# fenghuayumo/DIVSHOT

Hardware: AMD Instinct MI355X
Metric: train views/sec (fwd+bwd raster) at 1M splats 1920x1080 (higher is better)
Workload: dtype f32; 1 GPU; C3: 1000000 splats, 1920x1080, SH degree 3, 8 views per iteration sharded over 1 GPU(s) (BASELINE config C4), 8 view(s) per GPU per step as 1 multi-view pass(es) of 8 view(s) (dvs_raster_forward_views / dvs_raster_backward_*); absgrad=True, mode=batch, stagger=False, groups=1, views_per_group=8, early_gather=False, a9_chunks=1, async_forward=True, hip_graph=False, fwd_variant=quadrant, grad_mode=0, tile_bounds=canonical, shN_layout=tiled[N/64][45][64]

## Files before the change

### divshot_amd/_lib.py

```python
import ctypes as C
import os

_HERE = os.path.dirname(os.path.abspath(__file__))
LIB_PATH = os.environ.get("DVS_RASTER_LIB") or os.path.join(_HERE, "lib", "libdvsraster.so")


class DvsError(RuntimeError):
    pass


if not os.path.exists(LIB_PATH):
    raise ImportError(
        f"{LIB_PATH} is missing: build it with `make -C divshot_amd/csrc` (or __graft_entry__.build()). "
        "divshot_amd has no CPU fallback.")

lib = C.CDLL(LIB_PATH, mode=C.RTLD_GLOBAL)


class Splats(C.Structure):
    _fields_ = [("pos", C.c_void_p), ("sh0", C.c_void_p), ("shN", C.c_void_p), ("opacity", C.c_void_p),
                ("scale", C.c_void_p), ("rot", C.c_void_p), ("n", C.c_int32), ("_pad", C.c_int32)]


class Camera(C.Structure):
    _fields_ = [("view", C.c_float * 16), ("proj", C.c_float * 16), ("tan_fovx", C.c_float), ("tan_fovy", C.c_float),
                ("focal_x", C.c_float), ("focal_y", C.c_float), ("campos", C.c_float * 3), ("width", C.c_int32),
                ("height", C.c_int32), ("bg", C.c_float * 3)]


class Opts(C.Structure):
    _fields_ = [("sh_degree", C.c_int32), ("antialias", C.c_int32), ("absgrad", C.c_int32), ("accumulate", C.c_int32),
                ("shn_layout", C.c_int32), ("grad_mode", C.c_int32), ("tile_bounds", C.c_int32), ("_reserved", C.c_int32 * 1)]


class FwdState(C.Structure):
    _fields_ = [("radii", C.c_void_p), ("splat2d", C.c_void_p), ("depth", C.c_void_p), ("flags", C.c_void_p), ("tiles_touched", C.c_void_p), ("sorted_tile", C.c_void_p),
                ("sorted_splat", C.c_void_p), ("ranges", C.c_void_p), ("final_T", C.c_void_p), ("n_contrib", C.c_void_p),
                ("num_rendered", C.c_uint64), ("n", C.c_int32), ("width", C.c_int32), ("height", C.c_int32),
                ("tiles_x", C.c_int32), ("tiles_y", C.c_int32), ("_pad", C.c_int32)]


class SplatGrads(C.Structure):
    _fields_ = [("pos", C.c_void_p), ("sh0", C.c_void_p), ("shN", C.c_void_p), ("opacity", C.c_void_p),
                ("scale", C.c_void_p), ("rot", C.c_void_p), ("absgrad2d", C.c_void_p), ("mean2d", C.c_void_p), ("dcolor", C.c_void_p)]


class DensifyParams(C.Structure):
    _fields_ = [("grad_threshold", C.c_float), ("scale_threshold", C.c_float), ("min_opacity", C.c_float), ("max_world_scale", C.c_float),
                ("max_screen_radius", C.c_int32), ("cap_max", C.c_int32), ("seed", C.c_uint32), ("shn_layout", C.c_int32), ("revised_opacity", C.c_int32)]


class AdamGroup(C.Structure):
    _fields_ = [("param", C.c_void_p), ("grad", C.c_void_p), ("m", C.c_void_p), ("v", C.c_void_p), ("count", C.c_uint64),
                ("lr", C.c_float), ("width", C.c_int32), ("layout", C.c_int32), ("active_chunks", C.c_int32)]


class MetricsView(C.Structure):
    _fields_ = [("img", C.c_void_p), ("target", C.c_void_p), ("mask", C.c_void_p)]


class DownsampleView(C.Structure):
    _fields_ = [("src", C.c_void_p), ("dst", C.c_void_p)]


class McmcSets(C.Structure):
    _fields_ = [("param", C.c_void_p * 6), ("m", C.c_void_p * 6), ("v", C.c_void_p * 6)]


class SceneSpec(C.Structure):
    _fields_ = [("n", C.c_int32), ("width", C.c_int32), ("height", C.c_int32), ("sh_degree", C.c_int32),
                ("n_cams", C.c_int32), ("seed", C.c_uint64), ("fov_x_deg", C.c_float), ("scale_log_offset", C.c_float)]


_PROTOS = {
    "dvs_create": (C.c_void_p, [C.c_int, C.c_size_t, C.c_int, C.c_int]),
    "dvs_create_views": (C.c_void_p, [C.c_int, C.c_size_t, C.c_int, C.c_int, C.c_int]),
    "dvs_destroy": (None, [C.c_void_p]),
    "dvs_raster_forward_views": (C.c_int, [C.c_void_p, C.c_void_p, C.POINTER(Splats), C.POINTER(Camera), C.c_int, C.POINTER(Opts), C.c_void_p]),
    "dvs_raster_forward_cancel_prepared": (C.c_int, [C.c_void_p]),
    "dvs_raster_forward_views_prepare": (C.c_int, [C.c_void_p, C.c_void_p, C.POINTER(Splats), C.POINTER(Camera), C.c_int, C.POINTER(Opts), C.c_int64, C.c_int64]),
    "dvs_raster_backward_views": (C.c_int, [C.c_void_p, C.c_void_p, C.POINTER(Splats), C.POINTER(Camera), C.c_int, C.POINTER(Opts),
                                            C.c_void_p, C.POINTER(SplatGrads)]),
    "dvs_get_view_state": (C.c_int, [C.c_void_p, C.c_int, C.POINTER(FwdState)]),
    "dvs_raster_forward": (C.c_int, [C.c_void_p, C.c_void_p, C.POINTER(Splats), C.POINTER(Camera), C.POINTER(Opts),
                                     C.c_void_p, C.POINTER(FwdState), C.POINTER(C.c_uint64)]),
    "dvs_raster_backward": (C.c_int, [C.c_void_p, C.c_void_p, C.POINTER(Splats), C.POINTER(Camera), C.POINTER(Opts),
                                      C.c_void_p, C.POINTER(SplatGrads)]),
    "dvs_raster_backward_composite": (C.c_int, [C.c_void_p, C.c_void_p, C.c_void_p, C.POINTER(Opts), C.c_void_p]),
    "dvs_raster_backward_project": (C.c_int, [C.c_void_p, C.c_void_p, C.POINTER(Splats), C.c_void_p, C.POINTER(Opts),
                                              C.POINTER(SplatGrads)]),
    "dvs_raster_backward_project_chunk": (C.c_int, [C.c_void_p, C.c_void_p, C.POINTER(Splats), C.c_void_p, C.POINTER(Opts),
                                                    C.POINTER(SplatGrads), C.c_int64, C.c_int64]),
    "dvs_raster_backward_dcolor": (C.c_int, [C.c_void_p, C.c_void_p, C.c_void_p]),
    "dvs_sh_grad_combine": (C.c_int, [C.c_void_p, C.c_void_p, C.c_int, C.c_void_p, C.c_int, C.c_int, C.c_void_p, C.c_void_p, C.c_void_p,
                                      C.c_void_p, C.c_int, C.c_int]),
    "dvs_shn_relayout": (C.c_int, [C.c_void_p, C.c_void_p, C.c_int, C.c_void_p, C.c_void_p, C.c_int]),
    "dvs_sort_pairs_u32": (C.c_int, [C.c_void_p, C.c_void_p, C.c_void_p, C.c_void_p, C.c_uint64, C.c_int, C.c_int]),
    "dvs_export_sorted_keys": (C.c_int, [C.c_void_p, C.c_void_p, C.c_void_p]),
    "dvs_get_bwd_intermediates": (C.c_int, [C.c_void_p, C.POINTER(C.c_void_p), C.POINTER(C.c_int)]),
    "dvs_keep_bwd_intermediates": (C.c_int, [C.c_void_p, C.c_int]),
    "dvs_set_async": (C.c_int, [C.c_void_p, C.c_int]),
    "dvs_get_num_rendered": (C.c_int, [C.c_void_p, C.c_void_p, C.POINTER(C.c_uint64)]),
    "dvs_get_sort_rank_mode": (C.c_int, [C.c_void_p]),
    "dvs_debug_sort_depth_keys": (C.c_int, [C.c_void_p, C.c_void_p, C.c_void_p, C.c_uint64, C.c_void_p, C.POINTER(C.c_uint32), C.POINTER(C.c_uint32)]),
    "dvs_set_export_sorted_tiles": (C.c_int, [C.c_void_p, C.c_int]),
    "dvs_get_arena_info": (C.c_int, [C.c_void_p, C.POINTER(C.c_uint64), C.POINTER(C.c_uint64), C.POINTER(C.c_uint64), C.POINTER(C.c_uint64)]),
    "dvs_set_backward_variant": (C.c_int, [C.c_void_p, C.c_int]),
    "dvs_debug_record_decisions": (C.c_int, [C.c_void_p, C.c_void_p, C.c_uint64]),
    "dvs_set_forward_variant": (C.c_int, [C.c_void_p, C.c_int]),
    "dvs_set_live_lists": (C.c_int, [C.c_void_p, C.c_int]),
    "dvs_enable_stage_timing": (C.c_int, [C.c_void_p, C.c_int]),
    "dvs_enable_kernel_probe": (C.c_int, [C.c_void_p, C.c_int]),
    "dvs_read_kernel_probe": (C.c_int, [C.c_void_p, C.POINTER(C.c_float), C.POINTER(C.c_int)]),
    "dvs_get_stage_timing": (C.c_int, [C.c_void_p, C.POINTER(C.POINTER(C.c_char_p)), C.POINTER(C.POINTER(C.c_float))]),
    "dvs_memcpy_d2h": (C.c_int, [C.c_void_p, C.c_void_p, C.c_void_p, C.c_size_t]),
    "dvs_memcpy_h2d": (C.c_int, [C.c_void_p, C.c_void_p, C.c_void_p, C.c_size_t]),
    "dvs_device_malloc": (C.c_void_p, [C.c_void_p, C.c_size_t]),
    "dvs_device_free": (None, [C.c_void_p, C.c_void_p]),
    "dvs_comm_create": (C.c_void_p, [C.c_int, C.c_int, C.c_int, C.c_char_p, C.c_int]),
    "dvs_comm_bootstrap": (C.c_int, [C.c_int, C.c_int, C.c_char_p, C.c_int, C.c_void_p]),
    "dvs_comm_destroy": (None, [C.c_void_p]),
    "dvs_comm_rank": (C.c_int, [C.c_void_p]),
    "dvs_comm_world": (C.c_int, [C.c_void_p]),
    "dvs_comm_backend_ranks": (C.c_int, [C.c_void_p]),
    "dvs_comm_backend_name": (C.c_char_p, [C.c_void_p]),
    "dvs_comm_all_reduce_sum_f32": (C.c_int, [C.c_void_p, C.c_void_p, C.c_void_p, C.c_size_t]),
    "dvs_comm_all_reduce_max_i32": (C.c_int, [C.c_void_p, C.c_void_p, C.c_void_p, C.c_size_t]),
    "dvs_comm_reduce_scatter_sum_f32": (C.c_int, [C.c_void_p, C.c_void_p, C.c_void_p, C.c_void_p, C.c_size_t]),
    "dvs_comm_all_gather_f32": (C.c_int, [C.c_void_p, C.c_void_p, C.c_void_p, C.c_void_p, C.c_size_t]),
    "dvs_comm_broadcast": (C.c_int, [C.c_void_p, C.c_void_p, C.c_void_p, C.c_size_t, C.c_int]),
    "dvs_comm_group_start": (C.c_int, [C.c_void_p]),
    "dvs_comm_group_end": (C.c_int, [C.c_void_p]),
    "dvs_last_error": (C.c_char_p, []),
    "dvs_version": (C.c_char_p, []),
    "dvs_synth_splats": (C.c_int, [C.POINTER(SceneSpec)] + [C.c_void_p] * 6),
    "dvs_synth_camera": (C.c_int, [C.POINTER(SceneSpec), C.c_int, C.POINTER(Camera)]),
    "dvs_synth_target": (C.c_int, [C.POINTER(SceneSpec), C.c_int, C.c_void_p]),
    "dvs_make_camera": (C.c_int, [C.c_void_p, C.c_void_p, C.c_float, C.c_int, C.c_int, C.POINTER(Camera)]),
    "dvs_make_camera_intrinsics": (C.c_int, [C.c_void_p, C.c_void_p, C.c_double, C.c_double, C.c_double, C.c_double, C.c_int, C.c_int, C.POINTER(Camera)]),
    "dvs_camera_downscale": (C.c_int, [C.POINTER(Camera), C.c_int, C.POINTER(Camera)]),
    "dvs_l1_loss_grad": (C.c_int, [C.c_void_p, C.c_void_p, C.c_void_p, C.c_size_t, C.c_void_p, C.c_void_p]),
    "dvs_l1_loss_grad_w": (C.c_int, [C.c_void_p, C.c_void_p, C.c_void_p, C.c_size_t, C.c_float, C.c_void_p, C.c_void_p]),
    "dvs_l2_loss_grad": (C.c_int, [C.c_void_p, C.c_void_p, C.c_void_p, C.c_size_t, C.c_float, C.c_void_p, C.c_void_p]),
    "dvs_ssim_forward": (C.c_int, [C.c_void_p, C.c_void_p, C.c_void_p, C.c_int, C.c_int, C.c_void_p, C.c_void_p, C.c_void_p, C.c_void_p]),
    "dvs_ssim_backward": (C.c_int, [C.c_void_p, C.c_void_p, C.c_void_p, C.c_int, C.c_int, C.c_void_p, C.c_void_p, C.c_void_p, C.c_float,
                                    C.c_void_p, C.c_int]),
    "dvs_loss_l1_ssim_backward": (C.c_int, [C.c_void_p, C.c_void_p, C.c_void_p, C.c_int, C.c_int, C.c_void_p, C.c_void_p, C.c_void_p, C.c_float,
                                            C.c_void_p, C.c_void_p]),
    "dvs_image_metrics_scratch_bytes": (C.c_size_t, [C.c_int, C.c_int, C.c_int]),
    "dvs_image_metrics_views": (C.c_int, [C.c_void_p, C.POINTER(MetricsView), C.c_int, C.c_int, C.c_int, C.c_int, C.c_void_p, C.c_void_p]),
    "dvs_downsample_views": (C.c_int, [C.c_void_p, C.POINTER(DownsampleView), C.c_int, C.c_int, C.c_int, C.c_int, C.c_int, C.c_int]),
    "dvs_densify_accumulate": (C.c_int, [C.c_void_p, C.c_int, C.c_void_p, C.c_void_p, C.c_int, C.c_int, C.c_void_p, C.c_void_p, C.c_void_p]),
    "dvs_densify_accumulate_rows": (C.c_int, [C.c_void_p, C.c_int, C.c_int, C.c_void_p, C.c_void_p, C.c_int, C.c_int, C.c_void_p, C.c_void_p, C.c_void_p]),
    "dvs_any_view_radius": (C.c_int, [C.c_void_p, C.c_int, C.c_int, C.c_void_p, C.c_void_p]),
    "dvs_densify_plan": (C.c_int, [C.c_void_p, C.c_int, C.c_void_p, C.c_void_p, C.c_void_p, C.c_void_p, C.c_void_p, C.POINTER(DensifyParams),
                                   C.c_void_p, C.c_void_p, C.c_void_p, C.c_void_p]),
    "dvs_densify_apply": (C.c_int, [C.c_void_p, C.c_int, C.c_void_p, C.c_void_p, C.POINTER(DensifyParams), C.c_int, C.c_void_p, C.c_void_p, C.c_int]),
    "dvs_reset_opacity": (C.c_int, [C.c_void_p, C.c_int, C.c_void_p, C.c_float, C.c_void_p, C.c_void_p]),
    "dvs_adam_step": (C.c_int, [C.c_void_p, C.c_void_p, C.c_void_p, C.c_void_p, C.c_void_p, C.c_size_t, C.c_float, C.c_float,
                                C.c_float, C.c_float, C.c_int]),
    "dvs_mcmc_scratch_bytes": (C.c_size_t, [C.c_int]),
    "dvs_mcmc_init_scratch": (C.c_int, [C.c_void_p, C.c_void_p, C.c_int]),
    "dvs_mcmc_relocate": (C.c_int, [C.c_void_p, C.c_int, C.POINTER(McmcSets), C.c_float, C.c_uint32, C.c_int, C.c_void_p, C.c_int, C.c_void_p]),
    "dvs_mcmc_grow": (C.c_int, [C.c_void_p, C.c_int, C.c_int, C.POINTER(McmcSets), C.c_float, C.c_uint32, C.c_int, C.c_void_p, C.c_int]),
    "dvs_mcmc_add_noise": (C.c_int, [C.c_void_p, C.c_int, C.c_void_p, C.c_void_p, C.c_void_p, C.c_void_p, C.c_float, C.c_uint32]),
    "dvs_mcmc_regularize": (C.c_int, [C.c_void_p, C.c_int, C.c_void_p, C.c_void_p, C.c_void_p, C.c_void_p, C.c_float, C.c_float]),
    "dvs_mcmc_add_noise_range": (C.c_int, [C.c_void_p, C.c_int, C.c_int, C.c_int, C.c_void_p, C.c_void_p, C.c_void_p, C.c_void_p, C.c_float, C.c_uint32]),
    "dvs_mcmc_regularize_range": (C.c_int, [C.c_void_p, C.c_int, C.c_int, C.c_int, C.c_void_p, C.c_void_p, C.c_void_p, C.c_void_p, C.c_float, C.c_float]),
    "dvs_adam_step_groups": (C.c_int, [C.c_void_p, C.POINTER(AdamGroup), C.c_int, C.c_float, C.c_float, C.c_float, C.c_int, C.c_void_p,
                                       C.c_int32]),
}
class SpzLayout(C.Structure):
    _fields_ = [("off", C.c_uint64 * 6), ("bytes", C.c_uint64 * 6), ("total", C.c_uint64)]


_EXPORT_PROTOS = {
    "dvs_pack_scratch_bytes": (C.c_size_t, [C.c_int]),
    "dvs_pack_compressed": (C.c_int, [C.c_void_p, C.c_int, C.c_void_p, C.c_void_p, C.c_void_p, C.c_void_p, C.c_void_p, C.c_void_p, C.c_void_p,
                                      C.c_void_p, C.c_void_p]),
    "dvs_pack_splat32": (C.c_int, [C.c_void_p, C.c_int, C.c_void_p, C.c_void_p, C.c_void_p, C.c_void_p, C.c_void_p, C.c_void_p]),
    "dvs_spz_layout_for": (C.c_int, [C.c_int, C.c_int, C.POINTER(SpzLayout)]),
    "dvs_pack_spz": (C.c_int, [C.c_void_p, C.c_int, C.c_int, C.c_void_p, C.c_void_p, C.c_void_p, C.c_int, C.c_void_p, C.c_void_p, C.c_void_p,
                               C.c_void_p]),
    "dvs_unpack_spz": (C.c_int, [C.c_void_p, C.c_int, C.c_int, C.c_void_p, C.c_void_p, C.c_void_p, C.c_void_p, C.c_int, C.c_void_p, C.c_void_p,
                                 C.c_void_p]),
}
_INIT_PROTOS = {
    "dvs_knn_scratch_bytes": (C.c_size_t, [C.c_int]),
    "dvs_knn_mean_dist2": (C.c_int, [C.c_void_p, C.c_int, C.c_void_p, C.c_void_p, C.c_void_p]),
    "dvs_knn_mean_dist2_stats": (C.c_int, [C.c_void_p, C.c_int, C.c_void_p, C.c_void_p, C.c_void_p, C.c_void_p]),
    "dvs_init_from_points": (C.c_int, [C.c_void_p, C.c_int, C.c_void_p, C.c_void_p, C.c_void_p, C.c_void_p, C.c_void_p, C.c_void_p, C.c_void_p]),
}
class JpegDesc(C.Structure):
    _fields_ = [("width", C.c_int32), ("height", C.c_int32), ("components", C.c_int32), ("hs", C.c_int32), ("vs", C.c_int32),
                ("blocks_w", C.c_int32 * 3), ("blocks_h", C.c_int32 * 3), ("_pad", C.c_int32), ("offset", C.c_uint64 * 3),
                ("quant", (C.c_uint16 * 64) * 3)]


_IMAGE_PROTOS = {
    "dvs_jpeg_reconstruct": (C.c_int, [C.c_void_p, C.POINTER(JpegDesc), C.c_void_p, C.c_void_p]),
}
for _name, (_res, _args) in list(_PROTOS.items()) + list(_EXPORT_PROTOS.items()) + list(_INIT_PROTOS.items()) + list(_IMAGE_PROTOS.items()):
    _f = getattr(lib, _name)
    _f.restype = _res
    _f.argtypes = _args


def check(status, what="dvs call"):
    if status != 0:
        raise DvsError(f"{what} failed with status {status}: {lib.dvs_last_error().decode()}")


_JPEG_HOST_PROTOS = {
    "gstrain_jpeg_open": (C.c_void_p, [C.c_char_p, C.c_char_p, C.c_int]),
    "gstrain_jpeg_info": (C.c_int, [C.c_void_p, C.c_void_p, C.c_void_p, C.c_void_p]),
    "gstrain_jpeg_coefficients": (C.c_int, [C.c_void_p, C.c_void_p]),
    "gstrain_jpeg_close": (None, [C.c_void_p]),
}
_host_lib = None


def host_lib():
    global _host_lib
    if _host_lib is None:
        path = os.path.join(_HERE, "lib", "libgsplyio.so")
        if not os.path.exists(path):
            raise ImportError(f"{path} is missing: build it with `make -C divshot_amd/gstrain`")
        h = C.CDLL(path)
        for name, (res, args) in _JPEG_HOST_PROTOS.items():
            f = getattr(h, name)
            f.restype = res
            f.argtypes = args
        _host_lib = h
    return _host_lib


def jpeg_decode_coefficients(path):
    import numpy as np
    h = host_lib()
    err = C.create_string_buffer(1024)
    f = h.gstrain_jpeg_open(os.fsencode(path), err, 1024)
    if not f:
        raise DvsError(err.value.decode(errors="replace"))
    try:
        ints, offs, desc = (C.c_int32 * 15)(), (C.c_uint64 * 4)(), JpegDesc()
        check(h.gstrain_jpeg_info(f, ints, C.addressof(desc.quant), offs), "gstrain_jpeg_info")
        desc.width, desc.height, desc.components, desc.hs, desc.vs = ints[0], ints[1], ints[2], ints[3], ints[6]
        for k in range(3):
            desc.blocks_w[k], desc.blocks_h[k], desc.offset[k] = ints[9 + k], ints[12 + k], offs[k]
        coef = np.zeros(offs[3], np.int16)
        check(h.gstrain_jpeg_coefficients(f, coef.ctypes.data), "gstrain_jpeg_coefficients")
        return desc, coef
    finally:
        h.gstrain_jpeg_close(f)
```

### divshot_amd/csrc/dvs_api.cpp

```cpp
#include <hip/hip_runtime.h>
#include <cstddef>
#include <cstdio>
#include <cstdlib>
#include <cstdint>
#include <cstring>
#include <mutex>
#include <string>
#include <vector>
#include "../../include/dvs_raster.h"
#include "dvs_kernels.h"

static thread_local std::string g_last_error;
static void set_error(const char* what, hipError_t e, const char* file, int line) {
    char buf[512];
    snprintf(buf, sizeof buf, "%s: %s (%s:%d)", what, hipGetErrorString(e), file, line);
    g_last_error = buf;
}
void dvs_set_last_error(const char* msg) { g_last_error = msg ? msg : ""; }
static int fail(int code, const char* who, const char* what) { g_last_error = std::string(who) + ": " + what; return code; }
#define HIPCHECK(expr) do { hipError_t _e = (expr); if (_e != hipSuccess) { set_error(#expr, _e, __FILE__, __LINE__); return DVS_ERR_HIP; } } while (0)
#define TRY(expr) do { int _r = (expr); if (_r != DVS_OK) return _r; } while (0)

namespace {
struct Buf {
    void* p = nullptr;
    size_t bytes = 0;
    ~Buf() { if (p) (void)hipFree(p); }
    int ensure(size_t need) {
        if (need <= bytes) return DVS_OK;
        if (p) { (void)hipFree(p); p = nullptr; bytes = 0; }
        size_t want = need + need / 4;
        hipError_t e = hipMalloc(&p, want);
        if (e != hipSuccess) { e = hipMalloc(&p, need); want = need; }
        if (e != hipSuccess) { set_error("hipMalloc", e, __FILE__, __LINE__); p = nullptr; return DVS_ERR_HIP; }
        bytes = want;
        return DVS_OK;
    }
    template <class T> T* as() const { return (T*)p; }
};
struct Carver {
    char* base; size_t off = 0;
    template <class T> T* take(size_t count) { T* p = base ? (T*)(base + off) : nullptr; off += count * sizeof(T); return p; }
};

static_assert(sizeof(DvsCam) == sizeof(dvs_camera) && offsetof(DvsCam, campos) == offsetof(dvs_camera, campos) &&
              offsetof(DvsCam, bg) == offsetof(dvs_camera, bg), "DvsCam must mirror dvs_camera");
DvsCam to_dev_cam(const dvs_camera& c) { DvsCam d; memcpy(&d, &c, sizeof d); return d; }
DvsCams pack_cams(const dvs_camera* cams, int V) {
    DvsCams d;
    for (int v = 0; v < V; ++v) d.c[v] = to_dev_cam(cams[v]);
    return d;
}
struct CamVec3 {
    float v[DVS_MAX_VIEWS * 3];
    CamVec3(const dvs_camera* cams, int V, float (dvs_camera::*field)[3]) {
        for (int i = 0; i < V; ++i) for (int k = 0; k < 3; ++k) v[3 * i + k] = (cams[i].*field)[k];
    }
};
int bits_for(uint32_t max_value) { int b = 0; while (max_value) { ++b; max_value >>= 1; } return b; }

struct TileGrid {
    int tiles_x, tiles_y, tiles, rect_fmt;
    TileGrid(int W, int H, int tile_bounds = DVS_TILES_CANONICAL)
        : tiles_x((W + DVS_TILE - 1) / DVS_TILE), tiles_y((H + DVS_TILE - 1) / DVS_TILE), tiles(tiles_x * tiles_y),
          rect_fmt(tile_bounds == DVS_TILES_TIGHT ? DVS_FE_RECT_TIGHT : (tiles_x <= 255 && tiles_y <= 255) ? DVS_FE_RECT_U8 : DVS_FE_RECT_U16) {}
};

struct FwdPass {
    hipStream_t st;
    const dvs_splats* p; const dvs_camera* cams; int V; const dvs_opts* opts;
    int n; TileGrid g;
    uint64_t T = 0, T_expected = 0;
    const uint64_t* T_dev = nullptr;
    int icur = 0;
    int ranges_encoded = 0;
    bool keys_written = true;
};

struct Arenas {
    Buf radii, splat2d, depth, flags, tiles_touched, rect, rect_sorted, key[2], ids[2];
    Buf ranges, final_T, n_contrib;
    Buf ranges_canon;
    Buf inst_tile[2], inst_splat[2];
    uint64_t inst_cap = 0;
    uint64_t inst_grow_events = 0;
    uint64_t* total_dev = nullptr;
    uint64_t* total_host = nullptr;
    uint64_t overflow_seen = 0;
    Buf tmp_keys, tmp_vals;
};
struct FrontEnd {
    Buf state, hist;
    uint32_t nbv = 0, nsb = 0;
    int rank_atomic = 0;
    DvsSeg *seg_all = nullptr, *seg_vis = nullptr, *seg_tile = nullptr;
    uint32_t *superexcl = nullptr, *totals = nullptr, *block_sums = nullptr, *kred = nullptr, *tile_ranges = nullptr;
    unsigned long long* super = nullptr;
    size_t zero_bytes = 0;
    int seg_n = -1, seg_V = -1;
    uint32_t seg_rows = 0;
    size_t carve_state(void* base, int max_views) {
        Carver k{(char*)base};
        seg_all = k.take<DvsSeg>(DVS_MAX_VIEWS); seg_vis = k.take<DvsSeg>(DVS_MAX_VIEWS); seg_tile = k.take<DvsSeg>(DVS_MAX_VIEWS);
        superexcl = k.take<uint32_t>((size_t)max_views * nsb);
        totals = k.take<uint32_t>((size_t)max_views * DVS_FE_MAXBINS);
        block_sums = k.take<uint32_t>((size_t)max_views * nbv);
        return k.off;
    }
    size_t carve_ranges(void* base, int max_views, size_t tiles) {
        Carver k{(char*)base};
        kred = k.take<uint32_t>(DVS_FE_KRED_WORDS);
        super = k.take<unsigned long long>((size_t)max_views * nsb * DVS_FE_SUPER_STRIDE);
        zero_bytes = k.off = (k.off + 255) & ~(size_t)255;
        tile_ranges = k.take<uint32_t>(tiles * 2);
        return k.off;
    }
};
struct Forward {
    dvs_fwd_state st{};
    int n_views = 1;
    bool have = false;
    uint32_t* live_splat = nullptr;
    uint32_t* live_pos = nullptr;
    bool live_lists = true;
    uint64_t* rec_masks = nullptr; uint64_t rec_cap = 0;
    struct Prep {
        bool valid = false;
        int64_t next = 0;
        int n = 0, V = 0;
        dvs_splats p{};
        dvs_opts opts{};
        dvs_camera cams[DVS_MAX_VIEWS];
    } prep;
};
struct Backward {
    Buf g_rows;
    Buf dcolor;
    int variant = DVS_BWD_TR;
    bool keep_rows = false;
    bool rows_clean = false;
    bool rows_pending = false;
    int64_t proj_next = 0;
};
struct Timing {
    struct Span { const char* name; size_t begin, end; };
    bool on = false;
    std::vector<hipEvent_t> events;
    size_t used = 0;
    std::vector<Span> spans;
    std::vector<const char*> out_names;
    std::vector<float> out_ms;
};
struct Probe {
    bool on = false;
    std::vector<hipEvent_t> ev;
    std::vector<int> kind;
    size_t used = 0;
};
}

struct dvs_ctx {
    int device = 0;
    size_t max_splats = 0;
    int max_w = 0, max_h = 0;
    int max_views = 1;
    bool async_T = false;
    bool export_tiles = false;
    Arenas a;
    FrontEnd fe;
    Forward fwd;
    Backward bwd;
    Timing timing;
    Probe probe;
    ~dvs_ctx() {
        if (a.total_dev) (void)hipFree(a.total_dev);
        if (a.total_host) (void)hipHostFree(a.total_host);
        for (const auto* pool : {&timing.events, &probe.ev}) for (hipEvent_t e : *pool) (void)hipEventDestroy(e);
    }
};

namespace {
enum : unsigned { DROP_FWD = 1u, DROP_ROWS = 2u, DROP_PREP = 4u, DROP_SEGS = 8u };
void invalidate(dvs_ctx* c, unsigned what) {
    if (what & DROP_FWD) c->fwd.have = false;
    if (what & DROP_ROWS) c->bwd.rows_pending = false;
    if (what & DROP_PREP) c->fwd.prep.valid = false;
    if (what & DROP_SEGS) c->fe.seg_n = -1;
}

struct StageScope {
    dvs_ctx* c; hipStream_t st; bool append; size_t last = 0;
    StageScope(dvs_ctx* c_, hipStream_t s, bool append_) : c(c_), st(s), append(append_) { c->timing.used = 0; c->timing.spans.clear(); }
    size_t mark() {
        Timing& t = c->timing;
        if (!t.on) return 0;
        if (t.used == t.events.size()) { hipEvent_t e; (void)hipEventCreate(&e); t.events.push_back(e); }
        (void)hipEventRecord(t.events[t.used], st);
        return t.used++;
    }
    void begin() { last = mark(); }
    void stage(const char* name) { const size_t e = mark(); if (c->timing.on) c->timing.spans.push_back({name, last, e}); last = e; }
    int finish() {
        Timing& t = c->timing;
        if (!t.on) return DVS_OK;
        HIPCHECK(hipStreamSynchronize(st));
        if (!append) { t.out_names.clear(); t.out_ms.clear(); }
        for (const Timing::Span& s : t.spans) {
            float ms = 0.f;
            (void)hipEventSynchronize(t.events[s.end]);
            (void)hipEventElapsedTime(&ms, t.events[s.begin], t.events[s.end]);
            t.out_names.push_back(s.name); t.out_ms.push_back(ms);
        }
        return DVS_OK;
    }
};
void probe_event(dvs_ctx* c, hipStream_t st, int opens = -1) {
    Probe& pr = c->probe;
    if (!pr.on) return;
    if (pr.used == pr.ev.size()) { hipEvent_t e; (void)hipEventCreate(&e); pr.ev.push_back(e); }
    (void)hipEventRecord(pr.ev[pr.used++], st);
    if (opens >= 0) pr.kind.push_back(opens);
}

bool fe_no_key16() { static const bool v = [] { const char* e = getenv("DVS_FE_NO_KEY16"); return e && e[0] == '1'; }(); return v; }
bool fe_no_fuse() { static const bool v = [] { const char* e = getenv("DVS_FE_NO_FUSE_A6"); return e && e[0] == '1'; }(); return v; }

int ensure_frontend_arenas(dvs_ctx* c) {
    FrontEnd& fe = c->fe;
    dvs_fe_block_counts((int)c->max_splats, &fe.nbv, &fe.nsb);
    TRY(fe.state.ensure(fe.carve_state(nullptr, c->max_views)));
    fe.carve_state(fe.state.p, c->max_views);
    return fe.hist.ensure(dvs_fe_hist_words((uint64_t)c->max_splats * c->max_views, c->max_views, DVS_FE_MAXBINS) * 4);
}
int ensure_splat_arenas(dvs_ctx* c, size_t n) {
    Arenas& a = c->a;
    const struct { Buf* buf; size_t each; } need[] = {{&a.radii, 4}, {&a.splat2d, 64}, {&a.depth, 4}, {&a.flags, 4}, {&a.tiles_touched, 4},
        {&a.rect, 16}, {&a.rect_sorted, 16}, {&a.key[0], 4}, {&a.key[1], 4}, {&a.ids[0], 4}, {&a.ids[1], 4}, {&c->bwd.g_rows, 48}};
    for (const auto& x : need) TRY(x.buf->ensure(n * x.each));
    return DVS_OK;
}
int ensure_image_arenas(dvs_ctx* c, int w, int h, int views) {
    const size_t P = (size_t)w * h * views;
    const size_t tiles = (size_t)TileGrid(w, h).tiles * views;
    TRY(c->a.ranges.ensure(c->fe.carve_ranges(nullptr, c->max_views, tiles)));
    c->fe.carve_ranges(c->a.ranges.p, c->max_views, tiles);
    TRY(c->a.ranges_canon.ensure(tiles * 8));
    TRY(c->a.final_T.ensure(P * 4));
    return c->a.n_contrib.ensure(P * 4);
}
int ensure_instance_arenas(dvs_ctx* c, uint64_t T) {
    Arenas& a = c->a;
    if (a.inst_cap && T > a.inst_cap) ++a.inst_grow_events;
    uint64_t cap = (1ull << 32) - 1;
    for (Buf* b : {&a.inst_tile[0], &a.inst_splat[0], &a.inst_tile[1], &a.inst_splat[1]}) {
        TRY(b->ensure(T * 4));
        if (b->bytes / 4 < cap) cap = b->bytes / 4;
    }
    a.inst_cap = cap;
    return c->fe.hist.ensure(dvs_fe_hist_words(a.inst_cap, c->max_views, 512) * 4);
}
}

extern "C" {

const char* dvs_last_error(void) { return g_last_error.c_str(); }
const char* dvs_version(void) { return "divshot_amd raster 0.1 (gfx950)"; }

dvs_ctx* dvs_create_views(int device, size_t max_splats, int max_w, int max_h, int max_views) {
    int count = 0;
    hipError_t e = hipGetDeviceCount(&count);
    if (e != hipSuccess || device < 0 || device >= count) { fail(0, "dvs_create", "no such HIP device (the rasterizer has no CPU fallback)"); return nullptr; }
    if (max_views < 1 || max_views > DVS_MAX_VIEWS) { fail(0, "dvs_create_views", "max_views must be in [1, 16]"); return nullptr; }
    if ((e = hipSetDevice(device)) != hipSuccess) { set_error("hipSetDevice", e, __FILE__, __LINE__); return nullptr; }
    dvs_ctx* c = new dvs_ctx();
    c->device = device; c->max_splats = max_splats; c->max_w = max_w; c->max_h = max_h; c->max_views = max_views;
    if (const char* v = getenv("DVS_BWD_VARIANT")) c->bwd.variant = v[0] == '0' ? DVS_BWD_BLOCKS : DVS_BWD_TR;
    if (const char* v = getenv("DVS_LIVE_LISTS")) c->fwd.live_lists = v[0] != '0';
    if (hipMalloc((void**)&c->a.total_dev, 32) != hipSuccess || hipHostMalloc((void**)&c->a.total_host, 32, hipHostMallocDefault) != hipSuccess ||
        hipMemset(c->a.total_dev, 0, 32) != hipSuccess) {
        fail(0, "dvs_create", "hipMalloc failed");
        delete c;
        return nullptr;
    }
    c->a.total_host[0] = c->a.total_host[1] = c->a.total_host[2] = c->a.total_host[3] = 0;
    {
        static int probed[64];
        static std::mutex probe_mutex;
        std::lock_guard<std::mutex> probe_lock(probe_mutex);
        const char* mode = getenv("DVS_FE_RANK");
        if (mode && mode[0] == 'b') c->fe.rank_atomic = 0;
        else {
            if (device < 64 && probed[device] == 0) {
                uint32_t bad = 1u;
                uint32_t* word = nullptr;
                if (hipMalloc((void**)&word, 4) == hipSuccess && hipMemset(word, 0, 4) == hipSuccess && dvs_fe_probe_rank_atomic(nullptr, word) == hipSuccess &&
                    hipMemcpy(&bad, word, 4, hipMemcpyDeviceToHost) == hipSuccess)
                    probed[device] = bad == 0u ? 1 : 2;
                if (word) (void)hipFree(word);
            }
            c->fe.rank_atomic = (device < 64 && probed[device] == 1) ? 1 : 0;
        }
    }
    if (const char* v = getenv("DVS_ASYNC")) c->async_T = v[0] == '1';
    if (ensure_frontend_arenas(c) != DVS_OK ||
        ensure_splat_arenas(c, max_splats * (size_t)max_views) != DVS_OK || ensure_image_arenas(c, max_w, max_h, max_views) != DVS_OK ||
        ensure_instance_arenas(c, (uint64_t)max_splats * 4 * (uint64_t)max_views) != DVS_OK) {
        dvs_destroy(c);
        return nullptr;
    }
    return c;
}
dvs_ctx* dvs_create(int device, size_t max_splats, int max_w, int max_h) { return dvs_create_views(device, max_splats, max_w, max_h, 1); }

void dvs_destroy(dvs_ctx* c) {
    if (!c) return;
    (void)hipSetDevice(c->device);
    delete c;
}

static int run_a2(dvs_ctx* c, hipStream_t st, const dvs_splats* p, const dvs_camera* cams, int V, const dvs_opts* opts, int64_t first, int64_t count, bool begin) {
    const TileGrid g(cams[0].width, cams[0].height, opts->tile_bounds);
    Arenas& a = c->a;
    if (begin) HIPCHECK(hipMemsetAsync(a.ranges.p, 0, c->fe.zero_bytes + (size_t)g.tiles * V * 8, st));
    HIPCHECK(dvs_launch_preprocess_fwd(st, p->n, p->pos, p->sh0, p->shN, p->opacity, p->scale, p->rot, pack_cams(cams, V), V, opts->sh_degree,
                                       opts->antialias, g.tiles_x, g.tiles_y, a.radii.as<int>(), a.splat2d.as<float>(),
                                       a.depth.as<float>(), a.flags.as<uint32_t>(), a.tiles_touched.as<uint32_t>(), a.key[0].as<uint32_t>(),
                                       opts->shn_layout, a.rect.as<uint32_t>(), g.rect_fmt, c->fe.kred, (int)first, (int)count));
    return DVS_OK;
}
static bool prep_matches(const dvs_ctx* c, const dvs_splats* p, const dvs_camera* cams, int V, const dvs_opts* opts) {
    const Forward::Prep& q = c->fwd.prep;
    return q.valid && q.n == p->n && q.V == V && memcmp(&q.p, p, sizeof *p) == 0 && memcmp(&q.opts, opts, sizeof *opts) == 0 &&
           memcmp(q.cams, cams, sizeof(dvs_camera) * (size_t)V) == 0;
}
static void publish_prep(dvs_ctx* c, const dvs_splats* p, const dvs_camera* cams, int V, const dvs_opts* opts, int64_t next) {
    Forward::Prep& q = c->fwd.prep;
    q.valid = true; q.next = next; q.n = p->n; q.V = V; q.p = *p; q.opts = *opts;
    memcpy(q.cams, cams, sizeof(dvs_camera) * (size_t)V);
}
static int ensure_segs(dvs_ctx* c, hipStream_t st, int n, int V, uint32_t rows) {
    FrontEnd& fe = c->fe;
    if (fe.seg_n == n && fe.seg_V == V && fe.seg_rows == rows) return DVS_OK;
    HIPCHECK(dvs_launch_seg_init(st, n, V, rows, fe.seg_all));
    fe.seg_n = n; fe.seg_V = V; fe.seg_rows = rows;
    return DVS_OK;
}


static int fwd_capacity_policy(dvs_ctx* c, FwdPass& f) {
    if (!c->async_T) return DVS_OK;
    Arenas& a = c->a;
    const uint64_t lastT = a.total_host[0], overflow = a.total_host[1];
    const bool overflowed = overflow != a.overflow_seen;
    if (overflowed || lastT + lastT / 8 > a.inst_cap) {
        a.overflow_seen = overflow;
        HIPCHECK(hipStreamSynchronize(f.st));
        TRY(ensure_instance_arenas(c, lastT + lastT / 2));
        if (overflowed)
            return fail(DVS_ERR_CAPACITY, "dvs_raster_forward (async)", "an earlier forward on this context produced more tile instances than the "
                        "instance arena held; its outputs are invalid. The arena has been enlarged — repeat that view.");
    }
    f.T = a.inst_cap;
    f.T_dev = a.total_dev;
    f.T_expected = lastT > 0 ? lastT + lastT / 16 + 4096 : 0;
    return DVS_OK;
}
static int fwd_project(dvs_ctx* c, const FwdPass& f, StageScope& tm) {
    const bool prepared = prep_matches(c, f.p, f.cams, f.V, f.opts) && c->fwd.prep.next == (int64_t)f.n;
    invalidate(c, DROP_PREP);
    tm.begin();
    if (!prepared) TRY(run_a2(c, f.st, f.p, f.cams, f.V, f.opts, 0, f.n, true));
    tm.stage("preprocess_fwd");
    return DVS_OK;
}
static hipError_t seg_binning(dvs_ctx* c, const FwdPass& f, uint32_t tile_part, unsigned long long capacity, int stage,
                              uint32_t* inst_tile = nullptr, uint32_t* inst_splat = nullptr, int key16 = 0) {
    Arenas& a = c->a; FrontEnd& fe = c->fe;
    return dvs_launch_seg_binning(f.st, f.n, f.V, f.g.rect_fmt, fe.seg_vis, fe.seg_tile, a.ids[1].as<uint32_t>(), a.rect.as<uint32_t>(),
                                  a.rect_sorted.as<uint32_t>(), fe.block_sums, fe.super, fe.superexcl, tile_part,
                                  (unsigned long long*)a.total_dev, capacity, stage, f.g.tiles_x, inst_tile, inst_splat, key16);
}
static int fwd_bin(dvs_ctx* c, FwdPass& f, StageScope& tm) {
    Arenas& a = c->a; FrontEnd& fe = c->fe;
    hipStream_t st = f.st;
    const int n = f.n, V = f.V, tiles = f.g.tiles;
    if (n > 0) {
        TRY(ensure_segs(c, st, n, V, dvs_depth_sort_rows_per_view(n, V)));
        HIPCHECK(dvs_launch_depth_sort(st, n, V, a.key[0].as<uint32_t>(), a.ids[0].as<uint32_t>(), a.key[1].as<uint32_t>(), a.ids[1].as<uint32_t>(),
                                       fe.seg_all, fe.seg_vis, fe.kred, fe.hist.as<uint32_t>(), fe.totals, fe.rank_atomic));
    }
    tm.stage("depth_sort");
    const uint64_t lastT = a.total_host[0];
    const uint64_t t_hint = f.T_expected ? f.T_expected : (lastT ? lastT : (uint64_t)n * V * 3);
    const uint32_t tile_part = dvs_fe_part_for(t_hint);
    if (n > 0) HIPCHECK(seg_binning(c, f, tile_part, c->async_T ? a.inst_cap : ~0ull, 0));
    else HIPCHECK(hipMemsetAsync(a.total_dev, 0, 8, st));
    HIPCHECK(hipMemcpyAsync(a.total_host, a.total_dev, 32, hipMemcpyDeviceToHost, st));
    tm.stage("tile_scan");
    if (!c->async_T) {
        HIPCHECK(hipStreamSynchronize(st));
        f.T = a.total_host[0];
        if (f.T >= (1ull << 32)) return fail(DVS_ERR_CAPACITY, "dvs_raster_forward", "more than 2^32 tile instances");
        TRY(ensure_instance_arenas(c, f.T ? f.T : 1));
    }
    const int key16 = (tiles <= 65536 && !fe_no_key16()) ? 1 : 0;
    tm.begin();
    if (n > 0) HIPCHECK(seg_binning(c, f, tile_part, a.inst_cap, 1, a.inst_tile[0].as<uint32_t>(), a.inst_splat[0].as<uint32_t>(), key16));
    tm.stage("duplicate");
    const bool fuse_a6 = !fe_no_fuse();
    f.keys_written = !(fuse_a6 && c->async_T) || c->export_tiles;
    if (n > 0) {
        const uint64_t cap = c->async_T ? a.inst_cap : f.T;
        const uint32_t nbtot = (uint32_t)(cap / tile_part) + (uint32_t)V + 2u;
        HIPCHECK(dvs_launch_seg_sort(st, V, a.inst_tile[0].as<uint32_t>(), a.inst_splat[0].as<uint32_t>(), a.inst_tile[1].as<uint32_t>(),
                                     a.inst_splat[1].as<uint32_t>(), fe.seg_tile, 0, tiles > 1 ? bits_for((uint32_t)(tiles - 1)) : 1,
                                     c->async_T ? (f.T_expected ? f.T_expected : a.inst_cap) : f.T, tile_part, nbtot, fe.hist.as<uint32_t>(), fe.totals,
                                     (uint32_t)tiles, &f.icur, fuse_a6 ? fe.tile_ranges : nullptr, f.keys_written ? 1 : 0, key16, fe.rank_atomic));
    }
    tm.stage("tile_sort");
    if (fuse_a6) f.ranges_encoded = n > 0 ? 1 : 0;
    else HIPCHECK(dvs_launch_tile_ranges(st, f.T, a.inst_tile[f.icur].as<uint32_t>(), fe.tile_ranges, f.T_dev, f.T_expected));
    tm.stage("tile_ranges");
    return DVS_OK;
}
static int fwd_composite_and_publish(dvs_ctx* c, const FwdPass& f, float* out_rgb, dvs_fwd_state* saved, uint64_t* num_rendered, StageScope& tm) {
    Arenas& a = c->a; Forward& fw = c->fwd;
    const int W = f.cams[0].width, H = f.cams[0].height, icur = f.icur;
    probe_event(c, f.st, 0);
    fw.live_splat = nullptr; fw.live_pos = nullptr;
    uint64_t* rec_masks = nullptr; uint64_t rec_cap = 0;
    if (fw.rec_masks && f.V == 1 && !c->async_T) {
        rec_masks = fw.rec_masks; rec_cap = fw.rec_cap;
        HIPCHECK(hipMemsetAsync(rec_masks, 0, (size_t)(f.T < rec_cap ? f.T : rec_cap) * 32, f.st));
    }
    if (fw.live_lists && c->bwd.variant == DVS_BWD_TR) { fw.live_splat = a.inst_splat[icur ^ 1].as<uint32_t>(); fw.live_pos = a.inst_tile[icur ^ 1].as<uint32_t>(); }
    uint32_t* const canon = f.ranges_encoded ? a.ranges_canon.as<uint32_t>() : nullptr;
    HIPCHECK(dvs_launch_render_fwd(f.st, W, H, f.g.tiles_x, f.g.tiles_y, f.V, c->fe.tile_ranges, a.inst_splat[icur].as<uint32_t>(),
                                   a.splat2d.as<float>(), CamVec3(f.cams, f.V, &dvs_camera::bg).v, out_rgb, a.final_T.as<float>(),
                                   a.n_contrib.as<uint32_t>(), fw.live_splat, fw.live_pos, rec_masks, rec_cap, canon));
    probe_event(c, f.st);
    tm.stage("render_fwd");

    dvs_fwd_state& s = fw.st;
    s.radii = a.radii.as<int32_t>(); s.splat2d = a.splat2d.as<float>(); s.depth = a.depth.as<float>();
    s.flags = a.flags.as<uint32_t>();
    s.tiles_touched = a.tiles_touched.as<uint32_t>();
    s.sorted_tile = f.keys_written ? a.inst_tile[icur].as<uint32_t>() : nullptr; s.sorted_splat = a.inst_splat[icur].as<uint32_t>();
    s.ranges = canon ? canon : c->fe.tile_ranges; s.final_T = a.final_T.as<float>(); s.n_contrib = a.n_contrib.as<uint32_t>();
    s.num_rendered = c->async_T ? DVS_T_UNKNOWN : f.T; s.n = f.n; s.width = W; s.height = H; s.tiles_x = f.g.tiles_x; s.tiles_y = f.g.tiles_y;
    s._pad = 0;
    fw.n_views = f.V;
    fw.have = true;
    if (saved) *saved = s;
    if (num_rendered) *num_rendered = s.num_rendered;
    return DVS_OK;
}
static int check_fwd_args(dvs_ctx* c, const dvs_splats* p, const dvs_camera* cams, int V, const dvs_opts* opts, const float* out_rgb) {
    const char* const who = "dvs_raster_forward";
    if (!c || !p || !cams || !opts || !out_rgb) return fail(DVS_ERR_INVALID, who, "null argument");
    if (V < 1 || V > c->max_views) return fail(DVS_ERR_CAPACITY, who, "n_views exceeds the max_views given to dvs_create_views");
    const dvs_camera* cam = &cams[0];
    if (p->n < 0 || cam->width <= 0 || cam->height <= 0 || opts->sh_degree < 0 || opts->sh_degree > 3 ||
        (opts->shn_layout != DVS_SHN_ROWS && opts->shn_layout != DVS_SHN_TILED) ||
        (opts->tile_bounds != DVS_TILES_CANONICAL && opts->tile_bounds != DVS_TILES_TIGHT))
        return fail(DVS_ERR_INVALID, who, "bad n / image size / sh_degree / shn_layout / tile_bounds");
    for (int v = 1; v < V; ++v)
        if (cams[v].width != cam->width || cams[v].height != cam->height) return fail(DVS_ERR_INVALID, who, "the views of a batch must share one image size");
    if (p->n > 0 && (((uintptr_t)p->pos | (uintptr_t)p->sh0 | (uintptr_t)p->shN | (uintptr_t)p->opacity | (uintptr_t)p->scale | (uintptr_t)p->rot) & 15u))
        return fail(DVS_ERR_INVALID, who, "parameter arrays must be 16-byte aligned");
    if ((size_t)p->n > c->max_splats || cam->width > c->max_w || cam->height > c->max_h)
        return fail(DVS_ERR_CAPACITY, who, "exceeds the capacity given to dvs_create");
    if ((uint64_t)p->n * (uint64_t)V >= (1ull << 31)) return fail(DVS_ERR_CAPACITY, who, "n * n_views must stay below 2^31");
    return DVS_OK;
}
static int forward_views(dvs_ctx* c, hipStream_t st, const dvs_splats* p, const dvs_camera* cams, int V, const dvs_opts* opts,
                         float* out_rgb, dvs_fwd_state* saved, uint64_t* num_rendered) {
    TRY(check_fwd_args(c, p, cams, V, opts, out_rgb));
    HIPCHECK(hipSetDevice(c->device));
    FwdPass f{st, p, cams, V, opts, p->n, TileGrid(cams[0].width, cams[0].height, opts->tile_bounds)};
    invalidate(c, DROP_FWD | DROP_ROWS);
    StageScope tm(c, st, false);
    TRY(fwd_capacity_policy(c, f));
    TRY(fwd_project(c, f, tm));
    TRY(fwd_bin(c, f, tm));
    TRY(fwd_composite_and_publish(c, f, out_rgb, saved, num_rendered, tm));
    return tm.finish();
}

int dvs_raster_forward(dvs_ctx* c, void* stream, const dvs_splats* p, const dvs_camera* cam, const dvs_opts* opts,
                       float* out_rgb, dvs_fwd_state* saved, uint64_t* num_rendered) {
    return forward_views(c, (hipStream_t)stream, p, cam, 1, opts, out_rgb, saved, num_rendered);
}

int dvs_raster_forward_views(dvs_ctx* c, void* stream, const dvs_splats* p, const dvs_camera* cams, int n_views, const dvs_opts* opts,
                             float* out_rgb) {
    return forward_views(c, (hipStream_t)stream, p, cams, n_views, opts, out_rgb, nullptr, nullptr);
}

int dvs_raster_forward_cancel_prepared(dvs_ctx* c) {
    if (!c) return fail(DVS_ERR_INVALID, "dvs_raster_forward_cancel_prepared", "null context");
    invalidate(c, DROP_PREP);
    return DVS_OK;
}
int dvs_raster_forward_views_prepare(dvs_ctx* c, void* stream, const dvs_splats* p, const dvs_camera* cams, int n_views, const dvs_opts* opts,
                                     int64_t first, int64_t count) {
    const char* const who = "dvs_raster_forward_views_prepare";
    static float dummy_rgb;
    TRY(check_fwd_args(c, p, cams, n_views, opts, &dummy_rgb));
    if (opts->shn_layout != DVS_SHN_TILED) return fail(DVS_ERR_INVALID, who, "needs the DVS_SHN_TILED layout");
    const bool begin = first == 0;
    if (!begin && !(prep_matches(c, p, cams, n_views, opts) && c->fwd.prep.next == first)) {
        invalidate(c, DROP_PREP);
        return fail(DVS_ERR_STATE, who, "chunks must cover [0, n) in ascending order with the same parameters, cameras and options");
    }
    if (count <= 0 || first < 0 || first + count > p->n || (first % 256) != 0) {
        invalidate(c, DROP_PREP);
        return fail(DVS_ERR_INVALID, who, "bad chunk (each starts at a multiple of 256 and lies inside [0, n))");
    }
    HIPCHECK(hipSetDevice(c->device));
    if (begin) invalidate(c, DROP_FWD | DROP_ROWS | DROP_PREP);
    const int r = run_a2(c, (hipStream_t)stream, p, cams, n_views, opts, first, count, begin);
    if (r != DVS_OK) { invalidate(c, DROP_PREP); return r; }
    publish_prep(c, p, cams, n_views, opts, first + count);
    return DVS_OK;
}

int dvs_get_view_state(dvs_ctx* c, int view, dvs_fwd_state* out) {
    if (!c || !out) return fail(DVS_ERR_INVALID, "dvs_get_view_state", "null argument");
    if (!c->fwd.have || view < 0 || view >= c->fwd.n_views) return fail(DVS_ERR_STATE, "dvs_get_view_state", "no such view in the last forward");
    dvs_fwd_state s = c->fwd.st;
    const size_t on = (size_t)view * s.n, op = (size_t)view * s.width * s.height, ot = (size_t)view * s.tiles_x * s.tiles_y;
    s.radii += on; s.splat2d += on * DVS_S2D_FLOATS; s.depth += on; s.flags += on; s.tiles_touched += on;
    s.ranges += 2 * ot; s.final_T += op; s.n_contrib += op;
    *out = s;
    return DVS_OK;
}

static int bwd_composite(dvs_ctx* c, hipStream_t st, const dvs_camera* cams, const dvs_opts* opts, const float* dL_drgb, StageScope& tm) {
    const dvs_fwd_state& s = c->fwd.st;
    Backward& b = c->bwd;
    const int V = c->fwd.n_views;
    tm.begin();
    if (!b.rows_clean) HIPCHECK(hipMemsetAsync(b.g_rows.p, 0, b.g_rows.bytes, st));
    b.rows_clean = false;
    tm.stage("bwd_zero");
    const CamVec3 bgs(cams, V, &dvs_camera::bg);
    probe_event(c, st, 1);
    if (b.variant == DVS_BWD_TR)
        HIPCHECK(dvs_launch_render_bwd_tr(st, s.width, s.height, s.tiles_x, s.tiles_y, V, s.ranges, s.sorted_splat, s.splat2d, bgs.v, s.final_T,
                                          s.n_contrib, dL_drgb, b.g_rows.as<float>(), opts->absgrad, opts->grad_mode, c->fwd.live_splat, c->fwd.live_pos));
    else
        HIPCHECK(dvs_launch_render_bwd_blocks(st, s.width, s.height, s.tiles_x, s.tiles_y, V, s.ranges, s.sorted_splat, s.splat2d,
                                              bgs.v, s.final_T, s.n_contrib, dL_drgb, b.g_rows.as<float>(), opts->absgrad, opts->grad_mode));
    probe_event(c, st);
    tm.stage("render_bwd");
    b.rows_pending = true;
    b.proj_next = 0;
    return DVS_OK;
}
static int bwd_project(dvs_ctx* c, hipStream_t st, const dvs_splats* p, const dvs_camera* cams, const dvs_opts* opts,
                       const dvs_splat_grads* out, int64_t first, int64_t count, StageScope& tm) {
    const dvs_fwd_state& s = c->fwd.st;
    Backward& b = c->bwd;
    const int V = c->fwd.n_views, n = p->n;
    tm.begin();
    if (opts->shn_layout == DVS_SHN_TILED) {
        const char* nf = getenv("DVS_A9_NO_FUSE_SH");
        const bool no_fuse = nf && nf[0] == '1';
        const bool fuse = !out->dcolor && out->sh0 && out->shN && !no_fuse;
        float* dcol = out->dcolor;
        if (!dcol && !fuse) { TRY(b.dcolor.ensure((size_t)V * n * 3 * sizeof(float))); dcol = b.dcolor.as<float>(); }
        HIPCHECK(dvs_launch_preprocess_bwd_views(st, n, V, p->pos, p->shN, p->opacity, p->scale, p->rot, pack_cams(cams, V), opts->sh_degree,
                                                 opts->antialias, s.radii, s.flags, b.g_rows.as<float>(), out->pos, out->opacity, out->scale,
                                                 out->rot, opts->absgrad ? out->absgrad2d : nullptr, out->mean2d, dcol, opts->accumulate,
                                                 b.keep_rows ? 0 : 1, opts->grad_mode, (int)first, (int)count, fuse ? out->sh0 : nullptr,
                                                 fuse ? out->shN : nullptr));
        if (!fuse && out->sh0 && out->shN)
            HIPCHECK(dvs_launch_sh_grad_combine(st, n, p->pos, opts->sh_degree, V, CamVec3(cams, V, &dvs_camera::campos).v, dcol, out->sh0,
                                                out->shN, opts->accumulate, 1));
    } else {
        for (int v = 0; v < V; ++v) {
            const DvsCam dcam = to_dev_cam(cams[v]);
            const size_t on = (size_t)v * n;
            HIPCHECK(dvs_launch_preprocess_bwd(st, n, p->pos, p->shN, p->opacity, p->scale, p->rot, dcam, opts->sh_degree, opts->antialias,
                                               s.radii + on, s.flags + on, b.g_rows.as<float>() + on * 12, out->pos, out->sh0, out->shN,
                                               out->opacity, out->scale, out->rot, opts->absgrad ? out->absgrad2d : nullptr, out->mean2d,
                                               out->dcolor ? out->dcolor + on * 3 : nullptr, (opts->accumulate || v > 0) ? 1 : 0,
                                               b.keep_rows ? 0 : 1, opts->shn_layout, opts->grad_mode));
        }
    }
    tm.stage("preprocess_bwd");
    b.proj_next = first + count < n ? first + count : 0;
    if (b.proj_next != 0) return DVS_OK;
    b.rows_clean = !b.keep_rows;
    b.rows_pending = b.keep_rows;
    return DVS_OK;
}
static int check_bwd_args(dvs_ctx* c, const dvs_splats* p, const dvs_camera* cams, int V , const dvs_opts* opts, const char* who) {
    if (!c || !cams || !opts) return fail(DVS_ERR_INVALID, who, "null argument");
    if (V < 0) V = c->fwd.n_views;
    if (opts->grad_mode != DVS_GRAD_TRUE && opts->grad_mode != DVS_GRAD_LINEAGE) return fail(DVS_ERR_INVALID, who, "bad grad_mode");
    if (!c->fwd.have || V != c->fwd.n_views || (p && c->fwd.st.n != p->n) || c->fwd.st.width != cams[0].width || c->fwd.st.height != cams[0].height)
        return fail(DVS_ERR_STATE, who, "no matching forward on this context");
    return DVS_OK;
}
static int check_dL(const float* dL_drgb, const char* who) {
    if (!dL_drgb) return fail(DVS_ERR_INVALID, who, "null argument");
    if ((uintptr_t)dL_drgb & 15u) return fail(DVS_ERR_INVALID, who, "dL_drgb must be 16-byte aligned (the composite backward reads it as 16-byte words)");
    return DVS_OK;
}
static int check_grads(const dvs_splats* p, const dvs_splat_grads* out, const char* who) {
    if (!p || !out) return fail(DVS_ERR_INVALID, who, "null argument");
    if (p->n > 0 && (!out->pos || !out->opacity || !out->scale || !out->rot || ((!out->sh0 || !out->shN) && !out->dcolor)))
        return fail(DVS_ERR_INVALID, who, "null gradient row pointer (sh0/shN may be NULL only when dcolor is given)");
    if (p->n > 0 && (((uintptr_t)out->pos | (uintptr_t)out->sh0 | (uintptr_t)out->shN | (uintptr_t)out->opacity | (uintptr_t)out->scale |
                      (uintptr_t)out->rot | (uintptr_t)out->absgrad2d | (uintptr_t)out->mean2d | (uintptr_t)out->dcolor) & 15u))
        return fail(DVS_ERR_INVALID, who, "gradient arrays must be 16-byte aligned");
    return DVS_OK;
}

static int backward_views(dvs_ctx* c, void* stream, const dvs_splats* p, const dvs_camera* cams, int V, const dvs_opts* opts,
                          const float* dL_drgb, const dvs_splat_grads* out, const char* who) {
    TRY(check_dL(dL_drgb, "dvs_raster_backward"));
    TRY(check_grads(p, out, who));
    TRY(check_bwd_args(c, p, cams, V, opts, who));
    HIPCHECK(hipSetDevice(c->device));
    StageScope tm(c, (hipStream_t)stream, true);
    TRY(bwd_composite(c, tm.st, cams, opts, dL_drgb, tm));
    TRY(bwd_project(c, tm.st, p, cams, opts, out, 0, p->n, tm));
    return tm.finish();
}
int dvs_raster_backward(dvs_ctx* c, void* stream, const dvs_splats* p, const dvs_camera* cam, const dvs_opts* opts,
                        const float* dL_drgb, const dvs_splat_grads* out) {
    return backward_views(c, stream, p, cam, 1, opts, dL_drgb, out, "dvs_raster_backward");
}
int dvs_raster_backward_views(dvs_ctx* c, void* stream, const dvs_splats* p, const dvs_camera* cams, int n_views, const dvs_opts* opts,
                              const float* dL_drgb, const dvs_splat_grads* out) {
    return backward_views(c, stream, p, cams, n_views, opts, dL_drgb, out, "dvs_raster_backward_views");
}

int dvs_raster_backward_composite(dvs_ctx* c, void* stream, const dvs_camera* cam, const dvs_opts* opts, const float* dL_drgb) {
    const char* const who = "dvs_raster_backward_composite";
    TRY(check_dL(dL_drgb, who));
    TRY(check_bwd_args(c, nullptr, cam, -1, opts, who));
    HIPCHECK(hipSetDevice(c->device));
    StageScope tm(c, (hipStream_t)stream, true);
    TRY(bwd_composite(c, tm.st, cam, opts, dL_drgb, tm));
    return tm.finish();
}

static int check_project(dvs_ctx* c, const dvs_splats* p, const dvs_camera* cam, const dvs_opts* opts, const dvs_splat_grads* out,
                         const char* who, const char* pending) {
    TRY(check_grads(p, out, who));
    TRY(check_bwd_args(c, p, cam, -1, opts, who));
    return c->bwd.rows_pending ? DVS_OK : fail(DVS_ERR_STATE, who, pending);
}
int dvs_raster_backward_project(dvs_ctx* c, void* stream, const dvs_splats* p, const dvs_camera* cam, const dvs_opts* opts,
                                const dvs_splat_grads* out) {
    const char* const who = "dvs_raster_backward_project";
    TRY(check_project(c, p, cam, opts, out, who, "no dvs_raster_backward_composite on this context"));
    if (c->bwd.proj_next != 0)
        return fail(DVS_ERR_STATE, who, "a dvs_raster_backward_project_chunk sequence is in progress on this context (finish it up to n)");
    HIPCHECK(hipSetDevice(c->device));
    StageScope tm(c, (hipStream_t)stream, true);
    TRY(bwd_project(c, tm.st, p, cam, opts, out, 0, p->n, tm));
    return tm.finish();
}

int dvs_raster_backward_project_chunk(dvs_ctx* c, void* stream, const dvs_splats* p, const dvs_camera* cam, const dvs_opts* opts,
                                      const dvs_splat_grads* out, int64_t first, int64_t count) {
    const char* const who = "dvs_raster_backward_project_chunk";
    TRY(check_project(c, p, cam, opts, out, who, "no dvs_raster_backward_composite pending on this context"));
    if (opts->shn_layout != DVS_SHN_TILED || !out->dcolor || out->sh0 || out->shN)
        return fail(DVS_ERR_INVALID, who, "needs the DVS_SHN_TILED layout and the factorised form (out->dcolor given, sh0 / shN NULL)");
    if (first != c->bwd.proj_next || count <= 0 || first + count > p->n || (first % 256) != 0)
        return fail(DVS_ERR_INVALID, who, "chunks must cover [0, n) in ascending order, each starting at a multiple of 256");
    HIPCHECK(hipSetDevice(c->device));
    StageScope tm(c, (hipStream_t)stream, true);
    TRY(bwd_project(c, tm.st, p, cam, opts, out, first, count, tm));
    return tm.finish();
}

int dvs_sort_pairs_u32(dvs_ctx* c, void* stream, uint32_t* keys, uint32_t* vals, uint64_t n, int bit_lo, int bit_hi) {
    if (!c || (n > 0 && (!keys || !vals)) || bit_lo < 0 || bit_hi > 32 || bit_lo > bit_hi) return fail(DVS_ERR_INVALID, "dvs_sort_pairs_u32", "bad argument");
    HIPCHECK(hipSetDevice(c->device));
    hipStream_t st = (hipStream_t)stream;
    if (n == 0) return DVS_OK;
    TRY(c->a.tmp_keys.ensure(n * 4));
    TRY(c->a.tmp_vals.ensure(n * 4));
    uint32_t* k[2] = {keys, c->a.tmp_keys.as<uint32_t>()};
    uint32_t* v[2] = {vals, c->a.tmp_vals.as<uint32_t>()};
    int cur = 0;
    if (n > (1ull << 32) - 4097ull) return fail(DVS_ERR_CAPACITY, "dvs_sort_pairs_u32", "n must be at most 2^32 - 4097");
    TRY(c->fe.hist.ensure(dvs_fe_hist_words(n, 1, 512) * 4));
    const uint32_t part = dvs_fe_part_for(n);
    HIPCHECK(dvs_launch_seg_init(st, (int)n, 1, 0, c->fe.seg_all));
    invalidate(c, DROP_SEGS);
    HIPCHECK(dvs_launch_seg_sort(st, 1, k[0], v[0], k[1], v[1], c->fe.seg_all, bit_lo, bit_hi - bit_lo, n, part, (uint32_t)(n / part) + 3u,
                                 c->fe.hist.as<uint32_t>(), c->fe.totals, 0u, &cur, nullptr, 1, 0, c->fe.rank_atomic));
    if (cur == 1) {
        HIPCHECK(hipMemcpyAsync(keys, k[1], n * 4, hipMemcpyDeviceToDevice, st));
        HIPCHECK(hipMemcpyAsync(vals, v[1], n * 4, hipMemcpyDeviceToDevice, st));
    }
    return DVS_OK;
}

int dvs_debug_sort_depth_keys(dvs_ctx* c, void* stream, const uint32_t* keys, uint64_t n, uint32_t* sorted_ids, uint32_t* n_sorted, uint32_t* digit_bits) {
    if (!c || !keys || !sorted_ids || !n_sorted || n == 0 || n > c->max_splats * (uint64_t)c->max_views || n >= (1ull << 31))
        return fail(DVS_ERR_INVALID, "dvs_debug_sort_depth_keys", "bad argument (n must be in [1, max_splats * max_views])");
    HIPCHECK(hipSetDevice(c->device));
    hipStream_t st = (hipStream_t)stream;
    Arenas& a = c->a; FrontEnd& fe = c->fe;
    std::vector<uint32_t> h(n);
    HIPCHECK(hipMemcpyAsync(h.data(), keys, n * 4, hipMemcpyDeviceToHost, st));
    HIPCHECK(hipStreamSynchronize(st));
    uint32_t mn = 0xFFFFFFFFu, mx = 0u; bool any = false;
    for (uint32_t k : h) if (k != 0xFFFFFFFFu) { mn = k < mn ? k : mn; mx = k > mx ? k : mx; any = true; }
    uint32_t slots[64 * 16] = {0};
    if (any) { slots[0] = ~mn; slots[1] = mx; }
    invalidate(c, DROP_FWD | DROP_PREP | DROP_SEGS);
    HIPCHECK(hipMemcpyAsync(fe.kred, slots, sizeof slots, hipMemcpyHostToDevice, st));
    HIPCHECK(hipMemcpyAsync(a.key[0].p, keys, n * 4, hipMemcpyDeviceToDevice, st));
    HIPCHECK(dvs_launch_seg_init(st, (int)n, 1, dvs_depth_sort_rows_per_view((int)n, 1), fe.seg_all));
    HIPCHECK(dvs_launch_depth_sort(st, (int)n, 1, a.key[0].as<uint32_t>(), a.ids[0].as<uint32_t>(), a.key[1].as<uint32_t>(), a.ids[1].as<uint32_t>(),
                                   fe.seg_all, fe.seg_vis, fe.kred, fe.hist.as<uint32_t>(), fe.totals, fe.rank_atomic));
    DvsSeg sv;
    HIPCHECK(hipMemcpyAsync(&sv, fe.seg_vis, sizeof sv, hipMemcpyDeviceToHost, st));
    HIPCHECK(hipStreamSynchronize(st));
    *n_sorted = sv.count;
    if (digit_bits) *digit_bits = sv.bits;
    HIPCHECK(hipMemcpyAsync(sorted_ids, a.ids[1].p, (size_t)sv.count * 4, hipMemcpyDeviceToDevice, st));
    HIPCHECK(hipMemsetAsync(fe.kred, 0, sizeof slots, st));
    return DVS_OK;
}

int dvs_export_sorted_keys(dvs_ctx* c, void* stream, uint64_t* out_keys) {
    const char* const who = "dvs_export_sorted_keys";
    if (!c || !out_keys) return fail(DVS_ERR_INVALID, who, "null argument");
    if (!c->fwd.have) return fail(DVS_ERR_STATE, who, "no forward state");
    const dvs_fwd_state& s = c->fwd.st;
    if (s.num_rendered == DVS_T_UNKNOWN) { uint64_t t; TRY(dvs_get_num_rendered(c, stream, &t)); }
    if (!s.sorted_tile)
        return fail(DVS_ERR_STATE, who, "the last forward was asynchronous (dvs_set_async) and did not materialise the sorted tile ids; "
                    "export the keys of a synchronous forward");
    HIPCHECK(hipSetDevice(c->device));
    HIPCHECK(dvs_launch_export_keys((hipStream_t)stream, s.num_rendered, s.sorted_tile, s.sorted_splat, s.depth, out_keys));
    return DVS_OK;
}

int dvs_shn_relayout(dvs_ctx* c, void* stream, int n, const float* src, float* dst, int to_tiled) {
    if (!c || n < 0 || (n > 0 && (!src || !dst))) return fail(DVS_ERR_INVALID, "dvs_shn_relayout", "bad argument");
    HIPCHECK(hipSetDevice(c->device));
    HIPCHECK(dvs_launch_shn_relayout((hipStream_t)stream, n, src, dst, to_tiled));
    return DVS_OK;
}

int dvs_sh_grad_combine(dvs_ctx* c, void* stream, int n, const float* pos, int sh_degree, int n_views, const float* campos,
                        const float* dcolor, float* g_sh0, float* g_shN, int accumulate, int shn_layout) {
    if (!c || n < 0 || n_views < 0 || sh_degree < 0 || sh_degree > 3 || (n > 0 && n_views > 0 && (!pos || !campos || !dcolor || !g_sh0 || !g_shN)))
        return fail(DVS_ERR_INVALID, "dvs_sh_grad_combine", "bad argument");
    HIPCHECK(hipSetDevice(c->device));
    HIPCHECK(dvs_launch_sh_grad_combine((hipStream_t)stream, n, pos, sh_degree, n_views, campos, dcolor, g_sh0, g_shN, accumulate, shn_layout));
    return DVS_OK;
}

int dvs_raster_backward_dcolor(dvs_ctx* c, void* stream, float* dcolor) {
    const char* const who = "dvs_raster_backward_dcolor";
    if (!c || !dcolor || ((uintptr_t)dcolor & 15u)) return fail(DVS_ERR_INVALID, who, "bad argument (dcolor: 16-byte aligned device array)");
    if (!c->bwd.rows_pending) return fail(DVS_ERR_STATE, who, "no dvs_raster_backward_composite pending on this context");
    HIPCHECK(hipSetDevice(c->device));
    const dvs_fwd_state& s = c->fwd.st;
    HIPCHECK(dvs_launch_dcolor_from_rows((hipStream_t)stream, (int64_t)c->fwd.n_views * s.n, s.radii, s.flags, c->bwd.g_rows.as<float>(), dcolor));
    return DVS_OK;
}

int dvs_set_async(dvs_ctx* c, int enable) {
    if (!c) return fail(DVS_ERR_INVALID, "dvs_set_async", "null context");
    c->async_T = enable != 0;
    return DVS_OK;
}
int dvs_get_num_rendered(dvs_ctx* c, void* stream, uint64_t* T) {
    const char* const who = "dvs_get_num_rendered";
    if (!c || !T) return fail(DVS_ERR_INVALID, who, "null argument");
    if (!c->fwd.have) return fail(DVS_ERR_STATE, who, "no forward state");
    HIPCHECK(hipSetDevice(c->device));
    HIPCHECK(hipStreamSynchronize((hipStream_t)stream));
    Arenas& a = c->a;
    *T = a.total_host[0];
    c->fwd.st.num_rendered = *T;
    if (a.total_host[1] != a.overflow_seen) {
        a.overflow_seen = a.total_host[1];
        (void)ensure_instance_arenas(c, *T + *T / 2);
        return fail(DVS_ERR_CAPACITY, who, "the last forward produced more tile instances than the instance arena held; its outputs are "
                    "invalid. The arena has been enlarged — repeat that view.");
    }
    return DVS_OK;
}

int dvs_get_sort_rank_mode(dvs_ctx* c) { return c ? c->fe.rank_atomic : -1; }
int dvs_set_export_sorted_tiles(dvs_ctx* c, int enable) {
    if (!c) return fail(DVS_ERR_INVALID, "dvs_set_export_sorted_tiles", "null context");
    c->export_tiles = enable != 0;
    return DVS_OK;
}

int dvs_get_arena_info(dvs_ctx* c, uint64_t* cap, uint64_t* grows, uint64_t* last_T, uint64_t* overflows) {
    if (!c) return fail(DVS_ERR_INVALID, "dvs_get_arena_info", "null context");
    if (cap) *cap = c->a.inst_cap;
    if (grows) *grows = c->a.inst_grow_events;
    if (last_T) *last_T = c->a.total_host[0];
    if (overflows) *overflows = c->a.total_host[1];
    return DVS_OK;
}

int dvs_debug_record_decisions(dvs_ctx* c, uint64_t* take_masks, uint64_t capacity_instances) {
    if (!c || (take_masks && (((uintptr_t)take_masks & 7u) || capacity_instances == 0))) return fail(DVS_ERR_INVALID, "dvs_debug_record_decisions", "bad argument");
    c->fwd.rec_masks = take_masks; c->fwd.rec_cap = take_masks ? capacity_instances : 0;
    return DVS_OK;
}

int dvs_set_backward_variant(dvs_ctx* c, int variant) {
    const char* const who = "dvs_set_backward_variant";
    if (!c || variant < DVS_BWD_BLOCKS || variant > DVS_BWD_TR) return fail(DVS_ERR_INVALID, who, "bad argument");
    if (variant == DVS_BWD_REDUCE || variant == DVS_BWD_MM)
        return fail(DVS_ERR_UNSUPPORTED, who, "the 'reduce' and 'mm' kernels are retired — this library contains 'tr' (default) and 'blocks' only");
    c->bwd.variant = variant;
    return DVS_OK;
}
int dvs_set_live_lists(dvs_ctx* c, int enable) {
    if (!c) return fail(DVS_ERR_INVALID, "dvs_set_live_lists", "null context");
    c->fwd.live_lists = enable != 0;
    return DVS_OK;
}
int dvs_set_forward_variant(dvs_ctx* c, int variant) {
    if (!c || (variant != 0 && variant != 1)) return fail(DVS_ERR_INVALID, "dvs_set_forward_variant", "bad argument");
    if (variant == 0)
        return fail(DVS_ERR_UNSUPPORTED, "dvs_set_forward_variant", "the per-block forward is retired — this library contains the quadrant forward only");
    return DVS_OK;
}

int dvs_keep_bwd_intermediates(dvs_ctx* c, int keep) { if (!c) return DVS_ERR_INVALID; c->bwd.keep_rows = keep != 0; return DVS_OK; }

int dvs_get_bwd_intermediates(dvs_ctx* c, const float** rows, int* row_floats) {
    if (!c) return DVS_ERR_INVALID;
    if (rows) *rows = c->bwd.g_rows.as<float>();
    if (row_floats) *row_floats = 12;
    return DVS_OK;
}

int dvs_enable_stage_timing(dvs_ctx* c, int enable) { if (!c) return DVS_ERR_INVALID; c->timing.on = enable != 0; return DVS_OK; }
int dvs_enable_kernel_probe(dvs_ctx* c, int enable) {
    if (!c) return DVS_ERR_INVALID;
    c->probe.on = enable != 0;
    c->probe.used = 0; c->probe.kind.clear();
    return DVS_OK;
}
int dvs_read_kernel_probe(dvs_ctx* c, float mean_ms[2], int count[2]) {
    if (!c || !mean_ms || !count) return DVS_ERR_INVALID;
    HIPCHECK(hipSetDevice(c->device));
    Probe& pr = c->probe;
    double sum[2] = {0, 0};
    count[0] = count[1] = 0;
    for (size_t k = 0; k < pr.kind.size() && 2 * k + 1 < pr.used; ++k) {
        float ms = 0.f;
        HIPCHECK(hipEventSynchronize(pr.ev[2 * k + 1]));
        HIPCHECK(hipEventElapsedTime(&ms, pr.ev[2 * k], pr.ev[2 * k + 1]));
        sum[pr.kind[k]] += ms; count[pr.kind[k]]++;
    }
    for (int i = 0; i < 2; ++i) mean_ms[i] = count[i] ? (float)(sum[i] / count[i]) : 0.f;
    pr.used = 0; pr.kind.clear();
    return DVS_OK;
}
int dvs_get_stage_timing(dvs_ctx* c, const char*** names, const float** ms) {
    if (!c) return 0;
    if (names) *names = c->timing.out_names.data();
    if (ms) *ms = c->timing.out_ms.data();
    return (int)c->timing.out_names.size();
}

int dvs_memcpy_d2h(dvs_ctx* c, void* host_dst, const void* dev_src, size_t bytes) {
    if (!c) return DVS_ERR_INVALID;
    HIPCHECK(hipSetDevice(c->device));
    HIPCHECK(hipDeviceSynchronize());
    HIPCHECK(hipMemcpy(host_dst, dev_src, bytes, hipMemcpyDeviceToHost));
    return DVS_OK;
}
int dvs_memcpy_h2d(dvs_ctx* c, void* dev_dst, const void* host_src, size_t bytes) {
    if (!c) return DVS_ERR_INVALID;
    HIPCHECK(hipSetDevice(c->device));
    HIPCHECK(hipMemcpy(dev_dst, host_src, bytes, hipMemcpyHostToDevice));
    return DVS_OK;
}
void* dvs_device_malloc(dvs_ctx* c, size_t bytes) {
    if (!c) return nullptr;
    void* p = nullptr;
    if (hipSetDevice(c->device) != hipSuccess || hipMalloc(&p, bytes ? bytes : 1) != hipSuccess) return nullptr;
    return p;
}
void dvs_device_free(dvs_ctx* c, void* p) { if (c && p) { (void)hipSetDevice(c->device); (void)hipFree(p); } }

}
```

### divshot_amd/csrc/dvs_kernels.h

```cpp
#pragma once
#include <hip/hip_runtime.h>
#include <stdint.h>
#include "dvs_device.h"

hipError_t dvs_launch_preprocess_fwd(hipStream_t st, int n, const float* pos, const float* sh0, const float* shN,
                                     const float* opacity, const float* scale, const float* rot, const DvsCams& cams, int n_views,
                                     int deg, int antialias, int tiles_x, int tiles_y, int* radii , float* splat2d,
                                     float* depth, uint32_t* flags,
                                     uint32_t* tiles_touched, uint32_t* depth_key, int shn_tiled,
                                     uint32_t* rect , int rect_fmt ,
                                     uint32_t* kred ,
                                     int first, int count );
hipError_t dvs_launch_preprocess_bwd(hipStream_t st, int n, const float* pos, const float* shN, const float* opacity,
                                     const float* scale, const float* rot, const DvsCam& cam, int deg, int antialias,
                                     const int* radii, const uint32_t* flags, float* grad_rows ,
                                     float* g_pos, float* g_sh0, float* g_shN, float* g_opacity, float* g_scale,
                                     float* g_rot, float* out_absgrad2d , float* out_mean2d ,
                                     float* out_dcolor , int accumulate, int rezero_rows, int shn_tiled, int grad_mode);
hipError_t dvs_launch_preprocess_bwd_views(hipStream_t st, int n, int n_views, const float* pos, const float* shN, const float* opacity,
                                           const float* scale, const float* rot, const DvsCams& cams, int deg, int antialias,
                                           const int* radii, const uint32_t* flags, float* grad_rows, float* g_pos, float* g_opacity,
                                           float* g_scale, float* g_rot, float* out_absgrad2d, float* out_mean2d, float* out_dcolor,
                                           int accumulate, int rezero_rows, int grad_mode, int first, int count, float* g_sh0 ,
                                           float* g_shN );
hipError_t dvs_launch_sh_grad_combine(hipStream_t st, int n, const float* pos, int deg, int n_views, const float* campos_host,
                                      const float* dcolor, float* g_sh0, float* g_shN, int accumulate, int shn_tiled);
hipError_t dvs_launch_dcolor_from_rows(hipStream_t st, int64_t total, const int* radii, const uint32_t* flags, const float* rows, float* dcolor);
hipError_t dvs_launch_shn_relayout(hipStream_t st, int n, const float* src, float* dst, int to_tiled);

struct DvsSeg {
    uint32_t base;
    uint32_t count;
    uint32_t pstart;
    uint32_t sub;
    uint32_t bits;
    uint32_t _r0, _r1, _r2;
};
enum { DVS_FE_RECT_U8 = 0 ,
       DVS_FE_RECT_U16 = 1 ,
       DVS_FE_RECT_TIGHT = 2  };
template <int FMT> struct FeRect;
template <> struct FeRect<DVS_FE_RECT_U8> {
    typedef uint32_t T;
    static __device__ __forceinline__ T pack(uint32_t minx, uint32_t miny, uint32_t maxx, uint32_t maxy, unsigned long long) {
        return minx | (miny << 8) | ((maxx - minx) << 16) | ((maxy - miny) << 24);
    }
    static __device__ __forceinline__ uint32_t count(T r) { return ((r >> 16) & 0xFFu) * (r >> 24); }
    static __device__ __forceinline__ uint32_t minx(T r) { return r & 0xFFu; }
    static __device__ __forceinline__ uint32_t miny(T r) { return (r >> 8) & 0xFFu; }
    static __device__ __forceinline__ uint32_t width(T r) { return (r >> 16) & 0xFFu; }
    static __device__ __forceinline__ T zero() { return 0u; }
};
template <> struct FeRect<DVS_FE_RECT_U16> {
    typedef uint2 T;
    static __device__ __forceinline__ T pack(uint32_t minx, uint32_t miny, uint32_t maxx, uint32_t maxy, unsigned long long) {
        return make_uint2(minx | (maxx << 16), miny | (maxy << 16));
    }
    static __device__ __forceinline__ uint32_t count(T r) { return ((r.x >> 16) - (r.x & 0xFFFFu)) * ((r.y >> 16) - (r.y & 0xFFFFu)); }
    static __device__ __forceinline__ uint32_t minx(T r) { return r.x & 0xFFFFu; }
    static __device__ __forceinline__ uint32_t miny(T r) { return r.y & 0xFFFFu; }
    static __device__ __forceinline__ uint32_t width(T r) { return (r.x >> 16) - (r.x & 0xFFFFu); }
    static __device__ __forceinline__ T zero() { return make_uint2(0u, 0u); }
};
template <> struct FeRect<DVS_FE_RECT_TIGHT> {
    typedef uint4 T;
    static __device__ __forceinline__ T pack(uint32_t minx, uint32_t miny, uint32_t maxx, uint32_t maxy, unsigned long long mask) {
        return make_uint4(minx | (maxx << 16), miny | (maxy << 16), (uint32_t)mask, (uint32_t)(mask >> 32));
    }
    static __device__ __forceinline__ uint32_t count(T r) {
        const uint32_t both = r.z & r.w;
        return both == 0xFFFFFFFFu ? ((r.x >> 16) - (r.x & 0xFFFFu)) * ((r.y >> 16) - (r.y & 0xFFFFu)) : (uint32_t)(__popc(r.z) + __popc(r.w));
    }
    static __device__ __forceinline__ uint32_t minx(T r) { return r.x & 0xFFFFu; }
    static __device__ __forceinline__ uint32_t miny(T r) { return r.y & 0xFFFFu; }
    static __device__ __forceinline__ uint32_t width(T r) { return (r.x >> 16) - (r.x & 0xFFFFu); }
    static __device__ __forceinline__ T zero() { return make_uint4(0u, 0u, 0u, 0u); }
};
#define DVS_FE_KRED_WORDS (DVS_MAX_VIEWS * 64 * 16)
#define DVS_FE_MAXBINS 2048
#define DVS_FE_SUPER_STRIDE 32
size_t dvs_fe_hist_words(uint64_t max_elems, int n_views, int max_bins);
uint32_t dvs_depth_sort_rows_per_view(int n, int V);
uint32_t dvs_fe_part_for(uint64_t grid_elems);
void dvs_fe_block_counts(int n, uint32_t* nbv, uint32_t* nsb);
hipError_t dvs_launch_seg_init(hipStream_t st, int n, int V, uint32_t rows_per_view, DvsSeg* seg_all);
hipError_t dvs_launch_depth_sort(hipStream_t st, int n, int V, uint32_t* keys0, uint32_t* vals0, uint32_t* keys1, uint32_t* vals1,
                                 DvsSeg* seg_all, DvsSeg* seg_vis, const uint32_t* kred, uint32_t* hist, uint32_t* totals ,
                                 int rank_atomic = 0 );
hipError_t dvs_launch_seg_sort(hipStream_t st, int V, uint32_t* keys0, uint32_t* vals0, uint32_t* keys1, uint32_t* vals1, DvsSeg* seg, int bit_lo, int bits,
                               uint64_t grid_elems, uint32_t part, uint32_t nbtot, uint32_t* hist, uint32_t* totals, uint32_t key_add_per_view,
                               int* result_in, uint32_t* ranges_enc = nullptr ,
                               int write_last_keys = 1, int first_keys16 = 0 , int rank_atomic = 0);
hipError_t dvs_fe_probe_rank_atomic(hipStream_t st, uint32_t* bad_dev);
hipError_t dvs_launch_seg_binning(hipStream_t st, int n, int V, int rect_fmt, const DvsSeg* seg_vis, DvsSeg* seg_tile, const uint32_t* sorted_ids,
                                  const uint32_t* rect, uint32_t* rect_sorted, uint32_t* block_sums, unsigned long long* super, uint32_t* superexcl,
                                  uint32_t tile_part, unsigned long long* total_dev, unsigned long long capacity, int stage, int tiles_x,
                                  uint32_t* inst_tile, uint32_t* inst_splat, int key16 = 0 );

hipError_t dvs_launch_tile_ranges(hipStream_t st, uint64_t T, const uint32_t* sorted_tile, uint32_t* ranges ,
                                  const uint64_t* T_dev = nullptr, uint64_t T_expected = 0);
hipError_t dvs_launch_export_keys(hipStream_t st, uint64_t T, const uint32_t* sorted_tile, const uint32_t* sorted_splat,
                                  const float* depth, uint64_t* out_keys);

hipError_t dvs_launch_render_fwd(hipStream_t st, int W, int H, int tiles_x, int tiles_y, int n_views, const uint32_t* ranges ,
                                 const uint32_t* sorted_splat, const float* splat2d, const float* bgs, float* out_color, float* final_T,
                                 uint32_t* n_contrib, uint32_t* live_splat , uint32_t* live_pos ,
                                 uint64_t* take_masks ,
                                 uint64_t take_cap, uint32_t* ranges_out = nullptr );
enum { DVS_BWD_BLOCKS = 0 , DVS_BWD_REDUCE = 1 , DVS_BWD_MM = 2 ,
       DVS_BWD_TR = 3  };

hipError_t dvs_launch_render_bwd_tr(hipStream_t st, int W, int H, int tiles_x, int tiles_y, int n_views, const uint32_t* ranges,
                                    const uint32_t* sorted_splat, const float* splat2d, const float* bgs , const float* final_T,
                                    const uint32_t* n_contrib, const float* dL_dout, float* grad_rows, int absgrad, int grad_mode,
                                    const uint32_t* live_splat ,
                                    const uint32_t* live_pos);

hipError_t dvs_launch_render_bwd_blocks(hipStream_t st, int W, int H, int tiles_x, int tiles_y, int n_views, const uint32_t* ranges,
                                        const uint32_t* sorted_splat, const float* splat2d, const float* bgs , const float* final_T,
                                        const uint32_t* n_contrib, const float* dL_dout, float* grad_rows, int absgrad, int grad_mode);

size_t dvs_morton_scratch_bytes(int n);
hipError_t dvs_launch_morton_order(hipStream_t st, int n, const float* pos, void* scratch, const uint32_t** sorted, const float** bounds);
```

### divshot_amd/csrc/frontend.hip

```cpp
#include <cstdlib>
#include "dvs_device.h"
#include "dvs_kernels.h"

#define FE_BLOCK 256
#define FE_WAVES (FE_BLOCK / 64)
#define FE_MAXBINS DVS_FE_MAXBINS
#define FE_REORDER_BITS 9
#define FE_CULLED 0xFFFFFFFFu

__device__ __forceinline__ uint32_t fe_lane() { return __builtin_amdgcn_mbcnt_hi(~0u, __builtin_amdgcn_mbcnt_lo(~0u, 0u)); }

__device__ __forceinline__ uint64_t fe_match(uint32_t d, bool valid, uint32_t b) {
    const uint64_t v0 = __ballot(valid);
    uint32_t lo = (uint32_t)v0, hi = (uint32_t)(v0 >> 32);
    for (uint32_t k = 0; k < b; ++k) {
        const uint32_t m = (uint32_t)(((int32_t)(d << (31u - k))) >> 31);
        const uint64_t bal = __ballot(m != 0u);
        lo = lo & ~((uint32_t)bal ^ m);
        hi = hi & ~((uint32_t)(bal >> 32) ^ m);
    }
    const uint64_t peers = ((uint64_t)hi << 32) | lo;
    return valid ? peers : 0ull;
}

// ... 382 lines not shown
    int c = 0, shift = bit_lo;
    for (int k = 0; k < npass; ++k) {
        const bool last = k == npass - 1;
        hipError_t e = fe_launch_pass(L, kk[c], vv[c], (last && !write_last_keys) ? nullptr : kk[c ^ 1], vv[c ^ 1], seg, nullptr, 0, k, shift, widths[k], 0,
                                      last ? key_add_per_view : 0u, nullptr, last ? ranges_enc : nullptr, (k == 0 && first_keys16) ? 1 : 0);
        if (e != hipSuccess) return e;
        shift += widths[k];
        c ^= 1;
    }
    if (result_in) *result_in = c;
    return hipSuccess;
}

__global__ void __launch_bounds__(FE_BLOCK)
k_fe_probe_rank_atomic(uint32_t* __restrict__ bad, uint32_t seed) {
    __shared__ uint32_t cnt_a[FE_WAVES * 256];
    __shared__ uint16_t cnt_b[FE_WAVES * 512];
    const uint32_t lane = fe_lane(), wave = threadIdx.x >> 6;
    uint32_t errs = 0;
    for (uint32_t pat = 0; pat < 24; ++pat) {
        for (uint32_t e = threadIdx.x; e < FE_WAVES * 256; e += FE_BLOCK) cnt_a[e] = 0u;
        for (uint32_t e = threadIdx.x; e < FE_WAVES * 512; e += FE_BLOCK) cnt_b[e] = 0;
        __syncthreads();
        const uint32_t bits = pat < 8 ? 9u : 1u + (pat - 8u) % 9u;
        for (uint32_t r = 0; r < 16; ++r) {
            uint32_t h = (lane * 0x9E3779B1u) ^ ((blockIdx.x * FE_WAVES + wave) * 0x85EBCA6Bu) ^ ((pat * 16u + r) * 0xC2B2AE35u) ^ seed;
            h ^= h >> 15; h *= 0x2C1B3C6Du; h ^= h >> 12;
            uint32_t d;
            switch (pat) {
                case 0: d = 5u; break;
                case 1: d = 6u + (lane & 1u); break;
                case 2: d = lane >> 1; break;
                case 3: d = lane / 3u; break;
                case 4: d = lane >> 5; break;
                case 5: d = lane & 7u; break;
                case 6: d = (lane & 1u) ? 511u : (h & 3u); break;
                case 7: d = 63u - lane; break;
                default: d = h & ((1u << bits) - 1u); break;
            }
            const bool valid = (h >> 20 & 15u) != 0u || pat < 8;
            uint32_t ra = 0, rb = 0;
            if (valid) {
                const uint32_t old = atomicAdd(&cnt_a[wave * 256u + (d >> 1)], (d & 1u) ? 0x10000u : 1u);
                ra = (d & 1u) ? (old >> 16) : (old & 0xFFFFu);
            }
            const uint64_t peers = fe_match(d, valid, 9u);
            const uint32_t below = __builtin_amdgcn_mbcnt_hi((uint32_t)(peers >> 32), __builtin_amdgcn_mbcnt_lo((uint32_t)peers, 0u));
            if (valid) {
                const uint32_t prev = cnt_b[wave * 512u + d];
                if (below == 0) cnt_b[wave * 512u + d] = (uint16_t)(prev + (uint32_t)__popcll(peers));
                rb = prev + below;
            }
            errs += (valid && ra != rb) ? 1u : 0u;
        }
        __syncthreads();
    }
    if (errs) atomicAdd(bad, errs);
}
hipError_t dvs_fe_probe_rank_atomic(hipStream_t st, uint32_t* bad_dev ) {
    hipLaunchKernelGGL(k_fe_probe_rank_atomic, dim3(512), dim3(FE_BLOCK), 0, st, bad_dev, 0x1234567u);
    hipLaunchKernelGGL(k_fe_probe_rank_atomic, dim3(512), dim3(FE_BLOCK), 0, st, bad_dev, 0x89ABCDEu);
    return hipGetLastError();
}

template <int FMT>
__global__ void __launch_bounds__(FE_BLOCK)
k_seg_blocksum(int n, int V, uint32_t nbv, uint32_t nsb, const DvsSeg* __restrict__ seg_vis, const uint32_t* __restrict__ sorted_ids,
               const typename FeRect<FMT>::T* __restrict__ rect, typename FeRect<FMT>::T* __restrict__ rect_sorted,
               uint32_t* __restrict__ block_sums, unsigned long long* __restrict__ super) {
    __shared__ uint32_t wsum[4][FE_WAVES];
    const uint32_t view = blockIdx.x % (uint32_t)V, blk0 = (blockIdx.x / (uint32_t)V) * 4u;
    const uint32_t nvis = seg_vis[view].count;
    if (blk0 * FE_BLOCK >= nvis) return;
    const size_t o = (size_t)view * n;
    const uint32_t lane = fe_lane(), wave = threadIdx.x >> 6;
    uint32_t id[4];
#pragma unroll
    for (int k = 0; k < 4; ++k) { const uint32_t j = (blk0 + (uint32_t)k) * FE_BLOCK + threadIdx.x; id[k] = j < nvis ? sorted_ids[o + j] : 0u; }
    typename FeRect<FMT>::T r[4];
#pragma unroll
    for (int k = 0; k < 4; ++k) r[k] = rect[o + id[k]];
#pragma unroll
    for (int k = 0; k < 4; ++k) {
        const uint32_t j = (blk0 + (uint32_t)k) * FE_BLOCK + threadIdx.x;
        uint32_t v = 0;
        if (j < nvis) { rect_sorted[o + j] = r[k]; v = FeRect<FMT>::count(r[k]); }
        const uint32_t s = fe_wave_sum(v);
        if (lane == 0) wsum[k][wave] = s;
    }
    __syncthreads();
    if (threadIdx.x < 4) {
        const uint32_t k = threadIdx.x, blk = blk0 + k;
        uint32_t tot = 0;
#pragma unroll
        for (int wv = 0; wv < FE_WAVES; ++wv) tot += wsum[k][wv];
        if (blk < nbv) block_sums[(size_t)view * nbv + blk] = tot;
        const uint32_t t4 = tot + (uint32_t)__shfl_down(tot, 1, 64) + (uint32_t)__shfl_down(tot, 2, 64) + (uint32_t)__shfl_down(tot, 3, 64);
        if (k == 0 && t4) atomicAdd(&super[((size_t)view * nsb + (blk0 >> 8)) * DVS_FE_SUPER_STRIDE], (unsigned long long)t4);
    }
}

__global__ void __launch_bounds__(1024)
k_seg_totals(int V, uint32_t nsb, const unsigned long long* __restrict__ super, uint32_t* __restrict__ superexcl, DvsSeg* __restrict__ seg_tile,
             uint32_t tile_part, unsigned long long* __restrict__ total, unsigned long long capacity) {
    __shared__ unsigned long long vsum[DVS_MAX_VIEWS];
    const uint32_t lane = fe_lane(), wave = threadIdx.x >> 6;
    if (wave < (uint32_t)V) {
        unsigned long long carry = 0ull;
        for (uint32_t c0 = 0; c0 < nsb; c0 += 64) {
            const uint32_t i = c0 + lane;
            const unsigned long long v = i < nsb ? super[((size_t)wave * nsb + i) * DVS_FE_SUPER_STRIDE] : 0ull;
            unsigned long long inc = v;
#pragma unroll
            for (int k = 1; k < 64; k <<= 1) { const unsigned long long o = __shfl_up(inc, k, 64); if (lane >= (uint32_t)k) inc += o; }
            const unsigned long long ex = carry + inc - v;
            if (i < nsb) superexcl[(size_t)wave * nsb + i] = ex > 0xFFFFFFFFull ? 0xFFFFFFFFu : (uint32_t)ex;
            carry += __shfl(inc, 63, 64);
        }
        if (lane == 0) vsum[wave] = carry;
    }
    __syncthreads();
    if (threadIdx.x == 0) {
        unsigned long long start = 0ull;
        uint32_t prow = 0;
        for (int v = 0; v < V; ++v) {
            const unsigned long long end = start + vsum[v];
            const unsigned long long cs = start < capacity ? start : capacity, ce = end < capacity ? end : capacity;
            DvsSeg s;
            s.base = (uint32_t)cs; s.count = (uint32_t)(ce - cs); s.pstart = prow; s.sub = 0u; s.bits = 0u; s._r0 = s._r1 = s._r2 = 0u;
            seg_tile[v] = s;
            prow += (s.count + tile_part - 1) / tile_part;
            start = end;
        }
        total[0] = start;
        if (start > capacity) total[1] += 1ull;
    }
}

__device__ __forceinline__ uint32_t fe_nth_set_bit64(uint32_t lo, uint32_t hi, uint32_t t) {
    uint32_t w = lo, base = 0;
    const uint32_t c = (uint32_t)__popc(lo);
    if (t >= c) { t -= c; w = hi; base = 32u; }
#pragma unroll
    for (uint32_t h = 16u; h >= 1u; h >>= 1) {
        const uint32_t cl = (uint32_t)__popc(w & ((1u << h) - 1u));
        if (t >= cl) { t -= cl; w >>= h; base += h; }
    }
    return base;
}

__device__ __forceinline__ uint32_t fe_wave_incl_max(uint32_t v) {
#define FE_DPP_MAX(ctrl, rmask) { const uint32_t o_ = (uint32_t)__builtin_amdgcn_update_dpp(0, (int)v, ctrl, rmask, 0xF, false); v = v > o_ ? v : o_; }
    FE_DPP_MAX(0x111, 0xF); FE_DPP_MAX(0x112, 0xF); FE_DPP_MAX(0x114, 0xF); FE_DPP_MAX(0x118, 0xF);
    FE_DPP_MAX(0x142, 0xA);
    FE_DPP_MAX(0x143, 0xC);
#undef FE_DPP_MAX
    return v;
}
template <int FMT>
__global__ void __launch_bounds__(FE_BLOCK)
k_seg_duplicate(int n, int V, uint32_t nbv, uint32_t nsb, const DvsSeg* __restrict__ seg_vis, const DvsSeg* __restrict__ seg_tile,
                const uint32_t* __restrict__ sorted_ids, const typename FeRect<FMT>::T* __restrict__ rect_sorted,
                const uint32_t* __restrict__ block_sums, const uint32_t* __restrict__ superexcl, int tiles_x,
                uint32_t* __restrict__ inst_tile, uint32_t* __restrict__ inst_splat, unsigned long long capacity, int key16 ) {
    __shared__ uint32_t tmp[FE_WAVES];
    __shared__ uint32_t s_pre[FE_BLOCK];
    __shared__ uint32_t s_id[FE_BLOCK];
    __shared__ uint32_t s_tile[FE_BLOCK];
    __shared__ uint32_t s_w[FE_BLOCK];
    __shared__ uint32_t s_mark[FE_BLOCK];
    __shared__ uint2 s_mask[FMT == DVS_FE_RECT_TIGHT ? FE_BLOCK : 1];
    const uint32_t view = blockIdx.x % (uint32_t)V, blk0 = (blockIdx.x / (uint32_t)V) * 2u;
    const uint32_t nvis = seg_vis[view].count;
    if (blk0 * FE_BLOCK >= nvis) return;
    const size_t o = (size_t)view * n;
    const uint32_t lane = fe_lane(), w0 = (threadIdx.x >> 6) * 64u;
    uint32_t id[2] = {0u, 0u};
    typename FeRect<FMT>::T r[2] = {FeRect<FMT>::zero(), FeRect<FMT>::zero()};
#pragma unroll
    for (int h = 0; h < 2; ++h) {
        const uint32_t j = (blk0 + (uint32_t)h) * FE_BLOCK + threadIdx.x;
        if (j < nvis) { id[h] = sorted_ids[o + j]; r[h] = rect_sorted[o + j]; }
    }
    const uint32_t sb = blk0 >> 8, nprev = blk0 & 255u;
    const uint32_t part = threadIdx.x < nprev ? block_sums[(size_t)view * nbv + (size_t)sb * 256 + threadIdx.x] : 0u;
    const unsigned long long vbase = (unsigned long long)seg_tile[view].base + superexcl[(size_t)view * nsb + sb];
    uint32_t before, tot;
    (void)fe_block_excl_scan(part, tmp, &before);
#pragma unroll
    for (int h = 0; h < 2; ++h) {
        if ((blk0 + (uint32_t)h) * FE_BLOCK >= nvis) break;
        const uint32_t touched = FeRect<FMT>::count(r[h]);
        const uint32_t pre = fe_block_excl_scan(touched, tmp, &tot);
        s_pre[threadIdx.x] = pre;
        s_id[threadIdx.x] = (uint32_t)o + id[h];
        s_tile[threadIdx.x] = FeRect<FMT>::miny(r[h]) * (uint32_t)tiles_x + FeRect<FMT>::minx(r[h]);
        s_w[threadIdx.x] = FeRect<FMT>::width(r[h]);
        if constexpr (FMT == DVS_FE_RECT_TIGHT) s_mask[threadIdx.x] = make_uint2(r[h].z, r[h].w);
        const unsigned long long gbase = vbase + before;
        const uint32_t k_beg = (uint32_t)__builtin_amdgcn_readfirstlane((int)pre);
        const uint32_t k_end = (uint32_t)__builtin_amdgcn_readlane((int)(pre + touched), 63);
        uint32_t cur1 = 0;
        for (uint32_t k0 = k_beg; k0 < k_end; k0 += 64u) {
            s_mark[w0 + lane] = 0u;
            __builtin_amdgcn_wave_barrier();
            const uint32_t rel = pre - k0;
            if (touched != 0u && rel < 64u) s_mark[w0 + rel] = lane + 1u;
            __builtin_amdgcn_wave_barrier();
            uint32_t m = s_mark[w0 + lane];
            __builtin_amdgcn_wave_barrier();
            m = fe_wave_incl_max(m);
            m = m > cur1 ? m : cur1;
            cur1 = (uint32_t)__builtin_amdgcn_readlane((int)m, 63);
            const uint32_t k = k0 + lane;
            if (k < k_end) {
                const uint32_t src = w0 + m - 1u, w = s_w[src];
                uint32_t t = k - s_pre[src];
                if constexpr (FMT == DVS_FE_RECT_TIGHT) {
                    const uint2 mk = s_mask[src];
                    if ((mk.x & mk.y) != 0xFFFFFFFFu) t = fe_nth_set_bit64(mk.x, mk.y, t);
                }
                uint32_t q = (uint32_t)((float)t * __builtin_amdgcn_rcpf((float)w));
                int32_t rem = (int32_t)(t - q * w);
                if (rem < 0) { --q; rem += (int32_t)w; } else if (rem >= (int32_t)w) { ++q; rem -= (int32_t)w; }
                const unsigned long long g = gbase + k;
                if (g < capacity) {
                    const uint32_t tile = s_tile[src] + q * (uint32_t)tiles_x + (uint32_t)rem;
                    if (key16) reinterpret_cast<uint16_t*>(inst_tile)[g] = (uint16_t)tile; else inst_tile[g] = tile;
                    inst_splat[g] = s_id[src];
                }
            }
        }
        before += tot;
        __builtin_amdgcn_wave_barrier();
    }
}

hipError_t dvs_launch_seg_binning(hipStream_t st, int n, int V, int rect_fmt, const DvsSeg* seg_vis, DvsSeg* seg_tile, const uint32_t* sorted_ids,
                                  const uint32_t* rect, uint32_t* rect_sorted, uint32_t* block_sums, unsigned long long* super, uint32_t* superexcl,
                                  uint32_t tile_part, unsigned long long* total_dev, unsigned long long capacity, int stage ,
                                  int tiles_x, uint32_t* inst_tile, uint32_t* inst_splat, int key16) {
    if (n <= 0 || V <= 0) return hipSuccess;
    const uint32_t nbv = (uint32_t)((n + FE_BLOCK - 1) / FE_BLOCK), nsb = (nbv + 255u) / 256u;
    const dim3 grid(((nbv + 1u) / 2u) * (uint32_t)V), grid3(((nbv + 3u) / 4u) * (uint32_t)V), blk(FE_BLOCK);
    if (stage == 0) {
#define FE_A3(F) hipLaunchKernelGGL(k_seg_blocksum<F>, grid3, blk, 0, st, n, V, nbv, nsb, seg_vis, sorted_ids, (const FeRect<F>::T*)rect, (FeRect<F>::T*)rect_sorted, block_sums, super)
        if (rect_fmt == DVS_FE_RECT_U8) FE_A3(DVS_FE_RECT_U8); else if (rect_fmt == DVS_FE_RECT_U16) FE_A3(DVS_FE_RECT_U16); else FE_A3(DVS_FE_RECT_TIGHT);
#undef FE_A3
        hipLaunchKernelGGL(k_seg_totals, dim3(1), dim3(1024), 0, st, V, nsb, (const unsigned long long*)super, superexcl, seg_tile, tile_part, total_dev, capacity);
    } else {
#define FE_A4(F) hipLaunchKernelGGL(k_seg_duplicate<F>, grid, blk, 0, st, n, V, nbv, nsb, seg_vis, (const DvsSeg*)seg_tile, sorted_ids, (const FeRect<F>::T*)rect_sorted, \
                                    (const uint32_t*)block_sums, (const uint32_t*)superexcl, tiles_x, inst_tile, inst_splat, capacity, key16)
        if (rect_fmt == DVS_FE_RECT_U8) FE_A4(DVS_FE_RECT_U8); else if (rect_fmt == DVS_FE_RECT_U16) FE_A4(DVS_FE_RECT_U16); else FE_A4(DVS_FE_RECT_TIGHT);
#undef FE_A4
    }
    return hipGetLastError();
}
void dvs_fe_block_counts(int n, uint32_t* nbv, uint32_t* nsb) { *nbv = (uint32_t)((n + FE_BLOCK - 1) / FE_BLOCK); *nsb = (*nbv + 255u) / 256u; }

__global__ void k_seg_init(int n, int V, uint32_t rows_per_view, DvsSeg* __restrict__ seg_all) {
    const int v = threadIdx.x;
    if (v < V) { DvsSeg s; s.base = (uint32_t)v * (uint32_t)n; s.count = (uint32_t)n; s.pstart = (uint32_t)v * rows_per_view; s.sub = 0; s.bits = 8; s._r0 = s._r1 = s._r2 = 0; seg_all[v] = s; }
}
hipError_t dvs_launch_seg_init(hipStream_t st, int n, int V, uint32_t rows_per_view, DvsSeg* seg_all) {
    hipLaunchKernelGGL(k_seg_init, dim3(1), dim3(64), 0, st, n, V, rows_per_view, seg_all);
    return hipGetLastError();
}

__global__ void __launch_bounds__(FE_BLOCK)
k_tile_ranges(uint64_t T_host, const uint64_t* __restrict__ T_dev, const uint32_t* __restrict__ sorted_tile, uint2* __restrict__ ranges) {
    const uint64_t T = T_dev ? (*T_dev < T_host ? *T_dev : T_host) : T_host;
    for (uint64_t q = (uint64_t)blockIdx.x * FE_BLOCK + threadIdx.x; q * 4 < T; q += (uint64_t)gridDim.x * FE_BLOCK) {
        const uint64_t j0 = q * 4;
        uint32_t t[6];
        if (j0 + 4 <= T) {
            const uint4 v = reinterpret_cast<const uint4*>(sorted_tile)[q];
            t[1] = v.x; t[2] = v.y; t[3] = v.z; t[4] = v.w;
        } else {
#pragma unroll
            for (int k = 0; k < 4; ++k) t[1 + k] = j0 + k < T ? sorted_tile[j0 + k] : 0xFFFFFFFFu;
        }
        t[0] = j0 > 0 ? sorted_tile[j0 - 1] : 0xFFFFFFFFu;
        t[5] = j0 + 4 < T ? sorted_tile[j0 + 4] : 0xFFFFFFFFu;
#pragma unroll
        for (int k = 0; k < 4; ++k) {
            const uint64_t j = j0 + k;
            if (j < T) {
                if (j == 0 || t[k] != t[k + 1]) ranges[t[k + 1]].x = (uint32_t)j;
                if (j + 1 == T || t[k + 2] != t[k + 1]) ranges[t[k + 1]].y = (uint32_t)(j + 1);
            }
        }
    }
}

hipError_t dvs_launch_tile_ranges(hipStream_t st, uint64_t T, const uint32_t* sorted_tile, uint32_t* ranges, const uint64_t* T_dev,
                                  uint64_t T_expected) {
    if (T == 0) return hipSuccess;
    const uint64_t T_grid = (T_dev && T_expected > 0 && T_expected < T) ? T_expected : T;
    const uint32_t nb = (uint32_t)((T_grid + 4 * FE_BLOCK - 1) / (4 * FE_BLOCK));
    hipLaunchKernelGGL(k_tile_ranges, dim3(nb), dim3(FE_BLOCK), 0, st, T, T_dev, sorted_tile, (uint2*)ranges);
    return hipGetLastError();
}

__global__ void __launch_bounds__(FE_BLOCK)
k_export_keys(uint64_t T, const uint32_t* __restrict__ sorted_tile, const uint32_t* __restrict__ sorted_splat,
              const float* __restrict__ depth, uint64_t* __restrict__ out) {
    const uint64_t j = (uint64_t)blockIdx.x * FE_BLOCK + threadIdx.x;
    if (j >= T) return;
    out[j] = ((uint64_t)sorted_tile[j] << 32) | (uint64_t)__float_as_uint(depth[sorted_splat[j]]);
}

hipError_t dvs_launch_export_keys(hipStream_t st, uint64_t T, const uint32_t* sorted_tile, const uint32_t* sorted_splat,
                                  const float* depth, uint64_t* out_keys) {
    if (T == 0) return hipSuccess;
    const uint32_t nb = (uint32_t)((T + FE_BLOCK - 1) / FE_BLOCK);
    hipLaunchKernelGGL(k_export_keys, dim3(nb), dim3(FE_BLOCK), 0, st, T, sorted_tile, sorted_splat, depth, out_keys);
    return hipGetLastError();
}
```

### divshot_amd/csrc/render.hip

```cpp
#include "dvs_device.h"
#include "dvs_kernels.h"
#include "render_common.h"

struct __attribute__((aligned(16))) FwdLds {
    float4 a[RB];
    float4 b[RB];
    float4 c[RB];
    uint64_t qmask[RB / 64][4];
    uint32_t wlive[RB / 64];
};
__device__ __forceinline__ void lds_put(FwdLds& L, int t, float2 xy, float4 co, float3 col) {
    L.a[t] = make_float4(xy.x, xy.y, -0.72134752044448170f * co.x, -1.4426950408889634f * co.y);
    L.b[t] = make_float4(-0.72134752044448170f * co.z, co.w, col.x, col.y);
    L.c[t].x = col.z;
}

__device__ __forceinline__ bool stage_batch(FwdLds& L, const uint32_t* __restrict__ sorted_splat, uint32_t first, int cnt,
                                            const float4* __restrict__ splat2d, float tile_x0, float tile_y0, uint32_t& id_out) {
    const int t = threadIdx.x;
    uint32_t qm = 0;
    id_out = 0u;
    if (t < cnt) {
        const uint32_t id = sorted_splat[first + t];
        id_out = id;
        const float4 r0 = splat2d[4 * (size_t)id], r1 = splat2d[4 * (size_t)id + 1];
        const float4 r2 = splat2d[4 * (size_t)id + 2], r3 = splat2d[4 * (size_t)id + 3];
        const float bl = r2.x;
        const float2 xy = make_float2(r0.x, r0.y);
        const float4 co = make_float4(r0.z, r0.w, r1.x, r1.y);
        const float3 col = make_float3(r1.z, r1.w, bl);
        lds_put(L, t, xy, co, col);
        const float bound = r2.w;
        const float a = co.x, c = co.z;
        const float det_c = r3.x, det_a = r3.y, nb_c = r3.z, nb_a = r3.w;
        const float ox = tile_x0 - xy.x, oy = tile_y0 - xy.y;
        float vy[2], vbase[2], hx[2], hbase[2];
        bool vin[2], hin[2];
#pragma unroll
        for (int i = 0; i < 2; ++i) {
            const float x0 = ox + 8.f * (float)i, x1 = x0 + 7.f, y0 = oy + 8.f * (float)i, y1 = y0 + 7.f;
            vin[i] = x0 <= 0.f && x1 >= 0.f; hin[i] = y0 <= 0.f && y1 >= 0.f;
            const float xe = x0 > 0.f ? x0 : x1, ye = y0 > 0.f ? y0 : y1;
            vy[i] = nb_c * xe; vbase[i] = vin[i] ? __builtin_inff() : xe * xe * det_c;
            hx[i] = nb_a * ye; hbase[i] = hin[i] ? __builtin_inff() : ye * ye * det_a;
        }
#pragma unroll
        for (int q = 0; q < 4; ++q) {
            const int col = q & 1, row = q >> 1;
            const float x0 = ox + 8.f * (float)col, x1 = x0 + 7.f, y0 = oy + 8.f * (float)row, y1 = y0 + 7.f;
            const float ty_ = fminf(fmaxf(vy[col], y0), y1) - vy[col], tx_ = fminf(fmaxf(hx[row], x0), x1) - hx[row];
            const float ev = __builtin_fmaf(c * ty_, ty_, vbase[col]), eh = __builtin_fmaf(a * tx_, tx_, hbase[row]);
            const float qmn = (vin[col] && hin[row]) ? 0.f : fminf(ev, eh);
            qm |= !(qmn > bound) ? (1u << q) : 0u;
        }
    }
    const uint64_t m0 = __ballot(qm & 1u), m1 = __ballot(qm & 2u), m2 = __ballot(qm & 4u), m3 = __ballot(qm & 8u);
    if ((t & 63) == 0) {
        uint64_t* dst = L.qmask[t >> 6];
        dst[0] = m0; dst[1] = m1; dst[2] = m2; dst[3] = m3;
    }
    return qm != 0u;
}

__device__ __forceinline__ uint64_t uniform_u64(uint64_t v) {
    const uint32_t lo = __builtin_amdgcn_readfirstlane((uint32_t)v), hi = __builtin_amdgcn_readfirstlane((uint32_t)(v >> 32));
    return ((uint64_t)hi << 32) | lo;
}

template <bool RECORD>
__global__ void __launch_bounds__(RB)
k_render_fwd(ViewBg bg_arg , int W, int H, int tiles_x, int tiles_per_view,
             int num_tiles , const uint2* __restrict__ ranges, uint2* __restrict__ ranges_out ,
             const uint32_t* __restrict__ sorted_splat, const float4* __restrict__ splat2d,
             float* __restrict__ out_color , float* __restrict__ final_T , uint32_t* __restrict__ n_contrib,
             uint32_t* __restrict__ live_splat ,
             uint32_t* __restrict__ live_pos ,
             uint64_t* __restrict__ take_masks , uint64_t take_cap) {
    __shared__ FwdLds L;
    (void)bg_arg;
    const int tile_g = tile_of_block(blockIdx.x, num_tiles);
    if (tile_g >= num_tiles) return;
    const int view = tile_g / tiles_per_view, tile = tile_g - view * tiles_per_view;
    const float3 bgv = dvs_load_bg(view);
    const float bg0 = bgv.x, bg1 = bgv.y, bg2 = bgv.z;
    out_color += (size_t)view * 3 * W * H; final_T += (size_t)view * W * H; n_contrib += (size_t)view * W * H;
    const int tx = tile % tiles_x, ty = tile / tiles_x;
    const int wave = threadIdx.x >> 6, lane = threadIdx.x & 63;
    const int px = tx * DVS_TILE + (wave & 1) * 8 + (lane & 7);
    const int py = ty * DVS_TILE + (wave >> 1) * 8 + (lane >> 3);
    const bool inside = px < W && py < H;
    const float pxf = (float)px, pyf = (float)py;
    uint2 range = ranges[tile_g];
    if (ranges_out) {
        range.x = range.y ? ~range.x : 0u;
        if (threadIdx.x == 0) ranges_out[tile_g] = range;
    }
    const int total = (int)(range.y - range.x);
    uint64_t notdone = __builtin_amdgcn_ballot_w64(inside);
    float T = 1.0f, C0 = 0.f, C1 = 0.f, C2 = 0.f;
    uint32_t last = 0;
    uint32_t live_base = 0;

    for (int base = 0; base < total; base += RB) {
        if (__syncthreads_and(notdone == 0ull)) break;
        const int cnt = min(RB, total - base);
        uint32_t my_id;
        const bool live = stage_batch(L, sorted_splat, range.x + base, cnt, splat2d, (float)(tx * DVS_TILE), (float)(ty * DVS_TILE), my_id);
        const uint64_t lm = __ballot(live);
        const uint32_t lrank = __builtin_amdgcn_mbcnt_hi((uint32_t)(lm >> 32), __builtin_amdgcn_mbcnt_lo((uint32_t)lm, 0u));
        if (lane == 0) L.wlive[wave] = (uint32_t)__popcll(lm);
        __syncthreads();
        if (live_pos) {
            uint32_t pre = 0, tot = 0;
#pragma unroll
            for (int w = 0; w < RB / 64; ++w) { const uint32_t c = L.wlive[w]; pre += w < wave ? c : 0u; tot += c; }
            const uint32_t lp = live_base + pre + lrank;
            if ((int)threadIdx.x < cnt) live_pos[range.x + base + threadIdx.x] = lp;
            if (live) live_splat[range.x + lp] = my_id;
            live_base += tot;
        }
        if (notdone == 0ull) continue;
#pragma unroll 1
        for (int lw = 0; lw < RB / 64; ++lw) {
            uint64_t m = uniform_u64(L.qmask[lw][wave]);
            if (m == 0) continue;
            if (notdone == 0ull) break;
            typedef float fwd_v4f __attribute__((ext_vector_type(4)));
            typedef __attribute__((address_space(3))) const fwd_v4f lds_cv4f;
            uint32_t word_a = (uint32_t)(uintptr_t)&L.a[lw * 64];
            asm("" : "+v"(word_a));
            const int idx0 = base + lw * 64 + 1;
            uint64_t exec_entry;
            asm volatile("s_mov_b64 %0, exec" : "=s"(exec_entry));
            while (m) {
                const int bit = __builtin_ctzll(m);
                asm("s_bitset0_b64 %0, %1" : "+s"(m) : "s"(bit));
                uint32_t ent_a;
                asm("v_lshl_add_u32 %0, %1, 4, %2" : "=v"(ent_a) : "s"(bit), "v"(word_a));
                const fwd_v4f A = *(lds_cv4f*)ent_a;
                const fwd_v4f B = *(lds_cv4f*)(ent_a + (uint32_t)sizeof(L.a));
                const float cb = *(const __attribute__((address_space(3))) float*)(ent_a + (uint32_t)(sizeof(L.a) + sizeof(L.b)));
                const float dx = A.x - pxf, dy = A.y - pyf;
                const float p2 = __builtin_fmaf(B.x * dy, dy, __builtin_fmaf(A.w, dy, A.z * dx) * dx);
                const float alpha = fminf(DVS_ALPHA_MAX, B.y * __builtin_amdgcn_exp2f(p2));
                const float aT = alpha * T;
                const float test_T = T - aT;
                const uint64_t nd_before = notdone;
                const uint32_t idx = (uint32_t)(idx0 + bit);
                asm volatile("s_mov_b64 exec, %[nd]\n\t"
                             "v_cmpx_nlt_f32_e32 vcc, 0, %[p2]\n\t"
                             "v_cmpx_ngt_f32_e32 vcc, %[amin], %[al]\n\t"
                             "v_cmp_gt_f32_e32 vcc, %[tstop], %[tt]\n\t"
                             "s_andn2_b64 %[nd], %[nd], vcc\n\t"
                             "s_andn2_b64 exec, exec, vcc\n\t"
                             "v_fmac_f32 %[c0], %[cr], %[at]\n\t"
                             "v_fmac_f32 %[c1], %[cg], %[at]\n\t"
                             "v_fmac_f32 %[c2], %[cbl], %[at]\n\t"
                             "v_sub_f32 %[T], %[T], %[at]\n\t"
                             "v_mov_b32 %[last], %[idx]\n\t"
                             "s_mov_b64 exec, %[ee]"
                             : [c0] "+v"(C0), [c1] "+v"(C1), [c2] "+v"(C2), [T] "+v"(T), [last] "+v"(last), [nd] "+s"(notdone)
                             : [p2] "v"(p2), [al] "v"(alpha), [tt] "v"(test_T), [cr] "v"(B.z), [cg] "v"(B.w), [cbl] "v"(cb), [at] "v"(aT), [idx] "s"(idx),
                               [amin] "s"(DVS_ALPHA_MIN), [tstop] "s"(DVS_T_STOP), [ee] "s"(exec_entry)
                             : "vcc", "scc");
                if (RECORD) {
                    const uint64_t took = nd_before & __builtin_amdgcn_ballot_w64(!(p2 > 0.f)) & __builtin_amdgcn_ballot_w64(!(alpha < DVS_ALPHA_MIN)) &
                                          ~__builtin_amdgcn_ballot_w64(test_T < DVS_T_STOP);
                    const uint64_t pos = (uint64_t)range.x + (uint64_t)(idx - 1u);
                    if (lane == 0 && pos < take_cap) take_masks[pos * 4 + wave] = took;
                }
            }
        }
    }
    if (inside) {
        const size_t P = (size_t)W * H, pix = (size_t)py * W + px;
        final_T[pix] = T;
        n_contrib[pix] = last;
        out_color[pix] = C0 + T * bg0;
        out_color[P + pix] = C1 + T * bg1;
        out_color[2 * P + pix] = C2 + T * bg2;
    }
}


hipError_t dvs_launch_render_fwd(hipStream_t st, int W, int H, int tiles_x, int tiles_y, int n_views, const uint32_t* ranges,
                                 const uint32_t* sorted_splat, const float* splat2d, const float* bgs, float* out_color, float* final_T,
                                 uint32_t* n_contrib, uint32_t* live_splat, uint32_t* live_pos, uint64_t* take_masks, uint64_t take_cap, uint32_t* ranges_out) {
    const int tiles_pv = tiles_x * tiles_y, num_tiles = tiles_pv * n_views;
    if (num_tiles <= 0) return hipSuccess;
    const int grid = ((num_tiles + 7) >> 3) << 3;
    if (take_masks)
        hipLaunchKernelGGL(k_render_fwd<true>, dim3(grid), dim3(RB), 0, st, make_view_bg(n_views, bgs), W, H, tiles_x, tiles_pv, num_tiles,
                           (const uint2*)ranges, (uint2*)ranges_out, sorted_splat, (const float4*)splat2d, out_color, final_T, n_contrib, live_splat, live_pos, take_masks, take_cap);
    else
        hipLaunchKernelGGL(k_render_fwd<false>, dim3(grid), dim3(RB), 0, st, make_view_bg(n_views, bgs), W, H, tiles_x, tiles_pv, num_tiles,
                           (const uint2*)ranges, (uint2*)ranges_out, sorted_splat, (const float4*)splat2d, out_color, final_T, n_contrib, live_splat, live_pos, (uint64_t*)nullptr, (uint64_t)0);
    return hipGetLastError();
}
```

### divshot_amd/csrc/render_blocks.hip

```cpp
#include "dvs_device.h"
#include "dvs_kernels.h"
#include "render_common.h"

#define BK_RB 64
#define BK_SW (BK_RB / 64)

struct __attribute__((aligned(16))) BlockLds {
    float4 xyc[BK_RB];
    float4 zoir[BK_RB];
    float4 cog[BK_RB];
    uint32_t id[BK_RB];
    uint8_t list[16][BK_RB];
    uint32_t cnt[16];
    uint32_t wcnt[BK_SW][16];
};

__device__ __forceinline__ void stage_blocks(BlockLds& L, const uint32_t* __restrict__ sorted_splat, uint32_t first, int cnt, int base,
                                             const float4* __restrict__ splat2d, float tile_x0, float tile_y0, const uint32_t* blast) {
    constexpr int GPT = 16 * BK_RB / RB, ROWS = GPT / 4;
    const int t = threadIdx.x, e = t % BK_RB, sub = t / BK_RB, lane = t & 63, ws = e >> 6;
    const bool stager = t < RB;
    uint32_t hits = 0;
    if (stager && e < cnt) {
        const uint32_t id = sorted_splat[first + e];
        const float4 r0 = splat2d[4 * (size_t)id], r1 = splat2d[4 * (size_t)id + 1];
        const float bl = splat2d[4 * (size_t)id + 2].x;
        const float a = r0.z, b = r0.w, c = r1.x, op = r1.y;
        if (sub == 0) {
            L.xyc[e] = make_float4(r0.x, r0.y, -0.72134752044448170f * a, -1.4426950408889634f * b);
            L.zoir[e] = make_float4(-0.72134752044448170f * c, op, bl, r1.z);
            L.cog[e] = make_float4(a, b, c, r1.w);
            L.id[e] = id;
        }
        const float bound = 1.3862943611f * __builtin_amdgcn_logf(255.0f * op) * 1.0001f + 1e-3f;
        const float det = fmaxf(0.f, __builtin_fmaf(-2.4e-7f, a * c, a * c - b * b));
        const float rc = __builtin_amdgcn_rcpf(c), ra = __builtin_amdgcn_rcpf(a);
        const float det_c = det * rc, det_a = det * ra, nb_c = -b * rc, nb_a = -b * ra;
        const float ox = tile_x0 - r0.x, oy = tile_y0 - r0.y;
        float vy[4], vbase[4], hx[ROWS], hbase[ROWS];
        bool vin[4], hin[ROWS];
        const float oyr = oy + (float)(4 * ROWS * sub);
#pragma unroll
        for (int i = 0; i < 4; ++i) {
            const float x0 = ox + 4.f * (float)i, x1 = x0 + 3.f;
            vin[i] = x0 <= 0.f && x1 >= 0.f;
            const float xe = x0 > 0.f ? x0 : x1;
            vy[i] = nb_c * xe; vbase[i] = vin[i] ? __builtin_inff() : xe * xe * det_c;
        }
#pragma unroll
        for (int r = 0; r < ROWS; ++r) {
            const float y0 = oyr + 4.f * (float)r, y1 = y0 + 3.f;
            hin[r] = y0 <= 0.f && y1 >= 0.f;
            const float ye = y0 > 0.f ? y0 : y1;
            hx[r] = nb_a * ye; hbase[r] = hin[r] ? __builtin_inff() : ye * ye * det_a;
        }
#pragma unroll
        for (int i = 0; i < GPT; ++i) {
            const int col = i & 3, r = i >> 2;
            const float x0 = ox + 4.f * (float)col, x1 = x0 + 3.f, y0 = oyr + 4.f * (float)r, y1 = y0 + 3.f;
            const float ty_ = fminf(fmaxf(vy[col], y0), y1) - vy[col], tx_ = fminf(fmaxf(hx[r], x0), x1) - hx[r];
            const float ev = __builtin_fmaf(c * ty_, ty_, vbase[col]), eh = __builtin_fmaf(a * tx_, tx_, hbase[r]);
            const float qm = (vin[col] && hin[r]) ? 0.f : fminf(ev, eh);
            bool h = !(qm > bound);
            h = h && ((uint32_t)(base + e) < blast[GPT * sub + i]);
            hits |= h ? (1u << i) : 0u;
        }
    }
    uint32_t rank[GPT];
    if (stager) {
#pragma unroll
        for (int i = 0; i < GPT; ++i) {
            const uint64_t m = __ballot((hits >> i) & 1u);
            rank[i] = __builtin_amdgcn_mbcnt_hi((uint32_t)(m >> 32), __builtin_amdgcn_mbcnt_lo((uint32_t)m, 0u));
            if (lane == 0) L.wcnt[ws][GPT * sub + i] = (uint32_t)__popcll(m);
        }
    }
    __syncthreads();
    if (stager) {
#pragma unroll
        for (int i = 0; i < GPT; ++i) {
            const int g = GPT * sub + i;
            uint32_t off = 0, tot = 0;
#pragma unroll
            for (int w = 0; w < BK_SW; ++w) { const uint32_t v = L.wcnt[w][g]; if (w < ws) off += v; tot += v; }
            if ((hits >> i) & 1u) L.list[g][off + rank[i]] = (uint8_t)e;
            if (e == 0) L.cnt[g] = tot;
        }
    }
}

__device__ __forceinline__ void lane_pixel(int wave, int lane, int& block, int& lx, int& ly) {
    const int gl = lane & 3, i = lane >> 2;
    const int bx = 2 * (wave & 1) + (gl & 1), by = 2 * (wave >> 1) + (gl >> 1);
    block = by * 4 + bx;
    lx = 4 * bx + (i & 3);
    ly = 4 * by + (i >> 2);
}
__device__ __forceinline__ int wave_max4(int v) {
    const int a = __builtin_amdgcn_readlane(v, 0), b = __builtin_amdgcn_readlane(v, 1), c = __builtin_amdgcn_readlane(v, 2),
              d = __builtin_amdgcn_readlane(v, 3);
    return max(max(a, b), max(c, d));
}

template <int NV>
__device__ __forceinline__ void group_reduce12(const float v[12], float q[3], int xaddr) {
    const float h0 = swap32_add(v[0], v[1]), h1 = swap32_add(v[2], v[3]), h2 = swap32_add(v[4], v[5]);
    const float h3 = swap32_add(v[6], v[7]);
    float h4, h5;
    if (NV == 11) {
        h4 = swap32_add(v[8], v[9]);
        h5 = v[10] + __int_as_float(__builtin_amdgcn_ds_bpermute(xaddr, __float_as_int(v[10])));
    } else {
        h4 = v[8] + __int_as_float(__builtin_amdgcn_ds_bpermute(xaddr, __float_as_int(v[8])));
        h5 = 0.f;
    }
    float r[3] = {swap16_add(h0, h1), swap16_add(h2, h3), swap16_add(h4, h5)};
#pragma unroll
    for (int k = 0; k < 3; ++k) {
        float x = r[k];
        x += __int_as_float(__builtin_amdgcn_ds_swizzle(__float_as_int(x), (4 << 10) | 0x1f));
        x += __int_as_float(__builtin_amdgcn_ds_swizzle(__float_as_int(x), (8 << 10) | 0x1f));
        q[k] = x;
    }
}

template <bool ABSGRAD>
__global__ void __launch_bounds__(RB) __attribute__((amdgpu_waves_per_eu(8, 8)))
k_render_bwd_blocks(ViewBg bg_arg , int W, int H, int tiles_x, int tiles_per_view,
                    int num_tiles , const uint2* __restrict__ ranges,
                    const uint32_t* __restrict__ sorted_splat, const float4* __restrict__ splat2d,
                    const float* __restrict__ final_T, const uint32_t* __restrict__ n_contrib, const float* __restrict__ dL_dout ,
                    float* __restrict__ grow , int lineage) {
    __shared__ BlockLds L;
    __shared__ float s_tab[4][BK_RB * 12];
    __shared__ uint32_t s_blast[16];
    (void)bg_arg;
    const int tile_g = tile_of_block(blockIdx.x, num_tiles);
    if (tile_g >= num_tiles) return;
    const int view = tile_g / tiles_per_view, tile = tile_g - view * tiles_per_view;
    const float3 bgv = dvs_load_bg(view);
    final_T += (size_t)view * W * H; n_contrib += (size_t)view * W * H; dL_dout += (size_t)view * 3 * W * H;
    const int tx = tile % tiles_x, ty = tile / tiles_x;
    const int wave = threadIdx.x >> 6, lane = threadIdx.x & 63;
    int block, lx, ly;
    lane_pixel(wave, lane, block, lx, ly);
    const int px = tx * DVS_TILE + lx, py = ty * DVS_TILE + ly;
    const bool inside = px < W && py < H;
    const float pxf = (float)px, pyf = (float)py;
    const uint2 range = ranges[tile_g];
    const size_t P = (size_t)W * H, pix = (size_t)py * W + px;
    const int lrow = lane >> 4, lsel = (lane & 15) >> 2;
    const int kv = lsel * 4 + ((lrow == 1) ? 2 : (lrow == 2) ? 1 : lrow);
    const bool publisher = lsel < 3 && kv < (ABSGRAD ? 11 : 9);
    const int xaddr = (lane ^ 32) << 2;
    const int mygroup = lane & 3;
    float* const tab = &s_tab[wave][kv];

    const float T_final = inside ? final_T[pix] : 0.f;
    const uint32_t last = inside ? n_contrib[pix] : 0u;
    float dLp0 = 0.f, dLp1 = 0.f, dLp2 = 0.f;
    if (inside) { dLp0 = dL_dout[pix]; dLp1 = dL_dout[P + pix]; dLp2 = dL_dout[2 * P + pix]; }
    const float bg_dot = (bgv.x * dLp0 + bgv.y * dLp1) + bgv.z * dLp2;

    uint32_t bmax = last;
#pragma unroll
    for (int d = 32; d >= 4; d >>= 1) bmax = max(bmax, (uint32_t)__shfl_xor((int)bmax, d, 64));
    if (lane < 4) s_blast[block] = bmax;
    for (int e = threadIdx.x; e < 4 * BK_RB * 12; e += RB) (&s_tab[0][0])[e] = 0.f;
    __syncthreads();
    uint32_t todo = 0;
#pragma unroll
    for (int g = 0; g < 16; ++g) todo = max(todo, s_blast[g]);
    if (todo == 0) return;

    float T = T_final;
    float D = T_final * bg_dot;
    const uint8_t* lp = &L.list[block][0];
    const int nbatch = (int)((todo + BK_RB - 1) / BK_RB);
    for (int b = nbatch - 1; b >= 0; --b) {
        const int base = b * BK_RB;
        const int cnt = min(BK_RB, (int)todo - base);
        __syncthreads();
        stage_blocks(L, sorted_splat, range.x + base, cnt, base, splat2d, (float)(tx * DVS_TILE), (float)(ty * DVS_TILE), s_blast);
        __syncthreads();
        const int len = (int)L.cnt[block];
        const int nmax = __builtin_amdgcn_readfirstlane(wave_max4(len));
        const int lastb = (int)min(last, (uint32_t)(base + BK_RB)) - base;
        int idx = len - 1;
        int jn = idx >= 0 ? (int)lp[idx] : 0;
#pragma unroll 1
        for (int it = 0; it < nmax; ++it, --idx) {
            const bool act = idx >= 0;
            const int j = jn;
            jn = idx >= 1 ? (int)lp[idx - 1] : 0;
            const float4 xy = L.xyc[j];
            const float4 zo4 = L.zoir[j];
            const float2 zo2 = make_float2(zo4.x, zo4.y);
            const float dx = xy.x - pxf, dy = xy.y - pyf;
            const float p2 = __builtin_fmaf(zo2.x * dy, dy, __builtin_fmaf(xy.w, dy, xy.z * dx) * dx);
            const float G = __builtin_amdgcn_exp2f(p2);
            const float oa = zo2.y * G;
            const float alpha = fminf(DVS_ALPHA_MAX, oa);
            const bool contrib = act && (j < lastb) && !(p2 > 0.f) && !(alpha < DVS_ALPHA_MIN);
            if (__builtin_amdgcn_ballot_w64(contrib) == 0) continue;
            const float4 cg = L.cog[j];
            const float3 c = make_float3(zo4.w, cg.w, zo4.z);
            const float al = contrib ? alpha : 0.f;
            const float inv_1ma = __builtin_amdgcn_rcpf(1.f - al);
            T = T * inv_1ma;
            const float w = al * T;
            const float cd = (c.x * dLp0 + c.y * dLp1) + c.z * dLp2;
            float dL_dalpha = cd * T - D * inv_1ma;
            D = D + cd * w;
            const bool capped = !lineage && (oa > DVS_ALPHA_MAX);
            dL_dalpha = (contrib && !capped) ? dL_dalpha : 0.f;
            const float v5 = G * dL_dalpha;
            const float sw = zo2.y * v5;
            const float su = sw * dx, st = sw * dy;
            float v[12];
            v[0] = su; v[1] = st;
            v[2] = su * dx; v[3] = su * dy; v[4] = st * dy;
            v[5] = v5;
            v[6] = w * dLp0; v[7] = w * dLp1; v[8] = w * dLp2;
            v[9] = ABSGRAD ? fabsf(__builtin_fmaf(cg.x, su, cg.y * st)) : 0.f;
            v[10] = ABSGRAD ? fabsf(__builtin_fmaf(cg.z, st, cg.y * su)) : 0.f;
            v[11] = 0.f;
            float q[3];
            group_reduce12<ABSGRAD ? 11 : 9>(v, q, xaddr);
            const float val = lsel == 0 ? q[0] : (lsel == 1 ? q[1] : q[2]);
            float* const slot = reinterpret_cast<float*>(reinterpret_cast<char*>(tab) + __umul24((unsigned)j, 48u));
            const bool pub = publisher && act;
#pragma unroll
            for (int g = 0; g < 4; ++g) {
                if (pub && mygroup == g) *slot += val;
                __builtin_amdgcn_wave_barrier();
                asm volatile("" ::: "memory");
            }
        }
        __syncthreads();
        for (int e = threadIdx.x; e < cnt * 12; e += RB) {
            const float val = (s_tab[0][e] + s_tab[1][e]) + (s_tab[2][e] + s_tab[3][e]);
            if (val != 0.f) {
                const int ent = e / 12, comp = e - 12 * ent;
                atomicAdd(&grow[(size_t)L.id[ent] * 12 + comp], val);
            }
            s_tab[0][e] = 0.f; s_tab[1][e] = 0.f; s_tab[2][e] = 0.f; s_tab[3][e] = 0.f;
        }
    }
}

hipError_t dvs_launch_render_bwd_blocks(hipStream_t st, int W, int H, int tiles_x, int tiles_y, int n_views, const uint32_t* ranges,
                                        const uint32_t* sorted_splat, const float* splat2d, const float* bgs, const float* final_T,
                                        const uint32_t* n_contrib, const float* dL_dout, float* grad_rows, int absgrad, int grad_mode) {
    const int tiles_pv = tiles_x * tiles_y, num_tiles = tiles_pv * n_views;
    if (num_tiles <= 0) return hipSuccess;
    const int grid = ((num_tiles + 7) >> 3) << 3;
    const int lineage = grad_mode == 1 ? 1 : 0;
#define DVS_RBB(KERNEL)                                                                                                     \
    hipLaunchKernelGGL(KERNEL, dim3(grid), dim3(RB), 0, st, make_view_bg(n_views, bgs), W, H, tiles_x, tiles_pv, num_tiles, \
                       (const uint2*)ranges, sorted_splat, (const float4*)splat2d, final_T, n_contrib, dL_dout, grad_rows, lineage)
    if (absgrad) DVS_RBB(k_render_bwd_blocks<true>); else DVS_RBB(k_render_bwd_blocks<false>);
#undef DVS_RBB
    return hipGetLastError();
}
```

### divshot_amd/csrc/render_common.h

```cpp
#pragma once
#include "dvs_device.h"

#define RB 256

struct ViewBg { float bg[DVS_MAX_VIEWS][4]; };
__device__ __forceinline__ float3 dvs_load_bg(int v) {
    typedef const __attribute__((address_space(4))) float* KF;
    const KF f = (KF)__builtin_amdgcn_kernarg_segment_ptr() + (size_t)v * 4;
    return make_float3(f[0], f[1], f[2]);
}

static inline ViewBg make_view_bg(int n_views, const float* bgs ) {
    ViewBg b{};
    for (int v = 0; v < n_views && v < DVS_MAX_VIEWS; ++v) for (int k = 0; k < 3; ++k) b.bg[v][k] = bgs[3 * v + k];
    return b;
}

__device__ __forceinline__ int tile_of_block(int b, int num_tiles) {
    const int chunk = (num_tiles + 7) >> 3;
    return (b & 7) * chunk + (b >> 3);
}

__device__ __forceinline__ float swap32_add(float a, float b) {
    const auto r = __builtin_amdgcn_permlane32_swap(__float_as_uint(a), __float_as_uint(b), false, false);
    return __uint_as_float(r[0]) + __uint_as_float(r[1]);
}
__device__ __forceinline__ float swap16_add(float a, float b) {
    const auto r = __builtin_amdgcn_permlane16_swap(__float_as_uint(a), __float_as_uint(b), false, false);
    return __uint_as_float(r[0]) + __uint_as_float(r[1]);
}
```

### divshot_amd/csrc/render_tr.hip

```cpp
#include "dvs_device.h"
#include "dvs_kernels.h"
#include "render_common.h"

#define TR_SLOTS 4
#define TR_SS 136
#define TR_MINW 6

template <int BK>
struct __attribute__((aligned(16))) TrLds {
    float4 ea[BK + 1];
    float4 eb[BK + 1];
    float4 ec[BK + 1];
    uint2 idop[2][BK];
    uint8_t list[(BK + 1) * 16];
    uint32_t cnt[16];
    uint32_t blast[16];
};

template <int BK>
__device__ __forceinline__ uint32_t tr_load_id(const uint32_t* __restrict__ sorted_splat, uint32_t first, int cnt) {
    const int e = threadIdx.x % BK;
    return e < cnt ? sorted_splat[first + e] : 0u;
}
template <int BK>
__device__ __forceinline__ void tr_stage(TrLds<BK>& L, const float4* __restrict__ splat2d, uint32_t id, int cnt, int base, int parity,
                                         float tile_x0, float tile_y0) {
    constexpr int GPT = 16 * BK / RB;
    static_assert(GPT == 4 || GPT == 2, "BK must be 64 or 32");
    const int t = threadIdx.x, e = t % BK, sub = t / BK, lane = t & 63;
    const int b0 = GPT * sub, row = b0 >> 2, col0 = b0 & 3;
    uint32_t hits = 0;
    if (e < cnt) {
        const float4 r0 = splat2d[4 * (size_t)id], r1 = splat2d[4 * (size_t)id + 1], r2 = splat2d[4 * (size_t)id + 2], r3 = splat2d[4 * (size_t)id + 3];
        const float a = r0.z, b = r0.w, c = r1.x, op = r1.y;
        if (sub == 0) {
            L.ea[e] = make_float4(r0.x, r0.y, -0.72134752044448170f * a, -1.4426950408889634f * b);
            L.eb[e] = make_float4(-0.72134752044448170f * c, op, r1.z, r1.w);
            L.ec[e] = make_float4(r2.x, a, b, c);
            L.idop[parity][e] = make_uint2(id, __float_as_uint(op));
        }
        const float bound = r2.w, det_c = r3.x, det_a = r3.y, nb_c = r3.z, nb_a = r3.w;
        const float ox = tile_x0 - r0.x + 4.f * (float)col0, oy = tile_y0 - r0.y + 4.f * (float)row;
        const float y0 = oy, y1 = oy + 3.f;
        const bool hin = y0 <= 0.f && y1 >= 0.f;
        const float ye = y0 > 0.f ? y0 : y1;
        const float hx = nb_a * ye, hbase = hin ? __builtin_inff() : ye * ye * det_a;
#pragma unroll
        for (int i = 0; i < GPT; ++i) {
            const float x0 = ox + 4.f * (float)i, x1 = x0 + 3.f;
            const bool vin = x0 <= 0.f && x1 >= 0.f;
            const float xe = x0 > 0.f ? x0 : x1;
            const float vy = nb_c * xe, vbase = vin ? __builtin_inff() : xe * xe * det_c;
            const float ty_ = fminf(fmaxf(vy, y0), y1) - vy, tx_ = fminf(fmaxf(hx, x0), x1) - hx;
            const float ev = __builtin_fmaf(c * ty_, ty_, vbase), eh = __builtin_fmaf(a * tx_, tx_, hbase);
            const float qm = (vin && hin) ? 0.f : fminf(ev, eh);
            bool h = !(qm > bound);
            h = h && ((uint32_t)(base + e) < L.blast[b0 + i]);
            hits |= h ? (1u << i) : 0u;
        }
    }
#pragma unroll
    for (int i = 0; i < GPT; ++i) {
        const bool hit = (hits & (1u << i)) != 0u;
        const uint64_t m = __ballot(hit);
        uint32_t rk, len;
        if (BK == 64) {
            rk = __builtin_amdgcn_mbcnt_hi((uint32_t)(m >> 32), __builtin_amdgcn_mbcnt_lo((uint32_t)m, 0u));
            len = (uint32_t)__popcll(m);
        } else {
            const uint32_t lo = (uint32_t)m, hi = (uint32_t)(m >> 32);
            const bool up = lane >= 32;
            rk = up ? __builtin_amdgcn_mbcnt_hi(hi, 0u) : __builtin_amdgcn_mbcnt_lo(lo, 0u);
            len = (uint32_t)__popc(up ? hi : lo);
        }
        if (hit) L.list[(rk + 1u) * 16u + (uint32_t)(b0 + i)] = (uint8_t)e;
        if (e == 0) L.cnt[b0 + i] = len;
    }
}

template <bool ABSGRAD, bool LINEAGE, int BK>
__global__ void __launch_bounds__(RB, TR_MINW)
k_render_bwd_tr(ViewBg bg_arg , int W, int H, int tiles_x, int tiles_per_view,
                int num_tiles , const uint2* __restrict__ ranges,
                const uint32_t* __restrict__ sorted_splat, const float4* __restrict__ splat2d,
                const float* __restrict__ final_T, const uint32_t* __restrict__ n_contrib, const float* __restrict__ dL_dout ,
                float* __restrict__ grow ,
                const uint32_t* __restrict__ live_splat ,
                const uint32_t* __restrict__ live_pos ) {
    __shared__ TrLds<BK> L;
    __shared__ __attribute__((aligned(16))) float s_tab[4][(BK + 1) * 12];
    __shared__ __attribute__((aligned(16))) float s_tb[4][TR_SLOTS * TR_SS];
    (void)bg_arg;
    const int tile_g = tile_of_block(blockIdx.x, num_tiles);
    if (tile_g >= num_tiles) return;
    const int view = tile_g / tiles_per_view, tile = tile_g - view * tiles_per_view;
    const float3 bgv = dvs_load_bg(view);
    final_T += (size_t)view * W * H; n_contrib += (size_t)view * W * H; dL_dout += (size_t)view * 3 * W * H;
    const int tx = tile % tiles_x, ty = tile / tiles_x;
    const int wave = threadIdx.x >> 6, lane = threadIdx.x & 63;
    const size_t P = (size_t)W * H;
    const int g1 = lane >> 4, pi = lane & 15;
    const int bx1 = 2 * (wave & 1) + (g1 & 1), by1 = 2 * (wave >> 1) + (g1 >> 1), blk1 = by1 * 4 + bx1;
    const int px = tx * DVS_TILE + 4 * bx1 + (pi & 3), py = ty * DVS_TILE + 4 * by1 + (pi >> 2);
    const bool inside = px < W && py < H;
    const size_t pix = (size_t)py * W + px;
    const float pxf = (float)px, pyf = (float)py;
    const uint2 range = ranges[tile_g];
    const int r2 = lane >> 4, s2 = (lane >> 2) & 3, g2 = lane & 3;
    const int bx2 = 2 * (wave & 1) + (g2 & 1), by2 = 2 * (wave >> 1) + (g2 >> 1);
    const int X0 = tx * DVS_TILE + 4 * bx2, Y0 = ty * DVS_TILE + 4 * by2 + r2;
    const float X0f = (float)X0, Y0f = (float)Y0;
    float d2[4][3];
    if ((W & 3) == 0) {
        const bool in2 = X0 < W && Y0 < H;
        const size_t q = (size_t)Y0 * W + X0;
#pragma unroll
        for (int c = 0; c < 3; ++c) {
            const float4 v = in2 ? *reinterpret_cast<const float4*>(dL_dout + c * P + q) : make_float4(0.f, 0.f, 0.f, 0.f);
            d2[0][c] = v.x; d2[1][c] = v.y; d2[2][c] = v.z; d2[3][c] = v.w;
        }
    } else {
#pragma unroll
        for (int x = 0; x < 4; ++x) {
            const bool in2 = X0 + x < W && Y0 < H;
            const size_t q = (size_t)Y0 * W + X0 + x;
#pragma unroll
            for (int c = 0; c < 3; ++c) d2[x][c] = in2 ? dL_dout[c * P + q] : 0.f;
        }
    }
    const int perm_r = (r2 == 1) ? 2 : (r2 == 2) ? 1 : r2;
    const int xaddr = (lane ^ 32) << 2;
    const int jaddr = (16 * g2) << 2;
    const uint32_t jshift = 8u * (uint32_t)(TR_SLOTS - 1 - s2);

    const float T_final = inside ? final_T[pix] : 0.f;
    uint32_t last = inside ? n_contrib[pix] : 0u;
    if (live_pos) {
        if (last > 0u) last = live_pos[range.x + last - 1u] + 1u;
        sorted_splat = live_splat;
    }
    float dLp0 = 0.f, dLp1 = 0.f, dLp2 = 0.f;
    if (inside) { dLp0 = dL_dout[pix]; dLp1 = dL_dout[P + pix]; dLp2 = dL_dout[2 * P + pix]; }
    const float bg_dot = (bgv.x * dLp0 + bgv.y * dLp1) + bgv.z * dLp2;

    uint32_t bmax = last;
#pragma unroll
    for (int d = 8; d >= 1; d >>= 1) bmax = max(bmax, (uint32_t)__shfl_xor((int)bmax, d, 64));
    if (pi == 0) L.blast[blk1] = bmax;
    for (int e = threadIdx.x; e < (BK + 1) * 12; e += RB) reinterpret_cast<float4*>(&s_tab[0][0])[e] = make_float4(0.f, 0.f, 0.f, 0.f);
    if (threadIdx.x < 16) L.list[threadIdx.x] = (uint8_t)BK;
    if (threadIdx.x == 0) { L.ea[BK] = make_float4(0.f, 0.f, 0.f, 0.f); L.eb[BK] = make_float4(0.f, 0.f, 0.f, 0.f); L.ec[BK] = make_float4(0.f, 0.f, 0.f, 0.f); }
    __syncthreads();
    uint32_t todo = 0;
#pragma unroll
    for (int g = 0; g < 16; ++g) todo = max(todo, L.blast[g]);
    if (todo == 0) return;

    float T = T_final;
    float D = T_final * bg_dot;
    const uint32_t tb_m0 = (uint32_t)__builtin_amdgcn_readfirstlane((int)(uint32_t)(uintptr_t)&s_tb[wave][0]);
    typedef __attribute__((address_space(3))) float lds_float;
    typedef float tr_v4f __attribute__((ext_vector_type(4)));
    typedef __attribute__((address_space(3))) const tr_v4f lds_cv4f;
    uint32_t tbr_a = (uint32_t)(uintptr_t)&s_tb[wave][TR_SS * s2 + 16 * g2 + 4 * r2];
    uint32_t tabw_a = (uint32_t)(uintptr_t)&s_tab[wave][perm_r];
    asm("" : "+v"(tbr_a), "+v"(tabw_a));
    const uint8_t* const lbase = &L.list[0];

    auto flush = [&](uint32_t jpack) {
        const uint32_t jp = (uint32_t)__builtin_amdgcn_ds_bpermute(jaddr, (int)jpack);
        const int j = (int)((jp >> jshift) & 0xffu);
        const tr_v4f V_ = *(lds_cv4f*)tbr_a, W_ = *(lds_cv4f*)(tbr_a + 256u);
        const float4 V = make_float4(V_.x, V_.y, V_.z, V_.w), Wv = make_float4(W_.x, W_.y, W_.z, W_.w);
        const float2 mean = *reinterpret_cast<const float2*>(&L.ea[j]);
        const float4 cq = L.ec[j];
        asm("" : : "v"(cq.x));
        const float Dx = mean.x - X0f, Dy = mean.y - Y0f;
        const float A0 = (V.x + V.y) + (V.z + V.w);
        const float B0 = __builtin_fmaf(3.f, V.w, __builtin_fmaf(2.f, V.z, V.y));
        const float C0 = __builtin_fmaf(9.f, V.w, __builtin_fmaf(4.f, V.z, V.y));
        float v[12];
        v[0] = __builtin_fmaf(Dx, A0, -B0);
        v[1] = Dy * A0;
        v[2] = __builtin_fmaf(Dx, v[0], -__builtin_fmaf(Dx, B0, -C0));
        v[3] = Dy * v[0];
        v[4] = Dy * v[1];
        v[5] = A0;
#pragma unroll
        for (int c = 0; c < 3; ++c)
            v[6 + c] = __builtin_fmaf(Wv.w, d2[3][c], __builtin_fmaf(Wv.z, d2[2][c], __builtin_fmaf(Wv.y, d2[1][c], Wv.x * d2[0][c])));
        if (ABSGRAD) {
            const float gx0 = __builtin_fmaf(cq.y, Dx, cq.z * Dy), gy0 = __builtin_fmaf(cq.z, Dx, cq.w * Dy);
            const float gx1 = gx0 - cq.y, gx2 = gx1 - cq.y, gx3 = gx2 - cq.y;
            const float gy1 = gy0 - cq.z, gy2 = gy1 - cq.z, gy3 = gy2 - cq.z;
            v[9] = __builtin_fmaf(fabsf(V.w), fabsf(gx3), __builtin_fmaf(fabsf(V.z), fabsf(gx2), __builtin_fmaf(fabsf(V.y), fabsf(gx1), fabsf(V.x) * fabsf(gx0))));
            v[10] = __builtin_fmaf(fabsf(V.w), fabsf(gy3), __builtin_fmaf(fabsf(V.z), fabsf(gy2), __builtin_fmaf(fabsf(V.y), fabsf(gy1), fabsf(V.x) * fabsf(gy0))));
        } else { v[9] = 0.f; v[10] = 0.f; }
        v[11] = 0.f;
        const float h0 = swap32_add(v[0], v[1]), h1 = swap32_add(v[2], v[3]), h2 = swap32_add(v[4], v[5]);
        const float h3 = swap32_add(v[6], v[7]);
        float h4, h5;
        if (ABSGRAD) {
            h4 = swap32_add(v[8], v[9]);
            h5 = v[10] + __int_as_float(__builtin_amdgcn_ds_bpermute(xaddr, __float_as_int(v[10])));
        } else {
            h4 = v[8] + __int_as_float(__builtin_amdgcn_ds_bpermute(xaddr, __float_as_int(v[8])));
            h5 = 0.f;
        }
        const float q0 = swap16_add(h0, h1), q1 = swap16_add(h2, h3), q2 = swap16_add(h4, h5);
        uint32_t slot_a;
        asm("v_mad_u32_u24 %0, %1, 48, %2" : "=v"(slot_a) : "v"(j), "v"(tabw_a));
        lds_float* const slot = (lds_float*)slot_a;
#pragma unroll
        for (int g = 0; g < 4; ++g) {
            if (g2 == g) { slot[0] += q0; slot[4] += q1; slot[8] += q2; }
            __builtin_amdgcn_wave_barrier();
            asm volatile("" ::: "memory");
        }
    };

    const int nbatch = (int)((todo + BK - 1) / BK);
    const float tile_x0 = (float)(tx * DVS_TILE), tile_y0 = (float)(ty * DVS_TILE);
    uint32_t id_stage = tr_load_id<BK>(sorted_splat, range.x + (nbatch - 1) * BK, min(BK, (int)todo - (nbatch - 1) * BK));
    for (int b = nbatch - 1; b >= 0; --b) {
        const int base = b * BK;
        const int cnt = min(BK, (int)todo - base);
        tr_stage<BK>(L, splat2d, id_stage, cnt, base, b & 1, tile_x0, tile_y0);
        __syncthreads();
        const int len = (int)L.cnt[blk1];
        int nmax = len;
        nmax = max(nmax, __shfl_xor(nmax, 16, 64));
        nmax = max(nmax, __shfl_xor(nmax, 32, 64));
        nmax = __builtin_amdgcn_readfirstlane(nmax);
        const int lastb = (int)min(last, (uint32_t)(base + BK)) - base;
        uint32_t p = (uint32_t)len * 16u + (uint32_t)blk1;
        uint32_t jn = lbase[p];
        asm("" : "+v"(jn));
        uint32_t jpack = 0;
        int nslot = 0;
#pragma unroll 1
        for (int it = 0; it < nmax; ++it) {
            const int j = (int)jn;
            jpack = (jpack << 8) | (uint32_t)j;
            const bool below_last = j < lastb;
            const float4 ea = L.ea[j];
            const float4 eb = L.eb[j];
            p = __builtin_elementwise_sub_sat(p, 16u);
            jn = lbase[p];
            asm("" : "+v"(jn));
            const float dx = ea.x - pxf, dy = ea.y - pyf;
            const float p2 = __builtin_fmaf(eb.x * dy, dy, __builtin_fmaf(ea.w, dy, ea.z * dx) * dx);
            const float G = __builtin_amdgcn_exp2f(p2);
            const float oa = eb.y * G;
            const float alpha = fminf(DVS_ALPHA_MAX, oa);
            const bool contrib = below_last && !(p2 > 0.f) && !(alpha < DVS_ALPHA_MIN);
            const float2 rg = make_float2(eb.z, eb.w);
            const float cb = L.ec[j].x;
            const float al = contrib ? alpha : 0.f;
            const float inv_1ma = __builtin_amdgcn_rcpf(1.f - al);
            T = T * inv_1ma;
            const float w = al * T;
            const float cd = (rg.x * dLp0 + rg.y * dLp1) + cb * dLp2;
            const float dL_dalpha = cd * T - D * inv_1ma;
            D = D + cd * w;
            const bool gate = LINEAGE ? contrib : (contrib && !(oa > DVS_ALPHA_MAX));
            const float v5 = gate ? G * dL_dalpha : 0.f;
            asm volatile("s_mov_b32 m0, %2\n\ts_nop 0\n\tds_write_addtid_b32 %0 offset:0\n\tds_write_addtid_b32 %1 offset:256"
                         : : "v"(v5), "v"(w), "s"(tb_m0 + (uint32_t)(TR_SS * 4) * (uint32_t)nslot) : "memory", "m0");
            if (++nslot == TR_SLOTS) { flush(jpack); nslot = 0; }
        }
        if (nslot > 0) {
            for (; nslot < TR_SLOTS; ++nslot) {
                float* const tbw = &s_tb[wave][lane];
                tbw[TR_SS * nslot] = 0.f; tbw[TR_SS * nslot + 64] = 0.f;
                jpack = (jpack << 8) | (uint32_t)BK;
            }
            flush(jpack);
        }
        __syncthreads();
        if (b > 0) id_stage = tr_load_id<BK>(sorted_splat, range.x + (b - 1) * BK, BK);
        for (int e = threadIdx.x; e < cnt * 12; e += RB) {
            const float val = (s_tab[0][e] + s_tab[1][e]) + (s_tab[2][e] + s_tab[3][e]);
            if (val != 0.f) {
                const int ent = e / 12, comp = e - 12 * ent;
                const uint2 io = L.idop[b & 1][ent];
                const float sc = (comp == 5 || (comp >= 6 && comp <= 8)) ? 1.f : __uint_as_float(io.y);
                if (comp < 11) atomicAdd(&grow[(size_t)io.x * 12 + comp], val * sc);
            }
            s_tab[0][e] = 0.f; s_tab[1][e] = 0.f; s_tab[2][e] = 0.f; s_tab[3][e] = 0.f;
        }
    }
}

hipError_t dvs_launch_render_bwd_tr(hipStream_t st, int W, int H, int tiles_x, int tiles_y, int n_views, const uint32_t* ranges,
                                    const uint32_t* sorted_splat, const float* splat2d, const float* bgs, const float* final_T,
                                    const uint32_t* n_contrib, const float* dL_dout, float* grad_rows, int absgrad, int grad_mode,
                                    const uint32_t* live_splat, const uint32_t* live_pos) {
    const int tiles_pv = tiles_x * tiles_y, num_tiles = tiles_pv * n_views;
    if (num_tiles <= 0) return hipSuccess;
    const int grid = ((num_tiles + 7) >> 3) << 3;
    const int lineage = grad_mode == 1 ? 1 : 0;
#define DVS_TR(A, LN, BKV)                                                                                                              \
    hipLaunchKernelGGL((k_render_bwd_tr<A, LN, BKV>), dim3(grid), dim3(RB), 0, st, make_view_bg(n_views, bgs), W, H, tiles_x, tiles_pv, \
                       num_tiles, (const uint2*)ranges, sorted_splat, (const float4*)splat2d, final_T, n_contrib, dL_dout, grad_rows, live_splat, live_pos)
#define DVS_TR_B(BKV)                                                                                   \
    do {                                                                                                \
        if (absgrad) { if (lineage) DVS_TR(true, true, BKV); else DVS_TR(true, false, BKV); }           \
        else { if (lineage) DVS_TR(false, true, BKV); else DVS_TR(false, false, BKV); }                 \
    } while (0)
    DVS_TR_B(64);
#undef DVS_TR_B
#undef DVS_TR
    return hipGetLastError();
}
```

### divshot_amd/raster.py

```python
import ctypes as C
import numpy as np
import torch
from ._lib import lib, Splats, Camera, Opts, FwdState, SplatGrads, check, DvsError

PARAM_KEYS = ("pos", "sh0", "shN", "opacity", "scale", "rot")
PARAM_WIDTH = {"pos": 3, "sh0": 3, "shN": 45, "opacity": 1, "scale": 3, "rot": 4}


def tiled_floats(n):
    return ((n + 63) // 64) * 64 * 48


def shn_rows_to_tiled_np(a):
    n = a.shape[0]
    nt = (n + 63) // 64
    pad = np.zeros((nt * 64, 48), a.dtype)
    pad[:n, :45] = a.reshape(n, 45)
    return np.ascontiguousarray(pad.reshape(nt, 64, 12, 4).transpose(0, 2, 1, 3)).reshape(-1)


def shn_tiled_to_rows_np(t, n):
    nt = (n + 63) // 64
    rows = np.ascontiguousarray(np.asarray(t).reshape(nt, 12, 64, 4).transpose(0, 2, 1, 3)).reshape(nt * 64, 48)
    return rows[:n, :45].reshape(n, 15, 3)


def _stream_ptr():
    return C.c_void_p(torch.cuda.current_stream().cuda_stream)


class Rasterizer:
    def __init__(self, device=0, max_splats=1 << 20, max_w=1920, max_h=1080, max_views=1):
        if not torch.cuda.is_available():
            raise DvsError("no HIP device visible: the rasterizer has no CPU fallback")
        self.device = device
        self.tdev = torch.device("cuda", device)
        self.max_views = max_views
        self.ctx = lib.dvs_create_views(device, max_splats, max_w, max_h, max_views)
        if not self.ctx:
            raise DvsError("dvs_create failed: " + lib.dvs_last_error().decode())
        self.state = None
        self._cam = None
        self._opts = None
        self._params = None

    def close(self):
        if self.ctx:
            lib.dvs_destroy(self.ctx)
            self.ctx = None

    def __del__(self):
        try:
            self.close()
        except Exception:
            pass

    def _splats(self, params, tiled=False):
        n = params["pos"].shape[0]
        for k in PARAM_KEYS:
            t = params[k]
            assert t.is_cuda and t.dtype == torch.float32 and t.is_contiguous(), k
            want = tiled_floats(n) if (tiled and k == "shN") else n * PARAM_WIDTH[k]
            assert t.numel() == want, (k, t.numel(), want)
        return Splats(*[params[k].data_ptr() for k in PARAM_KEYS], n, 0)

    def shn_relayout(self, src, n, to_tiled):
        dst = torch.zeros(tiled_floats(n) if to_tiled else n * 45, dtype=torch.float32, device=self.tdev)
        with torch.cuda.device(self.tdev):
            check(lib.dvs_shn_relayout(self.ctx, _stream_ptr(), n, src.data_ptr(), dst.data_ptr(), 1 if to_tiled else 0), "dvs_shn_relayout")
        return dst if to_tiled else dst.view(n, 15, 3)

    def keep_intermediates(self, on=True):
        check(lib.dvs_keep_bwd_intermediates(self.ctx, 1 if on else 0))

    def set_async(self, on=True):
        check(lib.dvs_set_async(self.ctx, 1 if on else 0), "dvs_set_async")

    def get_num_rendered(self):
        T = C.c_uint64(0)
        with torch.cuda.device(self.tdev):
            check(lib.dvs_get_num_rendered(self.ctx, _stream_ptr(), C.byref(T)), "dvs_get_num_rendered")
        self.num_rendered = int(T.value)
        if self.state is not None:
            self.state.num_rendered = self.num_rendered
        return self.num_rendered

    def set_backward_variant(self, variant):
        v = {"blocks": 0, "reduce": 1, "mm": 2, "tr": 3}.get(variant, variant)
        check(lib.dvs_set_backward_variant(self.ctx, int(v)), "dvs_set_backward_variant")

    def set_forward_variant(self, variant):
        v = {"blocks": 0, "quadrant": 1}.get(variant, variant)
        check(lib.dvs_set_forward_variant(self.ctx, int(v)), "dvs_set_forward_variant")

    def set_live_lists(self, on=True):
        check(lib.dvs_set_live_lists(self.ctx, 1 if on else 0), "dvs_set_live_lists")

    def record_decisions(self, capacity_instances):
        if not capacity_instances:
            check(lib.dvs_debug_record_decisions(self.ctx, None, 0), "dvs_debug_record_decisions")
            self._rec = None
            return None
        self._rec = torch.zeros((int(capacity_instances), 4), dtype=torch.int64, device=self.tdev)
        check(lib.dvs_debug_record_decisions(self.ctx, self._rec.data_ptr(), int(capacity_instances)), "dvs_debug_record_decisions")
        return self._rec

    def enable_timing(self, on=True):
        check(lib.dvs_enable_stage_timing(self.ctx, 1 if on else 0))

    def kernel_probe(self, on=True):
        check(lib.dvs_enable_kernel_probe(self.ctx, 1 if on else 0))

    def read_kernel_probe(self):
        ms, cnt = (C.c_float * 2)(), (C.c_int * 2)()
        check(lib.dvs_read_kernel_probe(self.ctx, ms, cnt), "dvs_read_kernel_probe")
        return {"render_fwd": (float(ms[0]), int(cnt[0])), "render_bwd": (float(ms[1]), int(cnt[1]))}

    def stage_timing(self):
        names = C.POINTER(C.c_char_p)()
        ms = C.POINTER(C.c_float)()
        k = lib.dvs_get_stage_timing(self.ctx, C.byref(names), C.byref(ms))
        return {names[i].decode(): float(ms[i]) for i in range(k)}

    def forward(self, params, cam, sh_degree=3, antialias=False, absgrad=False, out=None, shn_tiled=False, grad_mode=0, tight_tiles=False):
        sp = self._splats(params, shn_tiled)
        opts = Opts(sh_degree, int(antialias), int(absgrad), 0, int(shn_tiled), int(grad_mode), int(bool(tight_tiles)))
        self._tiled = bool(shn_tiled)
        if out is None:
            out = torch.empty((3, cam.height, cam.width), dtype=torch.float32, device=self.tdev)
        st = FwdState()
        T = C.c_uint64(0)
        with torch.cuda.device(self.tdev):
            check(lib.dvs_raster_forward(self.ctx, _stream_ptr(), C.byref(sp), C.byref(cam), C.byref(opts),
                                         out.data_ptr(), C.byref(st), C.byref(T)), "dvs_raster_forward")
        self.state, self._cam, self._opts, self._params = st, cam, opts, params
        self._cams = None
        self.num_rendered = int(T.value)
        return out

    def forward_views(self, params, cams, sh_degree=3, antialias=False, absgrad=False, out=None, shn_tiled=False, grad_mode=0, tight_tiles=False):
        V = len(cams)
        sp = self._splats(params, shn_tiled)
        opts = Opts(sh_degree, int(antialias), int(absgrad), 0, int(shn_tiled), int(grad_mode), int(bool(tight_tiles)))
        self._tiled = bool(shn_tiled)
        if out is None:
            out = torch.empty((V, 3, cams[0].height, cams[0].width), dtype=torch.float32, device=self.tdev)
        carr = (Camera * V)(*cams)
        with torch.cuda.device(self.tdev):
            check(lib.dvs_raster_forward_views(self.ctx, _stream_ptr(), C.byref(sp), carr, V, C.byref(opts), out.data_ptr()), "dvs_raster_forward_views")
        st = FwdState()
        check(lib.dvs_get_view_state(self.ctx, 0, C.byref(st)), "dvs_get_view_state")
        self.state, self._cam, self._cams, self._opts, self._params = st, cams[0], carr, opts, params
        self.num_rendered = int(st.num_rendered)
        return out

    def backward_views(self, dL_drgb, grads=None, accumulate=False, want_mean2d=False, factorised_sh=False):
        V = len(self._cams)
        n = self._params["pos"].shape[0]
        if factorised_sh and (grads is None or "dcolor" not in grads):
            grads = dict(grads or {}); grads["dcolor"] = torch.empty((V, n, 3), dtype=torch.float32, device=self.tdev)
        had = grads is not None and any(k in grads for k in PARAM_KEYS)
        if not had:
            base = {k: (torch.zeros_like(self._params[k]) if (k == "shN" and self._tiled) else torch.empty_like(self._params[k])) for k in PARAM_KEYS}
            base.update(grads or {}); grads = base; accumulate = False
        grads, opts, g = self._grad_args(grads, accumulate, want_mean2d, factorised_sh)
        sp = self._splats(self._params, self._tiled)
        assert dL_drgb.is_cuda and dL_drgb.dtype == torch.float32 and dL_drgb.is_contiguous() and dL_drgb.shape[0] == V
        with torch.cuda.device(self.tdev):
            check(lib.dvs_raster_backward_views(self.ctx, _stream_ptr(), C.byref(sp), self._cams, V, C.byref(opts), dL_drgb.data_ptr(), C.byref(g)),
                  "dvs_raster_backward_views")
        return grads

    def view_saved(self, v):
        st = FwdState()
        check(lib.dvs_get_view_state(self.ctx, v, C.byref(st)), "dvs_get_view_state")
        if self.state.num_rendered == 2 ** 64 - 1:
            self.get_num_rendered()
        n, W, H, tiles = st.n, st.width, st.height, st.tiles_x * st.tiles_y
        T = self.state.num_rendered
        rec = self._d2h(st.splat2d, (n, 16), np.float32)
        ranges = self._d2h(st.ranges, (tiles, 2), np.uint32).astype(np.int64)
        st0 = FwdState()
        check(lib.dvs_get_view_state(self.ctx, 0, C.byref(st0)), "dvs_get_view_state")
        all_tile = self._sorted_tile(st0, T, tiles * len(self._cams)); all_splat = self._d2h(st.sorted_splat, (T,), np.uint32)
        nz = ranges[:, 1] > ranges[:, 0]
        lo = int(ranges[nz, 0].min()) if nz.any() else 0
        hi = int(ranges[nz, 1].max()) if nz.any() else 0
        loc = ranges.copy(); loc[nz] -= lo; loc[~nz] = 0
        return {"radii": self._d2h(st.radii, (n,), np.int32), "mean2d": rec[:, 0:2].copy(), "depth": self._d2h(st.depth, (n,), np.float32),
                "conic_opacity": rec[:, 2:6].copy(), "rgb": rec[:, 6:9].copy(), "flags": self._d2h(st.flags, (n,), np.uint32),
                "tiles_touched": self._d2h(st.tiles_touched, (n,), np.uint32),
                "sorted_tile": all_tile[lo:hi] - np.uint32(v * tiles), "vals": all_splat[lo:hi] - np.uint32(v * n),
                "ranges": loc.astype(np.uint32), "final_T": self._d2h(st.final_T, (H, W), np.float32),
                "n_contrib": self._d2h(st.n_contrib, (H, W), np.uint32)}

    def _grad_args(self, grads, accumulate, want_mean2d, factorised_sh):
        params = self._params
        n = params["pos"].shape[0]
        if grads is None:
            grads = {k: (torch.zeros_like(params[k]) if (k == "shN" and self._tiled) else torch.empty_like(params[k])) for k in PARAM_KEYS}
            accumulate = False
        opts = Opts(self._opts.sh_degree, self._opts.antialias, self._opts.absgrad, int(accumulate), self._opts.shn_layout, self._opts.grad_mode,
                    self._opts.tile_bounds)
        if self._opts.absgrad and "absgrad2d" not in grads:
            grads["absgrad2d"] = torch.empty((n, 2), dtype=torch.float32, device=self.tdev)
        if want_mean2d and "mean2d" not in grads:
            grads["mean2d"] = torch.empty((n, 2), dtype=torch.float32, device=self.tdev)
        if factorised_sh and "dcolor" not in grads:
            grads["dcolor"] = torch.empty((n, 3), dtype=torch.float32, device=self.tdev)

        def ptr(k):
            if factorised_sh and k in ("sh0", "shN"):
                return None
            return grads[k].data_ptr()
        g = SplatGrads(*[ptr(k) for k in PARAM_KEYS],
                       grads["absgrad2d"].data_ptr() if "absgrad2d" in grads else None,
                       grads["mean2d"].data_ptr() if "mean2d" in grads else None,
                       grads["dcolor"].data_ptr() if factorised_sh else None)
        return grads, opts, g

    def backward(self, dL_drgb, grads=None, accumulate=False, want_mean2d=False, factorised_sh=False):
        assert self.state is not None, "forward first"
        grads, opts, g = self._grad_args(grads, accumulate, want_mean2d, factorised_sh)
        sp = self._splats(self._params, self._tiled)
        assert dL_drgb.is_cuda and dL_drgb.dtype == torch.float32 and dL_drgb.is_contiguous()
        with torch.cuda.device(self.tdev):
            check(lib.dvs_raster_backward(self.ctx, _stream_ptr(), C.byref(sp), C.byref(self._cam), C.byref(opts),
                                          dL_drgb.data_ptr(), C.byref(g)), "dvs_raster_backward")
        return grads

    def backward_composite(self, dL_drgb):
        assert self.state is not None, "forward first"
        assert dL_drgb.is_cuda and dL_drgb.dtype == torch.float32 and dL_drgb.is_contiguous()
        cam_arg = self._cams if getattr(self, "_cams", None) is not None else C.byref(self._cam)
        with torch.cuda.device(self.tdev):
            check(lib.dvs_raster_backward_composite(self.ctx, _stream_ptr(), cam_arg, C.byref(self._opts), dL_drgb.data_ptr()),
                  "dvs_raster_backward_composite")

    def backward_dcolor(self, dcolor):
        assert dcolor.is_cuda and dcolor.dtype == torch.float32 and dcolor.is_contiguous()
        with torch.cuda.device(self.tdev):
            check(lib.dvs_raster_backward_dcolor(self.ctx, _stream_ptr(), dcolor.data_ptr()), "dvs_raster_backward_dcolor")
        return dcolor

    def backward_project(self, grads=None, accumulate=False, want_mean2d=False, factorised_sh=False):
        grads, opts, g = self._grad_args(grads, accumulate, want_mean2d, factorised_sh)
        sp = self._splats(self._params, self._tiled)
        cam_arg = self._cams if getattr(self, "_cams", None) is not None else C.byref(self._cam)
        with torch.cuda.device(self.tdev):
            check(lib.dvs_raster_backward_project(self.ctx, _stream_ptr(), C.byref(sp), cam_arg, C.byref(opts), C.byref(g)),
                  "dvs_raster_backward_project")
        return grads

    def backward_project_chunks(self, grads, chunks, after_chunk, accumulate=False, want_mean2d=False):
        grads, opts, g = self._grad_args(grads, accumulate, want_mean2d, True)
        sp = self._splats(self._params, self._tiled)
        cam_arg = self._cams if getattr(self, "_cams", None) is not None else C.byref(self._cam)
        with torch.cuda.device(self.tdev):
            for k, (first, count) in enumerate(chunks):
                check(lib.dvs_raster_backward_project_chunk(self.ctx, _stream_ptr(), C.byref(sp), cam_arg, C.byref(opts), C.byref(g),
                                                            int(first), int(count)), "dvs_raster_backward_project_chunk")
                if after_chunk is not None:
                    after_chunk(k, first, count)
        return grads

    def sh_grad_combine(self, pos, campos, dcolor_all, g_sh0, g_shN, sh_degree, accumulate=False, shn_tiled=False):
        campos = np.ascontiguousarray(campos, np.float32)
        V, n = dcolor_all.shape[0], pos.shape[0]
        assert campos.shape == (V, 3) and dcolor_all.is_contiguous() and dcolor_all.shape == (V, n, 3)
        with torch.cuda.device(self.tdev):
            check(lib.dvs_sh_grad_combine(self.ctx, _stream_ptr(), n, pos.data_ptr(), sh_degree, V, campos.ctypes.data,
                                          dcolor_all.data_ptr(), g_sh0.data_ptr(), g_shN.data_ptr(), int(accumulate), int(shn_tiled)),
                  "dvs_sh_grad_combine")

    def _sorted_tile(self, st, T, total_tiles):
        if st.sorted_tile:
            return self._d2h(st.sorted_tile, (T,), np.uint32)
        rg = self._d2h(st.ranges, (total_tiles, 2), np.uint32).astype(np.int64)
        out = np.repeat(np.arange(total_tiles, dtype=np.uint32), (rg[:, 1] - rg[:, 0]))
        assert out.size == T, (out.size, T)
        return out

    def _d2h(self, ptr, shape, dtype):
        a = np.empty(shape, dtype)
        if a.nbytes:
            check(lib.dvs_memcpy_d2h(self.ctx, a.ctypes.data, C.c_void_p(ptr), a.nbytes), "dvs_memcpy_d2h")
        return a

    def saved(self):
        s = self.state
        if s.num_rendered == 2 ** 64 - 1:
            self.get_num_rendered()
        n, T, W, H = s.n, s.num_rendered, s.width, s.height
        tiles = s.tiles_x * s.tiles_y
        rec = self._d2h(s.splat2d, (n, 16), np.float32)
        return {
            "radii": self._d2h(s.radii, (n,), np.int32), "mean2d": rec[:, 0:2].copy(),
            "depth": self._d2h(s.depth, (n,), np.float32), "conic_opacity": rec[:, 2:6].copy(),
            "rgb": rec[:, 6:9].copy(), "splat2d": rec, "flags": self._d2h(s.flags, (n,), np.uint32),
            "tiles_touched": self._d2h(s.tiles_touched, (n,), np.uint32),
            "sorted_tile": self._sorted_tile(s, T, tiles), "vals": self._d2h(s.sorted_splat, (T,), np.uint32),
            "ranges": self._d2h(s.ranges, (tiles, 2), np.uint32), "final_T": self._d2h(s.final_T, (H, W), np.float32),
            "n_contrib": self._d2h(s.n_contrib, (H, W), np.uint32),
        }

    def sorted_keys(self):
        if self.state.num_rendered == 2 ** 64 - 1:
            self.get_num_rendered()
        T = self.state.num_rendered
        buf = torch.empty((max(T, 1),), dtype=torch.int64, device=self.tdev)
        check(lib.dvs_export_sorted_keys(self.ctx, _stream_ptr(), buf.data_ptr()), "dvs_export_sorted_keys")
        torch.cuda.synchronize(self.tdev)
        return buf[:T].cpu().numpy().view(np.uint64)

    def bwd_intermediates(self):
        rows, width = C.c_void_p(), C.c_int(0)
        check(lib.dvs_get_bwd_intermediates(self.ctx, C.byref(rows), C.byref(width)))
        n = self.state.n
        r = self._d2h(rows.value, (n, width.value), np.float32).astype(np.float64)
        rec = self._d2h(self.state.splat2d, (n, 16), np.float32).astype(np.float64)
        a, b, c = rec[:, 2], rec[:, 3], rec[:, 4]
        dmean = np.stack([-(a * r[:, 0] + b * r[:, 1]), -(c * r[:, 1] + b * r[:, 0])], 1)
        dconic = np.stack([-0.5 * r[:, 2], -r[:, 3], -0.5 * r[:, 4], r[:, 5]], 1)
        return {"dL_dmean2d": dmean.astype(np.float32), "dL_dconic_opacity": dconic.astype(np.float32),
                "dL_drgb": r[:, 6:9].astype(np.float32), "absgrad": r[:, 9:11].astype(np.float32)}

    def sort_pairs(self, keys, vals, bit_lo=0, bit_hi=32):
        assert keys.is_cuda and vals.is_cuda and keys.numel() == vals.numel()
        check(lib.dvs_sort_pairs_u32(self.ctx, _stream_ptr(), keys.data_ptr(), vals.data_ptr(), keys.numel(), bit_lo, bit_hi),
              "dvs_sort_pairs_u32")


def params_to_device(params_np, device):
    return {k: torch.from_numpy(np.ascontiguousarray(v)).to(device) for k, v in params_np.items()}
```

### include/dvs_raster.h

```cpp
#ifndef DVS_RASTER_H
#define DVS_RASTER_H

#include <stddef.h>
#include <stdint.h>

#ifdef __cplusplus
extern "C" {
#endif

#define DVS_TILE 16
#define DVS_SH_REST 15

enum {
    DVS_OK = 0,
    DVS_ERR_INVALID = 1,
    DVS_ERR_HIP = 2,
    DVS_ERR_CAPACITY = 3,
    DVS_ERR_STATE = 4,
    DVS_ERR_UNSUPPORTED = 5
};

typedef struct dvs_splats {
    const float* pos;
    const float* sh0;
    const float* shN;
    const float* opacity;
    const float* scale;
    const float* rot;
    int32_t n;
    int32_t _pad;
} dvs_splats;

typedef struct dvs_camera {
    float view[16];
    float proj[16];
    float tan_fovx, tan_fovy;
    float focal_x, focal_y;
    float campos[3];
    int32_t width, height;
    float bg[3];
} dvs_camera;

enum {
    DVS_SHN_ROWS = 0,
    DVS_SHN_TILED = 1
};
#define DVS_SHN_TILE_FLOATS 3072

typedef struct dvs_opts {
    int32_t sh_degree;
    int32_t antialias;
    int32_t absgrad;
    int32_t accumulate;
    int32_t shn_layout;
    int32_t grad_mode;
    int32_t tile_bounds;
    int32_t _reserved[1];
} dvs_opts;

enum { DVS_TILES_CANONICAL = 0, DVS_TILES_TIGHT = 1 };

enum { DVS_GRAD_TRUE = 0, DVS_GRAD_LINEAGE = 1 };

enum { DVS_S2D_X = 0, DVS_S2D_Y = 1, DVS_S2D_CONIC = 2, DVS_S2D_OPACITY = 5, DVS_S2D_RGB = 6, DVS_S2D_DEPTH = 9, DVS_S2D_RADIUS = 10,
       DVS_S2D_CULL = 11, DVS_S2D_FLOATS = 16 };
typedef struct dvs_fwd_state {
    const int32_t*  radii;
    const float*    splat2d;
    const float*    depth;
    const uint32_t* flags;
    const uint32_t* tiles_touched;
    const uint32_t* sorted_tile;
    const uint32_t* sorted_splat;
    const uint32_t* ranges;
    const float*    final_T;
    const uint32_t* n_contrib;
    uint64_t num_rendered;
    int32_t n, width, height, tiles_x, tiles_y, _pad;
} dvs_fwd_state;

typedef struct dvs_splat_grads {
    float* pos;
    float* sh0;
    float* shN;
    float* opacity;
    float* scale;
    float* rot;
    float* absgrad2d;
    float* mean2d;
    float* dcolor;
} dvs_splat_grads;

typedef struct dvs_ctx dvs_ctx;

dvs_ctx* dvs_create(int device, size_t max_splats, int max_w, int max_h);
void     dvs_destroy(dvs_ctx* ctx);

int dvs_raster_forward(dvs_ctx* ctx, void* stream, const dvs_splats* params, const dvs_camera* cam,
                       const dvs_opts* opts, float* out_rgb, dvs_fwd_state* saved, uint64_t* num_rendered);

int dvs_raster_backward(dvs_ctx* ctx, void* stream, const dvs_splats* params, const dvs_camera* cam,
                        const dvs_opts* opts, const float* dL_drgb, const dvs_splat_grads* out);

int dvs_raster_backward_composite(dvs_ctx* ctx, void* stream, const dvs_camera* cam, const dvs_opts* opts, const float* dL_drgb);
int dvs_raster_backward_project(dvs_ctx* ctx, void* stream, const dvs_splats* params, const dvs_camera* cam,
                                const dvs_opts* opts, const dvs_splat_grads* out);

int dvs_raster_backward_project_chunk(dvs_ctx* ctx, void* stream, const dvs_splats* params, const dvs_camera* cam,
                                      const dvs_opts* opts, const dvs_splat_grads* out, int64_t first, int64_t count);

int dvs_raster_backward_dcolor(dvs_ctx* ctx, void* stream, float* dcolor);

int dvs_sh_grad_combine(dvs_ctx* ctx, void* stream, int n, const float* pos, int sh_degree, int n_views, const float* campos,
                        const float* dcolor, float* g_sh0, float* g_shN, int accumulate, int shn_layout);
int dvs_shn_relayout(dvs_ctx* ctx, void* stream, int n, const float* src, float* dst, int to_tiled);

dvs_ctx* dvs_create_views(int device, size_t max_splats, int max_w, int max_h, int max_views);
int dvs_raster_forward_views(dvs_ctx* ctx, void* stream, const dvs_splats* params, const dvs_camera* cams, int n_views,
                             const dvs_opts* opts, float* out_rgb);
int dvs_raster_backward_views(dvs_ctx* ctx, void* stream, const dvs_splats* params, const dvs_camera* cams, int n_views,
                              const dvs_opts* opts, const float* dL_drgb, const dvs_splat_grads* out);

int dvs_raster_forward_views_prepare(dvs_ctx* ctx, void* stream, const dvs_splats* params, const dvs_camera* cams, int n_views,
                                     const dvs_opts* opts, int64_t first, int64_t count);
int dvs_raster_forward_cancel_prepared(dvs_ctx* ctx);
int dvs_get_view_state(dvs_ctx* ctx, int view, dvs_fwd_state* state);

#define DVS_T_UNKNOWN (~0ull)
int dvs_set_async(dvs_ctx* ctx, int enable);
int dvs_get_num_rendered(dvs_ctx* ctx, void* stream, uint64_t* num_rendered);
int dvs_get_arena_info(dvs_ctx* ctx, uint64_t* instance_capacity, uint64_t* grow_events, uint64_t* last_num_rendered, uint64_t* overflows);
int dvs_get_sort_rank_mode(dvs_ctx* ctx);
int dvs_set_export_sorted_tiles(dvs_ctx* ctx, int enable);

int dvs_debug_record_decisions(dvs_ctx* ctx, uint64_t* take_masks, uint64_t capacity_instances);
int dvs_debug_sort_depth_keys(dvs_ctx* ctx, void* stream, const uint32_t* keys, uint64_t n, uint32_t* sorted_ids, uint32_t* n_sorted, uint32_t* digit_bits);

int dvs_set_backward_variant(dvs_ctx* ctx, int variant);
int dvs_set_forward_variant(dvs_ctx* ctx, int variant);
int dvs_set_live_lists(dvs_ctx* ctx, int enable);

int dvs_sort_pairs_u32(dvs_ctx* ctx, void* stream, uint32_t* keys, uint32_t* vals, uint64_t n, int bit_lo, int bit_hi);
int dvs_export_sorted_keys(dvs_ctx* ctx, void* stream, uint64_t* out_keys);

int dvs_get_bwd_intermediates(dvs_ctx* ctx, const float** rows, int* row_floats);
int dvs_keep_bwd_intermediates(dvs_ctx* ctx, int keep);

int dvs_enable_stage_timing(dvs_ctx* ctx, int enable);
int dvs_get_stage_timing(dvs_ctx* ctx, const char*** names, const float** ms);
int dvs_enable_kernel_probe(dvs_ctx* ctx, int enable);
int dvs_read_kernel_probe(dvs_ctx* ctx, float mean_ms[2], int count[2]);

int dvs_memcpy_d2h(dvs_ctx* ctx, void* host_dst, const void* dev_src, size_t bytes);
int dvs_memcpy_h2d(dvs_ctx* ctx, void* dev_dst, const void* host_src, size_t bytes);
void* dvs_device_malloc(dvs_ctx* ctx, size_t bytes);
void  dvs_device_free(dvs_ctx* ctx, void* p);

const char* dvs_last_error(void);
const char* dvs_version(void);

#ifdef __cplusplus
}
#endif
#endif
```

Baseline: 1851 views/s.

## Add XCD-aware tile-to-block orderings (strips, work-balanced) for raster kernels

Replaces the fixed banded block-to-tile mapping with a selectable order: strips, which interleaves whole tile rows across the 8 XCDs, and a work-balanced order whose per-XCD tile bounds come from a prefix-max scan of the tile ranges. The default picks strips when the strip count divides evenly by 8, which holds for this configuration. The aim is to even out per-XCD render load, since under banded each XCD gets roughly one view and views differ in cost. Forward and both backward render kernels take the new order. Strips may weaken the vertical L2 locality each XCD had within a contiguous view region.

```diff
diff --git a/divshot_amd/_lib.py b/divshot_amd/_lib.py
--- a/divshot_amd/_lib.py
+++ b/divshot_amd/_lib.py
@@ -109,6 +109,8 @@
     "dvs_debug_record_decisions": (C.c_int, [C.c_void_p, C.c_void_p, C.c_uint64]),
     "dvs_set_forward_variant": (C.c_int, [C.c_void_p, C.c_int]),
     "dvs_set_live_lists": (C.c_int, [C.c_void_p, C.c_int]),
+    "dvs_set_tile_order": (C.c_int, [C.c_void_p, C.c_int]),
+    "dvs_debug_get_live_lists": (C.c_int, [C.c_void_p, C.POINTER(C.c_void_p), C.POINTER(C.c_void_p)]),
     "dvs_enable_stage_timing": (C.c_int, [C.c_void_p, C.c_int]),
     "dvs_enable_kernel_probe": (C.c_int, [C.c_void_p, C.c_int]),
     "dvs_read_kernel_probe": (C.c_int, [C.c_void_p, C.POINTER(C.c_float), C.POINTER(C.c_int)]),
diff --git a/divshot_amd/csrc/dvs_api.cpp b/divshot_amd/csrc/dvs_api.cpp
--- a/divshot_amd/csrc/dvs_api.cpp
+++ b/divshot_amd/csrc/dvs_api.cpp
@@ -88,6 +88,7 @@
     uint64_t* total_host = nullptr;
     uint64_t overflow_seen = 0;
     Buf tmp_keys, tmp_vals;
+    Buf tile_bound;
 };
 struct FrontEnd {
     Buf state, hist;
@@ -123,6 +124,10 @@
     uint32_t* live_splat = nullptr;
     uint32_t* live_pos = nullptr;
     bool live_lists = true;
+    int tile_order = DVS_ORDER_STRIPS;
+    bool tile_order_forced = false;
+    uint32_t tile_cost = DVS_WORK_TILE_COST;
+    DvsTileOrder order_used{DVS_ORDER_BANDED, nullptr};
     uint64_t* rec_masks = nullptr; uint64_t rec_cap = 0;
     struct Prep {
         bool valid = false;
@@ -222,6 +227,9 @@
     if (opens >= 0) pr.kind.push_back(opens);
 }
 
+int tile_order_by_name(const char* v) {
+    return !strcmp(v, "banded") ? DVS_ORDER_BANDED : !strcmp(v, "strips") ? DVS_ORDER_STRIPS : !strcmp(v, "work") ? DVS_ORDER_WORK : -1;
+}
 bool fe_no_key16() { static const bool v = [] { const char* e = getenv("DVS_FE_NO_KEY16"); return e && e[0] == '1'; }(); return v; }
 bool fe_no_fuse() { static const bool v = [] { const char* e = getenv("DVS_FE_NO_FUSE_A6"); return e && e[0] == '1'; }(); return v; }
 
@@ -276,6 +284,11 @@
     c->device = device; c->max_splats = max_splats; c->max_w = max_w; c->max_h = max_h; c->max_views = max_views;
     if (const char* v = getenv("DVS_BWD_VARIANT")) c->bwd.variant = v[0] == '0' ? DVS_BWD_BLOCKS : DVS_BWD_TR;
     if (const char* v = getenv("DVS_LIVE_LISTS")) c->fwd.live_lists = v[0] != '0';
+    if (const char* v = getenv("DVS_TILE_ORDER")) {
+        const int o = tile_order_by_name(v);
+        if (o >= 0) { c->fwd.tile_order = o; c->fwd.tile_order_forced = true; }
+    }
+    if (const char* v = getenv("DVS_TILE_COST")) { const long k = atol(v); if (k >= 0 && k <= 1000000) c->fwd.tile_cost = (uint32_t)k; }
     if (hipMalloc((void**)&c->a.total_dev, 32) != hipSuccess || hipHostMalloc((void**)&c->a.total_host, 32, hipHostMallocDefault) != hipSuccess ||
         hipMemset(c->a.total_dev, 0, 32) != hipSuccess) {
         fail(0, "dvs_create", "hipMalloc failed");
@@ -304,7 +317,7 @@
     if (const char* v = getenv("DVS_ASYNC")) c->async_T = v[0] == '1';
     if (ensure_frontend_arenas(c) != DVS_OK ||
         ensure_splat_arenas(c, max_splats * (size_t)max_views) != DVS_OK || ensure_image_arenas(c, max_w, max_h, max_views) != DVS_OK ||
-        ensure_instance_arenas(c, (uint64_t)max_splats * 4 * (uint64_t)max_views) != DVS_OK) {
+        ensure_instance_arenas(c, (uint64_t)max_splats * 4 * (uint64_t)max_views) != DVS_OK || c->a.tile_bound.ensure(64) != DVS_OK) {
         dvs_destroy(c);
         return nullptr;
     }
@@ -426,6 +439,11 @@
 static int fwd_composite_and_publish(dvs_ctx* c, const FwdPass& f, float* out_rgb, dvs_fwd_state* saved, uint64_t* num_rendered, StageScope& tm) {
     Arenas& a = c->a; Forward& fw = c->fwd;
     const int W = f.cams[0].width, H = f.cams[0].height, icur = f.icur;
+    fw.order_used = DvsTileOrder{fw.tile_order_forced ? fw.tile_order : dvs_default_tile_order(f.g.tiles * f.V, f.g.tiles_x), nullptr};
+    if (fw.order_used.order == DVS_ORDER_WORK) {
+        fw.order_used.bound = a.tile_bound.as<int>();
+        HIPCHECK(dvs_launch_tile_bands(f.st, f.g.tiles * f.V, c->fe.tile_ranges, fw.tile_cost, a.tile_bound.as<int>()));
+    }
     probe_event(c, f.st, 0);
     fw.live_splat = nullptr; fw.live_pos = nullptr;
     uint64_t* rec_masks = nullptr; uint64_t rec_cap = 0;
@@ -437,7 +455,7 @@
     uint32_t* const canon = f.ranges_encoded ? a.ranges_canon.as<uint32_t>() : nullptr;
     HIPCHECK(dvs_launch_render_fwd(f.st, W, H, f.g.tiles_x, f.g.tiles_y, f.V, c->fe.tile_ranges, a.inst_splat[icur].as<uint32_t>(),
                                    a.splat2d.as<float>(), CamVec3(f.cams, f.V, &dvs_camera::bg).v, out_rgb, a.final_T.as<float>(),
-                                   a.n_contrib.as<uint32_t>(), fw.live_splat, fw.live_pos, rec_masks, rec_cap, canon));
+                                   a.n_contrib.as<uint32_t>(), fw.live_splat, fw.live_pos, rec_masks, rec_cap, canon, fw.order_used));
     probe_event(c, f.st);
     tm.stage("render_fwd");
 
@@ -548,10 +566,10 @@
     probe_event(c, st, 1);
     if (b.variant == DVS_BWD_TR)
         HIPCHECK(dvs_launch_render_bwd_tr(st, s.width, s.height, s.tiles_x, s.tiles_y, V, s.ranges, s.sorted_splat, s.splat2d, bgs.v, s.final_T,
-                                          s.n_contrib, dL_drgb, b.g_rows.as<float>(), opts->absgrad, opts->grad_mode, c->fwd.live_splat, c->fwd.live_pos));
+                                          s.n_contrib, dL_drgb, b.g_rows.as<float>(), opts->absgrad, opts->grad_mode, c->fwd.live_splat, c->fwd.live_pos, c->fwd.order_used));
     else
         HIPCHECK(dvs_launch_render_bwd_blocks(st, s.width, s.height, s.tiles_x, s.tiles_y, V, s.ranges, s.sorted_splat, s.splat2d,
-                                              bgs.v, s.final_T, s.n_contrib, dL_drgb, b.g_rows.as<float>(), opts->absgrad, opts->grad_mode));
+                                              bgs.v, s.final_T, s.n_contrib, dL_drgb, b.g_rows.as<float>(), opts->absgrad, opts->grad_mode, c->fwd.order_used));
     probe_event(c, st);
     tm.stage("render_bwd");
     b.rows_pending = true;
@@ -832,6 +850,18 @@
     c->fwd.live_lists = enable != 0;
     return DVS_OK;
 }
+int dvs_set_tile_order(dvs_ctx* c, int order) {
+    if (!c || order < DVS_ORDER_BANDED || order > DVS_ORDER_WORK) return fail(DVS_ERR_INVALID, "dvs_set_tile_order", "bad argument");
+    c->fwd.tile_order = order;
+    c->fwd.tile_order_forced = true;
+    return DVS_OK;
+}
+int dvs_debug_get_live_lists(dvs_ctx* c, const uint32_t** live_splat, const uint32_t** live_pos) {
+    if (!c || !live_splat || !live_pos) return fail(DVS_ERR_INVALID, "dvs_debug_get_live_lists", "null argument");
+    if (!c->fwd.have) return fail(DVS_ERR_STATE, "dvs_debug_get_live_lists", "no forward on this context");
+    *live_splat = c->fwd.live_splat; *live_pos = c->fwd.live_pos;
+    return DVS_OK;
+}
 int dvs_set_forward_variant(dvs_ctx* c, int variant) {
     if (!c || (variant != 0 && variant != 1)) return fail(DVS_ERR_INVALID, "dvs_set_forward_variant", "bad argument");
     if (variant == 0)
diff --git a/divshot_amd/csrc/dvs_kernels.h b/divshot_amd/csrc/dvs_kernels.h
--- a/divshot_amd/csrc/dvs_kernels.h
+++ b/divshot_amd/csrc/dvs_kernels.h
@@ -2,6 +2,7 @@
 #include <hip/hip_runtime.h>
 #include <stdint.h>
 #include "dvs_device.h"
+#include "tile_order.h"
 
 hipError_t dvs_launch_preprocess_fwd(hipStream_t st, int n, const float* pos, const float* sh0, const float* shN,
                                      const float* opacity, const float* scale, const float* rot, const DvsCams& cams, int n_views,
@@ -99,6 +100,7 @@
 
 hipError_t dvs_launch_tile_ranges(hipStream_t st, uint64_t T, const uint32_t* sorted_tile, uint32_t* ranges ,
                                   const uint64_t* T_dev = nullptr, uint64_t T_expected = 0);
+hipError_t dvs_launch_tile_bands(hipStream_t st, int num_tiles, const uint32_t* ranges, uint32_t tile_cost, int* bound );
 hipError_t dvs_launch_export_keys(hipStream_t st, uint64_t T, const uint32_t* sorted_tile, const uint32_t* sorted_splat,
                                   const float* depth, uint64_t* out_keys);
 
@@ -106,7 +108,8 @@
                                  const uint32_t* sorted_splat, const float* splat2d, const float* bgs, float* out_color, float* final_T,
                                  uint32_t* n_contrib, uint32_t* live_splat , uint32_t* live_pos ,
                                  uint64_t* take_masks ,
-                                 uint64_t take_cap, uint32_t* ranges_out = nullptr );
+                                 uint64_t take_cap, uint32_t* ranges_out = nullptr ,
+                                 DvsTileOrder order = DvsTileOrder{DVS_ORDER_BANDED, nullptr} );
 enum { DVS_BWD_BLOCKS = 0 , DVS_BWD_REDUCE = 1 , DVS_BWD_MM = 2 ,
        DVS_BWD_TR = 3  };
 
@@ -114,11 +117,12 @@
                                     const uint32_t* sorted_splat, const float* splat2d, const float* bgs , const float* final_T,
                                     const uint32_t* n_contrib, const float* dL_dout, float* grad_rows, int absgrad, int grad_mode,
                                     const uint32_t* live_splat ,
-                                    const uint32_t* live_pos);
+                                    const uint32_t* live_pos, DvsTileOrder order = DvsTileOrder{DVS_ORDER_BANDED, nullptr});
 
 hipError_t dvs_launch_render_bwd_blocks(hipStream_t st, int W, int H, int tiles_x, int tiles_y, int n_views, const uint32_t* ranges,
                                         const uint32_t* sorted_splat, const float* splat2d, const float* bgs , const float* final_T,
-                                        const uint32_t* n_contrib, const float* dL_dout, float* grad_rows, int absgrad, int grad_mode);
+                                        const uint32_t* n_contrib, const float* dL_dout, float* grad_rows, int absgrad, int grad_mode,
+                                        DvsTileOrder order = DvsTileOrder{DVS_ORDER_BANDED, nullptr});
 
 size_t dvs_morton_scratch_bytes(int n);
 hipError_t dvs_launch_morton_order(hipStream_t st, int n, const float* pos, void* scratch, const uint32_t** sorted, const float** bounds);
diff --git a/divshot_amd/csrc/frontend.hip b/divshot_amd/csrc/frontend.hip
--- a/divshot_amd/csrc/frontend.hip
+++ b/divshot_amd/csrc/frontend.hip
@@ -708,6 +708,69 @@
     return hipGetLastError();
 }
 
+#define TB_BLOCK 1024
+__global__ void __launch_bounds__(TB_BLOCK)
+k_tile_bands(int num_tiles, const uint2* __restrict__ ranges, uint32_t tile_cost, int* __restrict__ bound) {
+    constexpr int NW = TB_BLOCK / 64;
+    __shared__ uint32_t s_max[NW];
+    __shared__ uint32_t s_cnt[DVS_XCDS];
+    const int wave = threadIdx.x >> 6, lane = threadIdx.x & 63;
+    const int sec = ((num_tiles + NW * 64 - 1) / (NW * 64)) * 64;
+    const int lo = min(wave * sec, num_tiles), hi = min(lo + sec, num_tiles);
+    uint32_t m = 0;
+    for (int t = lo + lane; t < hi; t += 64) m = max(m, ranges[t].y);
+#pragma unroll
+    for (int d = 32; d >= 1; d >>= 1) m = max(m, (uint32_t)__shfl_xor((int)m, d, 64));
+    if (lane == 0) s_max[wave] = m;
+    if (threadIdx.x < DVS_XCDS) s_cnt[threadIdx.x] = 0u;
+    __syncthreads();
+    uint32_t carry = 0, total = 0;
+#pragma unroll
+    for (int w = 0; w < NW; ++w) { const uint32_t v = s_max[w]; carry = max(carry, w < wave ? v : 0u); total = max(total, v); }
+    const uint64_t ctot = (uint64_t)total + (uint64_t)tile_cost * (uint64_t)num_tiles;
+    uint32_t cnt[DVS_XCDS - 1];
+#pragma unroll
+    for (int k = 0; k < DVS_XCDS - 1; ++k) cnt[k] = 0u;
+    for (int base = lo; base < hi; base += 64) {
+        const int t = base + lane;
+        uint32_t e = t < hi ? ranges[t].y : 0u;
+#pragma unroll
+        for (int d = 1; d < 64; d <<= 1) {
+            const uint32_t o = (uint32_t)__shfl_up((int)e, d, 64);
+            if (lane >= d) e = max(e, o);
+        }
+        e = max(e, carry);
+        carry = (uint32_t)__shfl((int)e, 63, 64);
+        if (t < hi) {
+            const uint64_t c = (uint64_t)e + (uint64_t)tile_cost * (uint64_t)(t + 1);
+#pragma unroll
+            for (int k = 0; k < DVS_XCDS - 1; ++k) cnt[k] += c * DVS_XCDS <= ctot * (uint64_t)(k + 1) ? 1u : 0u;
+        }
+    }
+#pragma unroll
+    for (int k = 0; k < DVS_XCDS - 1; ++k) {
+        uint32_t v = cnt[k];
+#pragma unroll
+        for (int d = 32; d >= 1; d >>= 1) v += (uint32_t)__shfl_xor((int)v, d, 64);
+        if (lane == 0 && v) atomicAdd(&s_cnt[k], v);
+    }
+    __syncthreads();
+    if (threadIdx.x == 0) {
+        int prev = 0;
+        bound[0] = 0;
+        for (int k = 1; k <= DVS_XCDS; ++k) {
+            prev = dvs_work_clamp_bound(k, k < DVS_XCDS ? (int)s_cnt[k - 1] : num_tiles, prev, num_tiles);
+            bound[k] = prev;
+        }
+    }
+}
+
+hipError_t dvs_launch_tile_bands(hipStream_t st, int num_tiles, const uint32_t* ranges, uint32_t tile_cost, int* bound) {
+    if (num_tiles <= 0) return hipSuccess;
+    hipLaunchKernelGGL(k_tile_bands, dim3(1), dim3(TB_BLOCK), 0, st, num_tiles, (const uint2*)ranges, tile_cost, bound);
+    return hipGetLastError();
+}
+
 __global__ void __launch_bounds__(FE_BLOCK)
 k_export_keys(uint64_t T, const uint32_t* __restrict__ sorted_tile, const uint32_t* __restrict__ sorted_splat,
               const float* __restrict__ depth, uint64_t* __restrict__ out) {
diff --git a/divshot_amd/csrc/render.hip b/divshot_amd/csrc/render.hip
--- a/divshot_amd/csrc/render.hip
+++ b/divshot_amd/csrc/render.hip
@@ -75,11 +75,11 @@
              float* __restrict__ out_color , float* __restrict__ final_T , uint32_t* __restrict__ n_contrib,
              uint32_t* __restrict__ live_splat ,
              uint32_t* __restrict__ live_pos ,
-             uint64_t* __restrict__ take_masks , uint64_t take_cap) {
+             uint64_t* __restrict__ take_masks , uint64_t take_cap, DvsTileOrder order) {
     __shared__ FwdLds L;
     (void)bg_arg;
-    const int tile_g = tile_of_block(blockIdx.x, num_tiles);
-    if (tile_g >= num_tiles) return;
+    const int tile_g = tile_of_block(blockIdx.x, num_tiles, tiles_x, order);
+    if (tile_g < 0) return;
     const int view = tile_g / tiles_per_view, tile = tile_g - view * tiles_per_view;
     const float3 bgv = dvs_load_bg(view);
     const float bg0 = bgv.x, bg1 = bgv.y, bg2 = bgv.z;
@@ -185,15 +185,15 @@
 
 hipError_t dvs_launch_render_fwd(hipStream_t st, int W, int H, int tiles_x, int tiles_y, int n_views, const uint32_t* ranges,
                                  const uint32_t* sorted_splat, const float* splat2d, const float* bgs, float* out_color, float* final_T,
-                                 uint32_t* n_contrib, uint32_t* live_splat, uint32_t* live_pos, uint64_t* take_masks, uint64_t take_cap, uint32_t* ranges_out) {
+                                 uint32_t* n_contrib, uint32_t* live_splat, uint32_t* live_pos, uint64_t* take_masks, uint64_t take_cap, uint32_t* ranges_out, DvsTileOrder order) {
     const int tiles_pv = tiles_x * tiles_y, num_tiles = tiles_pv * n_views;
     if (num_tiles <= 0) return hipSuccess;
-    const int grid = ((num_tiles + 7) >> 3) << 3;
+    const int grid = (int)dvs_tile_order_grid(order.order, num_tiles, tiles_x);
     if (take_masks)
         hipLaunchKernelGGL(k_render_fwd<true>, dim3(grid), dim3(RB), 0, st, make_view_bg(n_views, bgs), W, H, tiles_x, tiles_pv, num_tiles,
-                           (const uint2*)ranges, (uint2*)ranges_out, sorted_splat, (const float4*)splat2d, out_color, final_T, n_contrib, live_splat, live_pos, take_masks, take_cap);
+                           (const uint2*)ranges, (uint2*)ranges_out, sorted_splat, (const float4*)splat2d, out_color, final_T, n_contrib, live_splat, live_pos, take_masks, take_cap, order);
     else
         hipLaunchKernelGGL(k_render_fwd<false>, dim3(grid), dim3(RB), 0, st, make_view_bg(n_views, bgs), W, H, tiles_x, tiles_pv, num_tiles,
-                           (const uint2*)ranges, (uint2*)ranges_out, sorted_splat, (const float4*)splat2d, out_color, final_T, n_contrib, live_splat, live_pos, (uint64_t*)nullptr, (uint64_t)0);
+                           (const uint2*)ranges, (uint2*)ranges_out, sorted_splat, (const float4*)splat2d, out_color, final_T, n_contrib, live_splat, live_pos, (uint64_t*)nullptr, (uint64_t)0, order);
     return hipGetLastError();
 }
diff --git a/divshot_amd/csrc/render_blocks.hip b/divshot_amd/csrc/render_blocks.hip
--- a/divshot_amd/csrc/render_blocks.hip
+++ b/divshot_amd/csrc/render_blocks.hip
@@ -130,13 +130,13 @@
                     int num_tiles , const uint2* __restrict__ ranges,
                     const uint32_t* __restrict__ sorted_splat, const float4* __restrict__ splat2d,
                     const float* __restrict__ final_T, const uint32_t* __restrict__ n_contrib, const float* __restrict__ dL_dout ,
-                    float* __restrict__ grow , int lineage) {
+                    float* __restrict__ grow , int lineage, DvsTileOrder order) {
     __shared__ BlockLds L;
     __shared__ float s_tab[4][BK_RB * 12];
     __shared__ uint32_t s_blast[16];
     (void)bg_arg;
-    const int tile_g = tile_of_block(blockIdx.x, num_tiles);
-    if (tile_g >= num_tiles) return;
+    const int tile_g = tile_of_block(blockIdx.x, num_tiles, tiles_x, order);
+    if (tile_g < 0) return;
     const int view = tile_g / tiles_per_view, tile = tile_g - view * tiles_per_view;
     const float3 bgv = dvs_load_bg(view);
     final_T += (size_t)view * W * H; n_contrib += (size_t)view * W * H; dL_dout += (size_t)view * 3 * W * H;
@@ -251,14 +251,14 @@
 
 hipError_t dvs_launch_render_bwd_blocks(hipStream_t st, int W, int H, int tiles_x, int tiles_y, int n_views, const uint32_t* ranges,
                                         const uint32_t* sorted_splat, const float* splat2d, const float* bgs, const float* final_T,
-                                        const uint32_t* n_contrib, const float* dL_dout, float* grad_rows, int absgrad, int grad_mode) {
+                                        const uint32_t* n_contrib, const float* dL_dout, float* grad_rows, int absgrad, int grad_mode, DvsTileOrder order) {
     const int tiles_pv = tiles_x * tiles_y, num_tiles = tiles_pv * n_views;
     if (num_tiles <= 0) return hipSuccess;
-    const int grid = ((num_tiles + 7) >> 3) << 3;
+    const int grid = (int)dvs_tile_order_grid(order.order, num_tiles, tiles_x);
     const int lineage = grad_mode == 1 ? 1 : 0;
 #define DVS_RBB(KERNEL)                                                                                                     \
     hipLaunchKernelGGL(KERNEL, dim3(grid), dim3(RB), 0, st, make_view_bg(n_views, bgs), W, H, tiles_x, tiles_pv, num_tiles, \
-                       (const uint2*)ranges, sorted_splat, (const float4*)splat2d, final_T, n_contrib, dL_dout, grad_rows, lineage)
+                       (const uint2*)ranges, sorted_splat, (const float4*)splat2d, final_T, n_contrib, dL_dout, grad_rows, lineage, order)
     if (absgrad) DVS_RBB(k_render_bwd_blocks<true>); else DVS_RBB(k_render_bwd_blocks<false>);
 #undef DVS_RBB
     return hipGetLastError();
diff --git a/divshot_amd/csrc/render_common.h b/divshot_amd/csrc/render_common.h
--- a/divshot_amd/csrc/render_common.h
+++ b/divshot_amd/csrc/render_common.h
@@ -1,5 +1,6 @@
 #pragma once
 #include "dvs_device.h"
+#include "tile_order.h"
 
 #define RB 256
 
@@ -16,9 +17,10 @@
     return b;
 }
 
-__device__ __forceinline__ int tile_of_block(int b, int num_tiles) {
-    const int chunk = (num_tiles + 7) >> 3;
-    return (b & 7) * chunk + (b >> 3);
+__device__ __forceinline__ int tile_of_block(int b, int num_tiles, int tiles_x, DvsTileOrder o) {
+    if (o.order == DVS_ORDER_STRIPS) return dvs_tile_strips(b, num_tiles, tiles_x);
+    if (o.order == DVS_ORDER_WORK) return dvs_tile_work(b, num_tiles, o.bound);
+    return dvs_tile_banded(b, num_tiles);
 }
 
 __device__ __forceinline__ float swap32_add(float a, float b) {
diff --git a/divshot_amd/csrc/render_tr.hip b/divshot_amd/csrc/render_tr.hip
--- a/divshot_amd/csrc/render_tr.hip
+++ b/divshot_amd/csrc/render_tr.hip
@@ -86,13 +86,13 @@
                 const float* __restrict__ final_T, const uint32_t* __restrict__ n_contrib, const float* __restrict__ dL_dout ,
                 float* __restrict__ grow ,
                 const uint32_t* __restrict__ live_splat ,
-                const uint32_t* __restrict__ live_pos ) {
+                const uint32_t* __restrict__ live_pos , DvsTileOrder order) {
     __shared__ TrLds<BK> L;
     __shared__ __attribute__((aligned(16))) float s_tab[4][(BK + 1) * 12];
     __shared__ __attribute__((aligned(16))) float s_tb[4][TR_SLOTS * TR_SS];
     (void)bg_arg;
-    const int tile_g = tile_of_block(blockIdx.x, num_tiles);
-    if (tile_g >= num_tiles) return;
+    const int tile_g = tile_of_block(blockIdx.x, num_tiles, tiles_x, order);
+    if (tile_g < 0) return;
     const int view = tile_g / tiles_per_view, tile = tile_g - view * tiles_per_view;
     const float3 bgv = dvs_load_bg(view);
     final_T += (size_t)view * W * H; n_contrib += (size_t)view * W * H; dL_dout += (size_t)view * 3 * W * H;
@@ -295,14 +295,14 @@
 hipError_t dvs_launch_render_bwd_tr(hipStream_t st, int W, int H, int tiles_x, int tiles_y, int n_views, const uint32_t* ranges,
                                     const uint32_t* sorted_splat, const float* splat2d, const float* bgs, const float* final_T,
                                     const uint32_t* n_contrib, const float* dL_dout, float* grad_rows, int absgrad, int grad_mode,
-                                    const uint32_t* live_splat, const uint32_t* live_pos) {
+                                    const uint32_t* live_splat, const uint32_t* live_pos, DvsTileOrder order) {
     const int tiles_pv = tiles_x * tiles_y, num_tiles = tiles_pv * n_views;
     if (num_tiles <= 0) return hipSuccess;
-    const int grid = ((num_tiles + 7) >> 3) << 3;
+    const int grid = (int)dvs_tile_order_grid(order.order, num_tiles, tiles_x);
     const int lineage = grad_mode == 1 ? 1 : 0;
 #define DVS_TR(A, LN, BKV)                                                                                                              \
     hipLaunchKernelGGL((k_render_bwd_tr<A, LN, BKV>), dim3(grid), dim3(RB), 0, st, make_view_bg(n_views, bgs), W, H, tiles_x, tiles_pv, \
-                       num_tiles, (const uint2*)ranges, sorted_splat, (const float4*)splat2d, final_T, n_contrib, dL_dout, grad_rows, live_splat, live_pos)
+                       num_tiles, (const uint2*)ranges, sorted_splat, (const float4*)splat2d, final_T, n_contrib, dL_dout, grad_rows, live_splat, live_pos, order)
 #define DVS_TR_B(BKV)                                                                                   \
     do {                                                                                                \
         if (absgrad) { if (lineage) DVS_TR(true, true, BKV); else DVS_TR(true, false, BKV); }           \
diff --git a/divshot_amd/csrc/tile_order.h b/divshot_amd/csrc/tile_order.h
--- /dev/null
+++ b/divshot_amd/csrc/tile_order.h
@@ -0,0 +1,62 @@
+#pragma once
+
+#if defined(__HIPCC__)
+#define DVS_TO_FN __host__ __device__ __forceinline__
+#else
+#define DVS_TO_FN static inline
+#endif
+
+enum { DVS_ORDER_BANDED = 0, DVS_ORDER_STRIPS = 1, DVS_ORDER_WORK = 2 };
+#define DVS_XCDS 8
+#define DVS_WORK_TILE_COST 16u
+struct DvsTileOrder { int order; const int* bound; };
+
+DVS_TO_FN int dvs_tile_banded(int b, int num_tiles) {
+    const int chunk = (num_tiles + 7) >> 3, j = b >> 3;
+    const int t = (b & 7) * chunk + j;
+    return (j < chunk && t < num_tiles) ? t : -1;
+}
+DVS_TO_FN int dvs_tile_strips(int b, int num_tiles, int tiles_x) {
+    const int x = b & 7, j = b >> 3;
+    const int k = j / tiles_x, col = j - k * tiles_x;
+    const long long t = ((long long)x + 8ll * k) * tiles_x + col;
+    return t < (long long)num_tiles ? (int)t : -1;
+}
+DVS_TO_FN int dvs_tile_work(int b, int num_tiles, const int* bound) {
+    const int x = b & 7, j = b >> 3;
+    const int lo = bound[x], hi = bound[x + 1];
+    const long long t = (long long)lo + j;
+    return (lo >= 0 && t < (long long)hi && t < (long long)num_tiles) ? (int)t : -1;
+}
+
+DVS_TO_FN int dvs_work_band_cap(int num_tiles) {
+    const long long c = 2ll * ((num_tiles + 7) >> 3);
+    return c < (long long)num_tiles ? (int)c : num_tiles;
+}
+DVS_TO_FN long long dvs_tile_order_grid(int order, int num_tiles, int tiles_x) {
+    if (order == DVS_ORDER_STRIPS) {
+        const long long strips = ((long long)num_tiles + tiles_x - 1) / tiles_x;
+        return 8ll * ((strips + 7) >> 3) * tiles_x;
+    }
+    if (order == DVS_ORDER_WORK) return 8ll * dvs_work_band_cap(num_tiles);
+    return 8ll * ((num_tiles + 7) >> 3);
+}
+
+DVS_TO_FN int dvs_default_tile_order(int num_tiles, int tiles_x) {
+    const long long strips = ((long long)num_tiles + tiles_x - 1) / tiles_x;
+    return (strips % DVS_XCDS) == 0 ? DVS_ORDER_STRIPS : DVS_ORDER_BANDED;
+}
+
+DVS_TO_FN int dvs_work_clamp_bound(int k, int raw_k, int prev_bound, int num_tiles) {
+    if (k <= 0) return 0;
+    if (k >= DVS_XCDS) return num_tiles;
+    const long long cap = dvs_work_band_cap(num_tiles);
+    long long lo = (long long)num_tiles - (DVS_XCDS - k) * cap;
+    if (lo < prev_bound) lo = prev_bound;
+    long long hi = prev_bound + cap;
+    if (hi > num_tiles) hi = num_tiles;
+    long long v = raw_k;
+    if (v < lo) v = lo;
+    if (v > hi) v = hi;
+    return (int)v;
+}
diff --git a/divshot_amd/raster.py b/divshot_amd/raster.py
--- a/divshot_amd/raster.py
+++ b/divshot_amd/raster.py
@@ -95,6 +95,17 @@
 
     def set_live_lists(self, on=True):
         check(lib.dvs_set_live_lists(self.ctx, 1 if on else 0), "dvs_set_live_lists")
+
+    def set_tile_order(self, order):
+        v = {"banded": 0, "strips": 1, "work": 2}.get(order, order)
+        check(lib.dvs_set_tile_order(self.ctx, int(v)), "dvs_set_tile_order")
+
+    def live_lists(self, T):
+        ls, lp = C.c_void_p(), C.c_void_p()
+        check(lib.dvs_debug_get_live_lists(self.ctx, C.byref(ls), C.byref(lp)), "dvs_debug_get_live_lists")
+        if not ls.value or not lp.value:
+            return None
+        return self._d2h(ls.value, (T,), np.uint32), self._d2h(lp.value, (T,), np.uint32)
 
     def record_decisions(self, capacity_instances):
         if not capacity_instances:
diff --git a/include/dvs_raster.h b/include/dvs_raster.h
--- a/include/dvs_raster.h
+++ b/include/dvs_raster.h
@@ -139,6 +139,9 @@
 int dvs_set_backward_variant(dvs_ctx* ctx, int variant);
 int dvs_set_forward_variant(dvs_ctx* ctx, int variant);
 int dvs_set_live_lists(dvs_ctx* ctx, int enable);
+enum { DVS_TILE_ORDER_BANDED = 0, DVS_TILE_ORDER_STRIPS = 1, DVS_TILE_ORDER_WORK = 2 };
+int dvs_set_tile_order(dvs_ctx* ctx, int order);
+int dvs_debug_get_live_lists(dvs_ctx* ctx, const uint32_t** live_splat, const uint32_t** live_pos);
 
 int dvs_sort_pairs_u32(dvs_ctx* ctx, void* stream, uint32_t* keys, uint32_t* vals, uint64_t n, int bit_lo, int bit_hi);
 int dvs_export_sorted_keys(dvs_ctx* ctx, void* stream, uint64_t* out_keys);
```

Result: no change. 1865 views/s, median of 6 (+0.8%).
